# NingZhang1/pyscf_isdf

Measured on AMD Instinct MI355X. Metric: isdf_build_plus_get_jk_wall_time, lower is better.
Workload: dtype f64

## Files before the change

include/mi355_isdf.h:

```cpp
#ifndef MI355_ISDF_H
#define MI355_ISDF_H

#include <stdint.h>

#ifdef __cplusplus
extern "C" {
#endif

typedef struct isdf_ctx* isdf_handle;

#define ISDF_OK 0
#define ISDF_ERR_ARG 1
#define ISDF_ERR_HIP 2
#define ISDF_ERR_LIB 3
#define ISDF_ERR_NUM 4

int isdf_abi_version(void);

int isdf_create(int device_id, isdf_handle* out);
int isdf_destroy(isdf_handle h);
int isdf_set_stream(isdf_handle h, void* hip_stream);
const char* isdf_last_error(isdf_handle h);
int64_t isdf_workspace_bytes(isdf_handle h);
int isdf_release_workspace(isdf_handle h);
int isdf_set_option(isdf_handle h, const char* key, int value);
int isdf_set_coulomb_omega(isdf_handle h, double omega);
int isdf_set_coulomb_cutoff(isdf_handle h, double rc);
int isdf_set_coulomb_ws(isdf_handle h, double alpha, const double ak[9], const int32_t mesh[3], const double maxq[3],
                        const double* d_vq);

int isdf_prof_enable(isdf_handle h, int on);
int isdf_prof_reset(isdf_handle h);
int isdf_prof_count(isdf_handle h);
int isdf_prof_get(isdf_handle h, int index, char* name, int name_cap, int64_t* launches,
                  double* total_ms, double* total_work);

int isdf_eval_ao(isdf_handle h,
                 const int32_t* atm, int natm, const int32_t* bas, int nbas,
                 const double* env, int nenv,
                 const double* Ls, int nimgs, const double* rcut,
                 const double* d_coords, int64_t ngrids,
                 double* d_ao, int64_t ld);

int isdf_eval_ao_deriv1(isdf_handle h, const int32_t* atm, int natm, const int32_t* bas, int nbas, const double* env,
                        int nenv, const double* Ls, int nimgs, const double* rcut, const double* d_coords,
                        int64_t ngrids, double* d_ao, int64_t ld, int64_t plane_stride);
int isdf_eval_ao_k_deriv1(isdf_handle h, const int32_t* atm, int natm, const int32_t* bas, int nbas, const double* env,
                          int nenv, const double* Ls, int nimgs, const double* rcut, const double kpt[3], int periodic_part,
                          const double* d_coords, int64_t ngrids, double* d_re, double* d_im, int64_t ld,
                          int64_t plane_stride);

int isdf_eval_ao_k(isdf_handle h,
                   const int32_t* atm, int natm, const int32_t* bas, int nbas,
                   const double* env, int nenv,
                   const double* Ls, int nimgs, const double* rcut,
                   const double kpt[3], int periodic_part,
                   const double* d_coords, int64_t ngrids,
                   double* d_re, double* d_im, int64_t ld);

int isdf_block_row_absmax(isdf_handle h, const double* d_src, int nrow, int64_t ld, int nblk, const int64_t* d_blk_off,
                          double* d_out);
int isdf_gather_cols(isdf_handle h, const double* d_src, int nrow, int64_t ld_src,
                     const int64_t* d_idx, int64_t n, double* d_dst, int64_t ld_dst);

int isdf_partition_by_atom(isdf_handle h, const double* d_coords, int64_t ngrids, const double* atom_coords, int natm,
                           const double a[9], double tie_atol, int32_t* d_owner);

int isdf_select_ip(isdf_handle h, const double* d_ao, int nao, int64_t ld,
                   int nblk, const int64_t* blk_off, const int32_t* nip,
                   double tol, double tie_rtol,
                   double* d_L, int64_t ldL, int64_t* d_piv, int32_t* rank);

int isdf_select_ip_gram(isdf_handle h, double* d_A, int m, int64_t ldA, int nip, double tol, double tie_rtol,
                        int panel, int64_t* d_piv, int32_t* rank);

int isdf_select_ip_cplx(isdf_handle h, const double* d_ao, int nao, int nh, int64_t ld,
                        int nblk, const int64_t* blk_off, const int32_t* nip,
                        double tol, double tie_rtol,
                        double* d_L, int64_t ldL, int64_t* d_piv, int32_t* rank);

int isdf_fit_from_chol(isdf_handle h, double* d_L, int k, int64_t m, int64_t ldL,
                       const int64_t* d_piv);

int isdf_fit_prepare(isdf_handle h, const double* d_ao, int nao, int64_t ld,
                     const int64_t* d_ip, int P, double reg_rel, double* d_aoP, double* d_chol,
                     double* reg_used);
int isdf_fit_apply(isdf_handle h, const double* d_chol, const double* d_aoP, int P, int nao,
                   const double* d_ao, int64_t ng, int64_t ld, int forward_only,
                   double* d_theta, int64_t ldt);
int isdf_fit_prepare_cplx(isdf_handle h, const double* d_ao, int nao, int nh, int64_t ld,
                          const int64_t* d_ip, int P, double reg_rel, double* d_aoP, double* d_chol,
                          double* reg_used);
int isdf_fit_apply_cplx(isdf_handle h, const double* d_chol, const double* d_aoP, int P, int nao, int nh,
                        const double* d_ao, int64_t ng, int64_t ld, int forward_only,
                        double* d_theta, int64_t ldt);
int isdf_fit_global(isdf_handle h, const double* d_ao, int nao, int64_t ngrids, int64_t ld,
                    const int64_t* d_ip, int P, double reg_rel, double* d_theta, int64_t ldt,
                    double* d_aoP, double* reg_used);

int isdf_gather_aoP(isdf_handle h, const double* d_ao, int nao, int64_t ld, const int64_t* d_ip, int P,
                    double* d_aoP);
int isdf_gram_sq(isdf_handle h, const double* d_aoP, int P, int nao, int nh, double* d_A);
int isdf_pair_gram_rows(isdf_handle h, const double* d_aoP, int P, int nao, int nh, const double* d_ao,
                        int64_t ng, int64_t ld, double* d_B, int64_t ldb);
int isdf_block_chol(isdf_handle h, const double* d_A, int P, int nblk, const int32_t* blk_off,
                    double shift_rel, double* d_D, double* shift_used);
int isdf_block_solve(isdf_handle h, const double* d_D, int P, int nblk, const int32_t* blk_off, int side,
                     int trans, double* d_X, int64_t n, int64_t ldx);
int isdf_block_invert(isdf_handle h, const double* d_D, int P, int nblk, const int32_t* blk_off, double* d_Dinv);
int isdf_block_apply(isdf_handle h, const double* d_Dinv, int64_t ldd, int nblk, const int32_t* blk_off,
                     double* d_X, int64_t n, int64_t ldx);
int isdf_pair_rows_block_apply(isdf_handle h, const double* d_aoP, int P, int nao, const double* d_ao, int64_t ng,
                               int64_t ld, const double* d_Dinv, int64_t ldd, int nblk, const int32_t* blk_off,
                               double* d_B, int64_t ldb);

int isdf_gram_prod(isdf_handle h, const double* d_aoP, int P, int nao, const double* d_psiP, int nocc, double* d_A);
int isdf_pair_prod_rows(isdf_handle h, const double* d_aoP, int P, int nao, const double* d_psiP, int nocc,
                        const double* d_ao, int64_t ld, const double* d_psi, int64_t ldpsi, int64_t ng,
                        double* d_B, int64_t ldb);
int isdf_factor_solve_half(isdf_handle h, const double* d_fac, int P, int backward, double* d_X, int64_t n, int64_t ldx);
int isdf_gram_prod_cplx(isdf_handle h, const double* d_aoP, int P, int nao, int nh, const double* d_psiP, int npsi, int npsi_h,
                        double* d_A);
int isdf_pair_prod_rows_cplx(isdf_handle h, const double* d_aoP, int P, int nao, int nh, const double* d_psiP, int npsi,
                             int npsi_h, const double* d_ao, int64_t ld, const double* d_psi, int64_t ldpsi, int64_t ng,
                             double* d_B, int64_t ldb);

int isdf_shift_diag(isdf_handle h, double* d_A, int P, double shift_rel);
int isdf_chol_inplace(isdf_handle h, double* d_A, int P, double shift_rel, double* d_scratch, double* reg_used);

int isdf_factor_solve(isdf_handle h, const double* d_fac, int P, double* d_X, int64_t n, int64_t ldx);

int isdf_bj_probe_vectors(isdf_handle h, double* d_T, int n, const double* d_fac, const double* d_D, int P,
                          int nblk, const int32_t* blk_off);
int isdf_rows_combine(isdf_handle h, const double* d_E, int n, int64_t ldE, int rows, const double* d_Y,
                      int64_t ng, int64_t ldy, double* d_F, int64_t ldf, int accumulate);

int isdf_bj_probe_rows(isdf_handle h, double* d_T, int n, const double* d_fac, const double* d_D, int P, int nblk,
                       const int32_t* blk_off, const double* d_Yp, int64_t ng, int64_t ldy, double* d_F, int64_t ldf);

int isdf_gather_T(isdf_handle h, const double* d_L, int k, int64_t ldL, const int64_t* d_piv,
                  double* d_T);
int isdf_W_from_factor(isdf_handle h, const double* d_F, int P, int kind, double* d_M, int64_t ldm);

int isdf_coulomb_W(isdf_handle h, const double* d_theta, int P, int64_t ldt,
                   const int32_t mesh[3], const double a[9],
                   int row0, int nrows, int batch, int upper_only, double* d_W, int64_t ldw);
int isdf_coulG_half(isdf_handle h, const int32_t mesh[3], const double a[9], double* d_out);
int isdf_spectral_supported(isdf_handle h, const int32_t mesh[3], int batch, int* ok);
int isdf_spectral_rows(isdf_handle h, const double* d_in, int nrows, int64_t ld, const int32_t mesh[3], const int32_t* d_idx,
                       const double* d_scale, int npts, int batch, double* d_out, int64_t ldx);
int isdf_coulomb_rows(isdf_handle h, const double* d_in, int nrows, int64_t ld,
                      const int32_t mesh[3], const double a[9], int batch, double* d_out, int64_t ldo);
int isdf_symmetrize_upper(isdf_handle h, double* d_W, int P, int64_t ldw);
int isdf_symmetrize_mean(isdf_handle h, double* d_W, int P, int64_t ldw, int antisymmetric);

int isdf_get_j(isdf_handle h, const double* d_ao, int nao, int64_t ngrids, int64_t ld,
               const int32_t mesh[3], const double a[9],
               const double* d_dm, int nset, double* d_vj);
int isdf_rho(isdf_handle h, const double* d_ao, int nao, int64_t ng, int64_t ld,
             const double* d_dm, int nset, double* d_rho, int64_t ldrho);
int isdf_coulomb_potential(isdf_handle h, double* d_rho_inout, int nset, int64_t ldrho,
                           const int32_t mesh[3], const double a[9]);
int isdf_vj_from_vR(isdf_handle h, const double* d_ao, int nao, int64_t ng, int64_t ld,
                    const double* d_vR, int nset, int64_t ldv, double* d_vj);

int isdf_get_k_exact(isdf_handle h, const double* d_ao, int nao, int64_t ngrids, int64_t ld,
                     const double* d_C, int nocc, const int32_t mesh[3], const double a[9],
                     int i0, int ni, int max_rows, double* d_vk);

int isdf_get_k(isdf_handle h, const double* d_aoP, int P, int nao,
               const double* d_W, int64_t ldw, int row0, int nrows,
               const double* d_dm, int nset, double* d_vk);

int isdf_coulG_q(isdf_handle h, const int32_t mesh[3], const double a[9], const double q[3], int wrap_around,
                 double omega, double* d_out);

int isdf_coulomb_Wq(isdf_handle h, const double* d_theta, int P, int64_t ldt, const int32_t mesh[3],
                    const double* d_coulG, double weight, int row0, int nrows, int batch,
                    int upper_only, double* d_Wre, double* d_Wim, int64_t ldw);
int isdf_symmetrize_hermitian(isdf_handle h, double* d_Wre, double* d_Wim, int P, int64_t ldw);
int isdf_finish_Wq(isdf_handle h, const double* d_Wre, const double* d_Wim, int P, int64_t ldw,
                   const double* d_phase, double* d_Wc);
int isdf_get_k_pair(isdf_handle h, const double* d_A1, const double* d_A2, const double* d_D2,
                    const double* d_Wq, int P, int nao, double scale, double* d_vk);

int isdf_get_k_exact_kpt(isdf_handle h, const double* d_u1r, const double* d_u1i, int nao, int64_t ld1,
                         const double* d_m2r, const double* d_m2i, int nocc, int64_t ld2, const int32_t mesh[3],
                         const double* d_coulG, double weight, int i0, int ni, int max_rows, double* d_vk_re,
                         double* d_vk_im);

int isdf_coulomb_rows_q(isdf_handle h, const double* d_rows, int nrows, int64_t ld, const int32_t mesh[3],
                        const double* d_coulG, double* d_re, double* d_im);
int isdf_nyquist_spectra(isdf_handle h, const double* d_rows, int nrows, int64_t ld, const int32_t mesh[3], int axis,
                         double* d_re, double* d_im);
int isdf_zhadamard_planes(isdf_handle h, double* d_Ar, double* d_Ai, int64_t lda, const double* d_Br, const double* d_Bi,
                          int64_t ldb, int rows, int64_t cols);
int isdf_rho_k(isdf_handle h, const double* d_ur, const double* d_ui, int nao, int64_t ng, int64_t ld,
               const double* d_DTr, const double* d_DTi, double scale, double* d_rho);
int isdf_vj_k(isdf_handle h, const double* d_ur, const double* d_ui, int nao, int64_t ng, int64_t ld,
              const double* d_vR, double* d_vj_re, double* d_vj_im);

int isdf_pp_local_potential(isdf_handle h, int natm, const double* coords, const double* pp_par,
                            const int32_t mesh[3], const double a[9], double* d_vlocR);
int isdf_pp_projector_overlaps(isdf_handle h, const int32_t* atm, int natm, const int32_t* bas, int nbas,
                               const double* env, int nenv, const double* coords, const double kpt[3],
                               const int32_t* proj_tab, const double* proj_rl, int nproj,
                               const int32_t mesh[3], const double a[9], double* d_out);

int isdf_gemm_nn(isdf_handle h, int M, int64_t N, int K, double alpha, const double* d_A, int64_t lda, const double* d_B,
                 int64_t ldb, double beta, double* d_C, int64_t ldc);
int isdf_hadamard_rows(isdf_handle h, double* d_X, int64_t ldx, const double* d_Y, int64_t ldy, int rows, int64_t cols);

int isdf_uniform_grid(isdf_handle h, const int32_t mesh[3], const double a[9], double* d_coords_soa);
int isdf_rho_pair(isdf_handle h, const double* d_aoA, int nA, const double* d_aoB, int nB, int64_t ng, int64_t ld,
                  const double* d_dm, int nset, double* d_rho, int64_t ldrho);
int isdf_mg_embed_density(isdf_handle h, const double* d_field, int nset, const int32_t mesh_sub[3], double scale,
                          double* d_spec, const int32_t mesh[3], int accumulate);
int isdf_mg_restrict_potential(isdf_handle h, const double* d_spec, int nset, const int32_t mesh[3],
                               const int32_t mesh_sub[3], double scale, double* d_field);
int isdf_mg_coulomb_kernel(isdf_handle h, double* d_spec, int nset, const int32_t mesh[3], const double a[9]);
int isdf_lda_exchange(isdf_handle h, const double* d_rho, int64_t n, double* d_exc, double* d_vxc);
int isdf_lda_vwn_add(isdf_handle h, const double* d_rho, int64_t n, double* d_exc, double* d_vxc);
int isdf_gga_b88(isdf_handle h, const double* d_rho, const double* d_grad, int64_t gstride, int64_t n, double* d_exc,
                 double* d_vrho, double* d_w, int64_t wstride);
int isdf_xc_fused(isdf_handle h, const double* d_rho, const double* d_grad, int64_t gstride, int64_t n, double c_slater, double c_b88,
                  double c_vwn, int vwn_rpa, double c_lyp, double* d_exc, double* d_vrho, double* d_w, int64_t wstride);
int isdf_gga_lyp_polarised(isdf_handle h, const double* d_rho, const double* d_grad, int64_t gcstride, int64_t sstride, int64_t n,
                           double weight, int accumulate, double* d_ec, double* d_vrho, double* d_w, int64_t wcstride,
                           int64_t osstride);
int isdf_lda_exchange_fxc(isdf_handle h, const double* d_rho, int64_t n, double* d_fxc);
int isdf_lda_vwn_fxc_add(isdf_handle h, const double* d_rho, int64_t n, double* d_fxc);
int isdf_gga_b88_fxc(isdf_handle h, const double* d_rho0, int64_t r0stride, int64_t n, const double* d_rho1, int64_t r1xstride,
                     int64_t r1nstride, int nset, double* d_wv, int64_t wxstride, int64_t wnstride, double* d_fxc, int64_t fstride);
int isdf_xc_fxc_apply(isdf_handle h, int nx, const double* d_fxc, int64_t fxstride, int64_t fystride, int64_t n, const double* d_rho1,
                      int64_t r1xstride, int64_t r1nstride, int nset, double* d_wv, int64_t wxstride, int64_t wnstride, int accumulate);
int isdf_dot(isdf_handle h, const double* d_x, const double* d_y, int64_t n, double* result);

int isdf_gemm_nt(isdf_handle h, int M, int N, int64_t K, double alpha, const double* d_A, int64_t lda,
                 const double* d_B, int64_t ldb, const double* d_kscale, double beta, double* d_C,
                 int64_t ldc);

#ifdef __cplusplus
}
#endif
#endif
```

pyscf_isdf_amd/backend.py:

```python
import ctypes
import os
import numpy as np
import torch
from . import lib as _lib

_vp = ctypes.c_void_p


def _np_ptr(a):
    return a.ctypes.data_as(_vp)


class HipBackend:
    name = 'hip-gfx950'

    def __init__(self, device=0):
        if not torch.cuda.is_available():
            raise _lib.IsdfError('no GPU visible to torch; the ISDF path has no CPU fallback')
        self.device = torch.device('cuda', device)
        torch.cuda.set_device(self.device)
        self.handle = _lib.Handle(device)
        if os.environ.get('ISDF_TRSM') == 'subst':
            self.set_option('trsm_substitution', 1)
        if os.environ.get('ISDF_OWN_FFT') in ('0', '1', '2'):
            self.set_option('own_fft', int(os.environ['ISDF_OWN_FFT']))
        if os.environ.get('ISDF_GEMM_NN') == '1':
            self.set_option('gemm_nn_own', 1)

    def empty(self, shape, dtype=torch.float64):
        return torch.empty(shape, dtype=dtype, device=self.device)

    def zeros(self, shape, dtype=torch.float64):
        return torch.zeros(shape, dtype=dtype, device=self.device)

    def to_device(self, a, dtype=None):
        a = np.ascontiguousarray(a)
        if not a.flags.writeable:
            a = a.copy()
        t = torch.as_tensor(a)
        if dtype is not None:
            t = t.to(dtype)
        return t.to(self.device)

    def to_host(self, t):
        return t.detach().cpu().numpy()

    kernel_epoch = 0

    def set_coulomb_omega(self, omega):
        self.kernel_epoch += 1
        self.handle.call('isdf_set_coulomb_omega', float(omega or 0.0))

    def set_coulomb_cutoff(self, rc):
        self.kernel_epoch += 1
        self.handle.call('isdf_set_coulomb_cutoff', float(rc or 0.0))

    def set_coulomb_ws(self, ws):
        self.kernel_epoch += 1
        if ws is None:
            self.handle.call('isdf_set_coulomb_ws', 0.0, None, None, None, None)
            self._ws_table = None
            return
        ak = np.ascontiguousarray(ws['a'], dtype=np.float64)
        mesh = np.ascontiguousarray(ws['mesh'], dtype=np.int32)
        maxq = np.ascontiguousarray(ws['maxq'], dtype=np.float64)
        self._ws_table = self.to_device(np.ascontiguousarray(ws['vq'], dtype=np.float64))
        self.handle.call('isdf_set_coulomb_ws', float(ws['alpha']), _np_ptr(ak), _np_ptr(mesh), _np_ptr(maxq),
                         self._p(self._ws_table))

    def set_option(self, key, value):
        self.kernel_epoch += 1
        self.handle.call('isdf_set_option', key.encode(), int(value))

    def free_bytes(self):
        free, _ = torch.cuda.mem_get_info(self.device)
        return int(free + torch.cuda.memory_reserved(self.device) - torch.cuda.memory_allocated(self.device))

    def empty_cache(self):
        torch.cuda.empty_cache()

    def synchronize(self):
        torch.cuda.synchronize(self.device)

    def new_stream(self):
        return torch.cuda.Stream(device=self.device)

    def on_stream(self, stream):
        return torch.cuda.stream(stream)

    def record_event(self):
        ev = torch.cuda.Event()
        ev.record(torch.cuda.current_stream(self.device))
        return ev

    def wait_event(self, ev):
        if ev is not None:
            torch.cuda.current_stream(self.device).wait_event(ev)

    def release_workspace(self):
        self.handle.call('isdf_release_workspace')

    def prof_enable(self, on=True):
        self.handle.call('isdf_prof_enable', int(bool(on)))

    def prof_reset(self):
        self.handle.call('isdf_prof_reset')

    def prof_results(self):
        out = {}
        n = self.handle.lib.isdf_prof_count(self.handle.h)
        for i in range(n):
            name = ctypes.create_string_buffer(128)
            launches = ctypes.c_int64(0)
            ms = ctypes.c_double(0)
            work = ctypes.c_double(0)
            self.handle.call('isdf_prof_get', i, name, 128, ctypes.byref(launches), ctypes.byref(ms), ctypes.byref(work))
            out[name.value.decode()] = dict(launches=launches.value, ms=ms.value, work=work.value)
        return out

    def _stream(self):
        s = torch.cuda.current_stream(self.device).cuda_stream
        self.handle.call('isdf_set_stream', _vp(s))

    @staticmethod
    def _p(t):
        assert t.is_contiguous() or t.stride(-1) == 1
        return _vp(t.data_ptr())

    def eval_ao(self, atm, bas, env, Ls, rcut, coords_soa, ao):
        self._stream()
        atm = np.ascontiguousarray(atm, dtype=np.int32)
        bas = np.ascontiguousarray(bas, dtype=np.int32)
        env = np.ascontiguousarray(env, dtype=np.float64)
        Ls = np.ascontiguousarray(Ls, dtype=np.float64)
        rcut = np.ascontiguousarray(rcut, dtype=np.float64)
        G = coords_soa.shape[1]
        assert coords_soa.is_contiguous() and ao.stride(1) == 1 and ao.shape[1] >= G
        self.handle.call('isdf_eval_ao', _np_ptr(atm), len(atm), _np_ptr(bas), len(bas), _np_ptr(env), len(env),
                         _np_ptr(Ls), len(Ls), _np_ptr(rcut), self._p(coords_soa), G, self._p(ao), ao.stride(0))

    def eval_ao_deriv1(self, atm, bas, env, Ls, rcut, coords_soa, ao4):
        self._stream()
        atm = np.ascontiguousarray(atm, dtype=np.int32)
        bas = np.ascontiguousarray(bas, dtype=np.int32)
        env = np.ascontiguousarray(env, dtype=np.float64)
        Ls = np.ascontiguousarray(Ls, dtype=np.float64)
        rcut = np.ascontiguousarray(rcut, dtype=np.float64)
        G = coords_soa.shape[1]
        assert coords_soa.is_contiguous() and ao4.dim() == 3 and ao4.shape[0] == 4 and ao4.stride(2) == 1 and ao4.shape[2] >= G
        self.handle.call('isdf_eval_ao_deriv1', _np_ptr(atm), len(atm), _np_ptr(bas), len(bas), _np_ptr(env), len(env),
                         _np_ptr(Ls), len(Ls), _np_ptr(rcut), self._p(coords_soa), G, self._p(ao4), ao4.stride(1), ao4.stride(0))

    def eval_ao_k_deriv1(self, atm, bas, env, Ls, rcut, kpt, periodic_part, coords_soa, out_re, out_im):
        self._stream()
        atm = np.ascontiguousarray(atm, dtype=np.int32)
        bas = np.ascontiguousarray(bas, dtype=np.int32)
        env = np.ascontiguousarray(env, dtype=np.float64)
        Ls = np.ascontiguousarray(Ls, dtype=np.float64)
        rcut = np.ascontiguousarray(rcut, dtype=np.float64)
        kpt = np.ascontiguousarray(kpt, dtype=np.float64)
        G = coords_soa.shape[1]
        assert out_re.dim() == 3 and out_re.shape[0] == 4 and tuple(out_re.shape) == tuple(out_im.shape)
        assert out_re.stride() == out_im.stride() and out_re.stride(2) == 1 and out_re.shape[2] >= G
        self.handle.call('isdf_eval_ao_k_deriv1', _np_ptr(atm), len(atm), _np_ptr(bas), len(bas), _np_ptr(env), len(env),
                         _np_ptr(Ls), len(Ls), _np_ptr(rcut), _np_ptr(kpt), int(bool(periodic_part)), self._p(coords_soa), G,
                         self._p(out_re), self._p(out_im), out_re.stride(1), out_re.stride(0))

    def gather_cols(self, src, idx, dst):
        self._stream()
        assert idx.dtype == torch.int64 and src.stride(1) == 1 and dst.stride(1) == 1
        self.handle.call('isdf_gather_cols', self._p(src), src.shape[0], src.stride(0), self._p(idx), idx.numel(),
                         self._p(dst), dst.stride(0))

    def block_row_absmax(self, src, blk_off):
        self._stream()
        d_off = self.to_device(np.ascontiguousarray(blk_off, dtype=np.int64))
        out = self.empty((src.shape[0], len(blk_off) - 1))
        self.handle.call('isdf_block_row_absmax', self._p(src), src.shape[0], src.stride(0), len(blk_off) - 1, self._p(d_off), self._p(out))
        return self.to_host(out)

    def partition_by_atom(self, coords, atom_coords, a, tie_atol=1e-9):
        self._stream()
        coords_soa = self.to_device(np.ascontiguousarray(np.asarray(coords, dtype=np.float64).T))
        atoms = np.ascontiguousarray(atom_coords, dtype=np.float64)
        a = np.ascontiguousarray(a, dtype=np.float64)
        G = coords_soa.shape[1]
        owner = self.empty((G,), dtype=torch.int32)
        self.handle.call('isdf_partition_by_atom', self._p(coords_soa), G, _np_ptr(atoms), len(atoms), _np_ptr(a), float(tie_atol),
                         self._p(owner))
        return self.to_host(owner)

    def select_ip(self, ao, blk_off, nip, tol, tie_rtol, L, piv):
        self._stream()
        blk_off = np.ascontiguousarray(blk_off, dtype=np.int64)
        nip = np.ascontiguousarray(nip, dtype=np.int32)
        rank = np.zeros(len(nip), dtype=np.int32)
        assert piv.dtype == torch.int64 and piv.is_contiguous() and ao.stride(1) == 1 and L.stride(1) == 1
        self.handle.call('isdf_select_ip', self._p(ao), ao.shape[0], ao.stride(0), len(nip), _np_ptr(blk_off),
                         _np_ptr(nip), float(tol), float(tie_rtol), self._p(L), L.stride(0), self._p(piv), _np_ptr(rank))
        return rank

    def select_ip_gram(self, A, nip, tol, tie_rtol, piv, panel=0):
        self._stream()
        assert piv.dtype == torch.int64 and piv.is_contiguous() and A.stride(1) == 1 and A.shape[0] == A.shape[1]
        rank = ctypes.c_int32(0)
        self.handle.call('isdf_select_ip_gram', self._p(A), A.shape[0], A.stride(0), int(nip), float(tol), float(tie_rtol),
                         int(panel), self._p(piv), ctypes.byref(rank))
        return int(rank.value)

    def fit_from_chol(self, L, k, m, piv):
        self._stream()
        self.handle.call('isdf_fit_from_chol', self._p(L), int(k), int(m), L.stride(0), self._p(piv))

    def fit_prepare(self, ao, ip, reg_rel, aoP, chol):
        self._stream()
        assert ip.dtype == torch.int64 and aoP.is_contiguous() and chol.is_contiguous()
        reg = ctypes.c_double(0.0)
        self.handle.call('isdf_fit_prepare', self._p(ao), ao.shape[0], ao.stride(0), self._p(ip), ip.numel(),
                         float(reg_rel), self._p(aoP), self._p(chol), ctypes.byref(reg))
        return reg.value

    def fit_apply(self, chol, aoP, ao, ng, theta, forward_only=False):
        self._stream()
        self.handle.call('isdf_fit_apply', self._p(chol), self._p(aoP), aoP.shape[0], aoP.shape[1], self._p(ao),
                         int(ng), ao.stride(0), int(bool(forward_only)), self._p(theta), theta.stride(0))

    def gather_aoP(self, ao, ip, aoP):
        self._stream()
        self.handle.call('isdf_gather_aoP', self._p(ao), ao.shape[0], ao.stride(0), self._p(ip), ip.numel(), self._p(aoP))

    def gram_sq(self, aoP, A, nh=0):
        self._stream()
        self.handle.call('isdf_gram_sq', self._p(aoP), aoP.shape[0], aoP.shape[1], int(nh), self._p(A))

    def pair_gram_rows(self, aoP, ao, ng, B, nh=0):
        self._stream()
        self.handle.call('isdf_pair_gram_rows', self._p(aoP), aoP.shape[0], aoP.shape[1], int(nh), self._p(ao), int(ng),
                         ao.stride(0), self._p(B), B.stride(0))

    def gram_prod(self, aoP, psiP, A):
        self._stream()
        assert aoP.is_contiguous() and psiP.is_contiguous() and A.is_contiguous() and aoP.shape[0] == psiP.shape[0]
        self.handle.call('isdf_gram_prod', self._p(aoP), aoP.shape[0], aoP.shape[1], self._p(psiP), psiP.shape[1], self._p(A))

    def pair_prod_rows(self, aoP, psiP, ao, psi, ng, B):
        self._stream()
        assert aoP.is_contiguous() and psiP.is_contiguous() and aoP.shape[0] == psiP.shape[0]
        assert ao.stride(1) == 1 and psi.stride(1) == 1 and B.stride(1) == 1
        self.handle.call('isdf_pair_prod_rows', self._p(aoP), aoP.shape[0], aoP.shape[1], self._p(psiP), psiP.shape[1],
                         self._p(ao), ao.stride(0), self._p(psi), psi.stride(0), int(ng), self._p(B), B.stride(0))

    def gram_prod_cplx(self, aoP, nh, psiP, npsi_h, A):
        self._stream()
        assert aoP.is_contiguous() and psiP.is_contiguous() and A.is_contiguous() and aoP.shape[0] == psiP.shape[0]
        self.handle.call('isdf_gram_prod_cplx', self._p(aoP), aoP.shape[0], aoP.shape[1], int(nh), self._p(psiP), psiP.shape[1],
                         int(npsi_h), self._p(A))

    def pair_prod_rows_cplx(self, aoP, nh, psiP, npsi_h, ao, psi, ng, B):
        self._stream()
        assert aoP.is_contiguous() and psiP.is_contiguous() and aoP.shape[0] == psiP.shape[0]
        assert ao.stride(1) == 1 and psi.stride(1) == 1 and B.stride(1) == 1
        self.handle.call('isdf_pair_prod_rows_cplx', self._p(aoP), aoP.shape[0], aoP.shape[1], int(nh), self._p(psiP),
                         psiP.shape[1], int(npsi_h), self._p(ao), ao.stride(0), self._p(psi), psi.stride(0), int(ng), self._p(B),
                         B.stride(0))

    def factor_solve_half(self, fac, backward, X):
        self._stream()
        self.handle.call('isdf_factor_solve_half', self._p(fac), fac.shape[0], int(bool(backward)), self._p(X), X.shape[1],
                         X.stride(0))

    def block_chol(self, A, blk_off, shift_rel, D):
        self._stream()
        blk_off = np.ascontiguousarray(blk_off, dtype=np.int32)
        used = ctypes.c_double(0.0)
        self.handle.call('isdf_block_chol', self._p(A), A.shape[0], len(blk_off) - 1, _np_ptr(blk_off), float(shift_rel),
                         self._p(D), ctypes.byref(used))
        return used.value

    def block_solve(self, D, blk_off, side, trans, X):
        self._stream()
        blk_off = np.ascontiguousarray(blk_off, dtype=np.int32)
        n = X.shape[1] if side == 0 else X.shape[0]
        self.handle.call('isdf_block_solve', self._p(D), D.stride(0), len(blk_off) - 1, _np_ptr(blk_off), int(side), int(trans),
                         self._p(X), int(n), X.stride(0))

    def block_invert(self, D, blk_off, Dinv):
        self._stream()
        blk_off = np.ascontiguousarray(blk_off, dtype=np.int32)
        assert D.is_contiguous() and Dinv.is_contiguous() and Dinv.shape == D.shape
        self.handle.call('isdf_block_invert', self._p(D), D.shape[0], len(blk_off) - 1, _np_ptr(blk_off), self._p(Dinv))

    def block_apply(self, Dinv, blk_off, X):
        self._stream()
        blk_off = np.ascontiguousarray(blk_off, dtype=np.int32)
        self.handle.call('isdf_block_apply', self._p(Dinv), Dinv.stride(0), len(blk_off) - 1, _np_ptr(blk_off), self._p(X),
                         X.shape[1], X.stride(0))

    def pair_rows_block_apply(self, aoP, ao, ng, Dinv, blk_off, B):
        self._stream()
        blk_off = np.ascontiguousarray(blk_off, dtype=np.int32)
        assert aoP.stride(1) == 1 and aoP.stride(0) == aoP.shape[1]
        self.handle.call('isdf_pair_rows_block_apply', self._p(aoP), aoP.shape[0], aoP.shape[1], self._p(ao), int(ng), ao.stride(0),
                         self._p(Dinv), Dinv.stride(0), len(blk_off) - 1, _np_ptr(blk_off), self._p(B), B.stride(0))

    def shift_diag(self, A, shift_rel):
        self._stream()
        self.handle.call('isdf_shift_diag', self._p(A), A.shape[0], float(shift_rel))

    def chol_inplace(self, A, shift_rel, scratch=None):
        self._stream()
        reg = ctypes.c_double(0.0)
        assert scratch is None or scratch.numel() >= A.numel()
        self.handle.call('isdf_chol_inplace', self._p(A), A.shape[0], float(shift_rel),
                         self._p(scratch) if scratch is not None else None, ctypes.byref(reg))
        return reg.value

    def factor_solve(self, fac, X):
        self._stream()
        self.handle.call('isdf_factor_solve', self._p(fac), fac.shape[0], self._p(X), X.shape[1], X.stride(0))

    def bj_probe_rows(self, T, fac, D, blk_off, Yp, ng, F):
        self._stream()
        blk_off = np.ascontiguousarray(blk_off, dtype=np.int32)
        self.handle.call('isdf_bj_probe_rows', self._p(T), T.shape[0], self._p(fac), self._p(D), D.shape[0],
                         len(blk_off) - 1, _np_ptr(blk_off), self._p(Yp), int(ng), Yp.stride(0), self._p(F), F.stride(0))

    def bj_probe_vectors(self, T, fac, D, blk_off):
        self._stream()
        blk_off = np.ascontiguousarray(blk_off, dtype=np.int32)
        assert T.is_contiguous()
        self.handle.call('isdf_bj_probe_vectors', self._p(T), T.shape[0], self._p(fac), self._p(D), D.shape[0],
                         len(blk_off) - 1, _np_ptr(blk_off))

    def rows_combine(self, E, Y, F, accumulate=False):
        self._stream()
        assert E.stride(1) == 1 and Y.stride(1) == 1 and F.stride(1) == 1 and E.shape[1] == Y.shape[0]
        self.handle.call('isdf_rows_combine', self._p(E), E.shape[0], E.stride(0), E.shape[1], self._p(Y), Y.shape[1],
                         Y.stride(0), self._p(F), F.stride(0), int(bool(accumulate)))

    def gather_T(self, L, k, piv, T):
        self._stream()
        assert T.is_contiguous() and T.shape == (k, k)
        self.handle.call('isdf_gather_T', self._p(L), int(k), L.stride(0), self._p(piv), self._p(T))

    def W_from_factor(self, F, kind, M):
        self._stream()
        assert F.is_contiguous()
        self.handle.call('isdf_W_from_factor', self._p(F), M.shape[0], int(kind), self._p(M), M.stride(0))

    def fit_global(self, ao, ngrids, ip, reg_rel, theta, aoP):
        self._stream()
        assert ip.dtype == torch.int64 and aoP.is_contiguous()
        reg = ctypes.c_double(0.0)
        self.handle.call('isdf_fit_global', self._p(ao), ao.shape[0], int(ngrids), ao.stride(0), self._p(ip),
                         ip.numel(), float(reg_rel), self._p(theta), theta.stride(0), self._p(aoP), ctypes.byref(reg))
        return reg.value

    def coulomb_W(self, theta, mesh, a, row0, nrows, batch, W, upper_only=False):
        self._stream()
        mesh = np.ascontiguousarray(mesh, dtype=np.int32)
        a = np.ascontiguousarray(a, dtype=np.float64)
        self.handle.call('isdf_coulomb_W', self._p(theta), theta.shape[0], theta.stride(0), _np_ptr(mesh), _np_ptr(a),
                         int(row0), int(nrows), int(batch), int(bool(upper_only)), self._p(W), W.stride(0))

    def coulomb_rows(self, rows, mesh, a, batch, out=None):
        self._stream()
        out = rows if out is None else out
        mesh = np.ascontiguousarray(mesh, dtype=np.int32)
        a = np.ascontiguousarray(a, dtype=np.float64)
        self.handle.call('isdf_coulomb_rows', self._p(rows), rows.shape[0], rows.stride(0), _np_ptr(mesh), _np_ptr(a),
                         int(batch), self._p(out), out.stride(0))

    def spectral_supported(self, mesh, batch=512):
        ok = ctypes.c_int(0)
        mesh = np.ascontiguousarray(mesh, dtype=np.int32)
        self.handle.call('isdf_spectral_supported', _np_ptr(mesh), int(batch), ctypes.byref(ok))
        return bool(ok.value)

    def coulG_half(self, mesh, a):
        self._stream()
        mesh = np.ascontiguousarray(mesh, dtype=np.int32)
        a = np.ascontiguousarray(a, dtype=np.float64)
        out = self.empty((int(mesh[0]) * int(mesh[1]) * (int(mesh[2]) // 2 + 1),))
        self.handle.call('isdf_coulG_half', _np_ptr(mesh), _np_ptr(a), self._p(out))
        return self.to_host(out).reshape(int(mesh[0]), int(mesh[1]), int(mesh[2]) // 2 + 1)

    def spectral_rows(self, rows, mesh, idx, scale, out, batch=512):
        self._stream()
        mesh = np.ascontiguousarray(mesh, dtype=np.int32)
        assert rows.is_contiguous() and out.stride(1) == 1 and idx.dtype == torch.int32 and out.stride(0) % 2 == 0
        self.handle.call('isdf_spectral_rows', self._p(rows), rows.shape[0], rows.stride(0), _np_ptr(mesh), self._p(idx),
                         self._p(scale), int(idx.numel()), int(batch), self._p(out), out.stride(0))

    def symmetrize_upper(self, W):
        self._stream()
        self.handle.call('isdf_symmetrize_upper', self._p(W), W.shape[0], W.stride(0))

    def symmetrize_mean(self, W, antisymmetric=False):
        self._stream()
        self.handle.call('isdf_symmetrize_mean', self._p(W), W.shape[0], W.stride(0), int(bool(antisymmetric)))

    def get_j(self, ao, ngrids, mesh, a, dm, vj):
        self._stream()
        mesh = np.ascontiguousarray(mesh, dtype=np.int32)
        a = np.ascontiguousarray(a, dtype=np.float64)
        assert dm.is_contiguous() and vj.is_contiguous()
        self.handle.call('isdf_get_j', self._p(ao), ao.shape[0], int(ngrids), ao.stride(0), _np_ptr(mesh), _np_ptr(a),
                         self._p(dm), dm.shape[0], self._p(vj))

    def rho(self, ao, ng, dm, rho):
        self._stream()
        self.handle.call('isdf_rho', self._p(ao), ao.shape[0], int(ng), ao.stride(0), self._p(dm), dm.shape[0],
                         self._p(rho), rho.stride(0))

    def coulomb_potential(self, rho, mesh, a):
        self._stream()
        mesh = np.ascontiguousarray(mesh, dtype=np.int32)
        a = np.ascontiguousarray(a, dtype=np.float64)
        self.handle.call('isdf_coulomb_potential', self._p(rho), rho.shape[0], rho.stride(0), _np_ptr(mesh), _np_ptr(a))

    def vj_from_vR(self, ao, ng, vR, vj):
        self._stream()
        self.handle.call('isdf_vj_from_vR', self._p(ao), ao.shape[0], int(ng), ao.stride(0), self._p(vR), vR.shape[0],
                         vR.stride(0), self._p(vj))

    def get_k(self, aoP, W, row0, nrows, dm, vk):
        self._stream()
        assert aoP.is_contiguous() and dm.is_contiguous() and vk.is_contiguous()
        self.handle.call('isdf_get_k', self._p(aoP), aoP.shape[0], aoP.shape[1], self._p(W), W.stride(0), int(row0),
                         int(nrows), self._p(dm), dm.shape[0], self._p(vk))

    def get_k_exact(self, ao, ngrids, C, mesh, a, i0, ni, max_rows, vk):
        self._stream()
        mesh = np.ascontiguousarray(mesh, dtype=np.int32)
        a = np.ascontiguousarray(a, dtype=np.float64)
        assert C.is_contiguous() and vk.is_contiguous()
        self.handle.call('isdf_get_k_exact', self._p(ao), ao.shape[0], int(ngrids), ao.stride(0), self._p(C), C.shape[1],
                         _np_ptr(mesh), _np_ptr(a), int(i0), int(ni), int(max_rows), self._p(vk))

    def gemm_nn(self, A, B, C, alpha=1.0, beta=0.0):
        self._stream()
        self.handle.call('isdf_gemm_nn', A.shape[0], B.shape[1], A.shape[1], float(alpha), self._p(A), A.stride(0), self._p(B),
                         B.stride(0), float(beta), self._p(C), C.stride(0))

    def hadamard_rows(self, X, Y):
        self._stream()
        self.handle.call('isdf_hadamard_rows', self._p(X), X.stride(0), self._p(Y), Y.stride(0), X.shape[0], X.shape[1])

    def gemm_nt(self, A, B, C, alpha=1.0, beta=0.0, kscale=None):
        self._stream()
        M, K = A.shape
        N = B.shape[0]
        assert B.shape[1] == K and tuple(C.shape) == (M, N) and A.stride(1) == 1 and B.stride(1) == 1 and C.stride(1) == 1
        ks = self._p(kscale) if kscale is not None else _vp(0)
        self.handle.call('isdf_gemm_nt', M, N, K, float(alpha), self._p(A), A.stride(0), self._p(B), B.stride(0), ks,
                         float(beta), self._p(C), C.stride(0))

    def uniform_grid(self, mesh, a):
        self._stream()
        mesh = np.ascontiguousarray(mesh, dtype=np.int32)
        a = np.ascontiguousarray(a, dtype=np.float64)
        out = self.empty((3, int(np.prod(mesh))))
        self.handle.call('isdf_uniform_grid', _np_ptr(mesh), _np_ptr(a), self._p(out))
        return out

    def rho_pair(self, aoA, aoB, ng, dm, rho):
        self._stream()
        assert aoA.stride(0) == aoB.stride(0) and aoA.stride(1) == 1 and aoB.stride(1) == 1 and dm.is_contiguous()
        assert tuple(dm.shape[1:]) == (aoA.shape[0], aoB.shape[0])
        self.handle.call('isdf_rho_pair', self._p(aoA), aoA.shape[0], self._p(aoB), aoB.shape[0], int(ng), aoA.stride(0),
                         self._p(dm), dm.shape[0], self._p(rho), rho.stride(0))

    def mg_embed_density(self, field, mesh_sub, scale, spec, mesh, accumulate=True):
        self._stream()
        mesh_sub = np.ascontiguousarray(mesh_sub, dtype=np.int32)
        mesh = np.ascontiguousarray(mesh, dtype=np.int32)
        assert field.is_contiguous() and spec.is_contiguous() and spec.dtype == torch.complex128
        assert field.shape[1] == int(np.prod(mesh_sub)) and spec.shape[1] == int(mesh[0]) * int(mesh[1]) * (int(mesh[2]) // 2 + 1)
        self.handle.call('isdf_mg_embed_density', self._p(field), field.shape[0], _np_ptr(mesh_sub), float(scale), self._p(spec),
                         _np_ptr(mesh), int(bool(accumulate)))

    def mg_restrict_potential(self, spec, mesh, mesh_sub, scale, field):
        self._stream()
        mesh_sub = np.ascontiguousarray(mesh_sub, dtype=np.int32)
        mesh = np.ascontiguousarray(mesh, dtype=np.int32)
        assert field.is_contiguous() and spec.is_contiguous() and spec.dtype == torch.complex128
        assert field.shape[1] == int(np.prod(mesh_sub)) and spec.shape[1] == int(mesh[0]) * int(mesh[1]) * (int(mesh[2]) // 2 + 1)
        self.handle.call('isdf_mg_restrict_potential', self._p(spec), spec.shape[0], _np_ptr(mesh), _np_ptr(mesh_sub), float(scale),
                         self._p(field))

    def mg_coulomb_kernel(self, spec, mesh, a):
        self._stream()
        mesh = np.ascontiguousarray(mesh, dtype=np.int32)
        a = np.ascontiguousarray(a, dtype=np.float64)
        assert spec.is_contiguous() and spec.dtype == torch.complex128
        self.handle.call('isdf_mg_coulomb_kernel', self._p(spec), spec.shape[0], _np_ptr(mesh), _np_ptr(a))

    def lda_exchange(self, rho, exc, vxc):
        self._stream()
        assert rho.is_contiguous() and exc.is_contiguous() and vxc.is_contiguous()
        self.handle.call('isdf_lda_exchange', self._p(rho), rho.numel(), self._p(exc), self._p(vxc))

# ... 199 lines not shown
```

pyscf_isdf_amd/csrc/common.h:

```cpp
#pragma once
#include <hip/hip_runtime.h>
#include <rocblas/rocblas.h>
#include <rocsolver/rocsolver.h>
#include <hipfft/hipfft.h>
#include <cstdint>
#include <cstdio>
#include <cstring>
#include <string>
#include <vector>
#include <map>
#include "../../include/mi355_isdf.h"

struct FftPlan {
  hipfftHandle fwd = 0, bwd = 0;
  size_t work_bytes = 0;
};

struct ProfRec {
  hipEvent_t e0 = nullptr, e1 = nullptr;
};
struct ProfEntry {
  std::vector<ProfRec> recs;
  double work = 0.0;
  double ms = 0.0;
  int64_t launches = 0;
};

struct WsKernel {
  double alpha = 0.0;
  double ak[9] = {0};
  int mesh[3] = {0, 0, 0};
  double maxq[3] = {0, 0, 0};
  const double* vq = nullptr;
};

struct isdf_ctx {
  int profiling = 0;
  std::map<std::string, ProfEntry> prof;
  int device = 0;
  hipStream_t stream = nullptr;
  rocblas_handle blas = nullptr;
  std::string err;
  std::map<std::vector<int>, FftPlan> plans;
  std::map<std::string, std::pair<void*, size_t>> ws;
  int num_cu = 256;
  int trsm_substitution = 0;
  int own_fft = 2;
  int gemm_nn_own = 0;
  int attr_gemm_b = 0, attr_gemm_nn = 0;
  int conv_pipe = 1;
  int conv_sub_rows = 0;
  int gram_pivot_tpb = 256;
  int gram_compact = 1;
  int gram_compact_permille = 875;
  int block_apply_waves = 16;
  int block_apply_reg = 1;
  double coul_omega = 0.0;
  double coul_rc = 0.0;
  int coul_sphere = 0;
  WsKernel wsk;
};

int isdf_fail(isdf_handle h, int code, const char* fmt, ...);
void* isdf_ws(isdf_handle h, const char* name, size_t bytes);
int isdf_get_plan(isdf_handle h, const int32_t mesh[3], int batch, FftPlan** out);
int get_coulG_half(isdf_handle h, const int32_t mesh[3], const double a[9], double extra_scale, double** out);
bool conv_rows_own_supported(const int32_t mesh[3], int nb);
bool conv_rows_q_own_supported(isdf_handle h, const int32_t mesh[3], int nb);
bool spectral_rows_own_supported(isdf_handle h, const int32_t mesh[3], int nb);
int spectral_rows_own(isdf_handle h, const double* d_in, int nb, const int32_t mesh[3], const int32_t* d_idx, const double* d_scale,
                      int npts, double* d_out, int64_t ldx, HIP_vector_type<double, 2u>* zbuf);
int conv_rows_q_own(isdf_handle h, const double* d_in, double* d_re, double* d_im, int nb, const int32_t mesh[3], const double* tab,
                    double2* zhalf, double2* zfull);
int conv_rows_own(isdf_handle h, const double* d_in, double* d_out, int nb, const int32_t mesh[3], const double* cg,
                  double2* zbuf);

#define HIP_TRY(h, expr)                                                                    \
  do {                                                                                      \
    hipError_t e_ = (expr);                                                                 \
    if (e_ != hipSuccess)                                                                   \
      return isdf_fail(h, ISDF_ERR_HIP, "%s:%d %s -> %s", __FILE__, __LINE__, #expr,        \
                       hipGetErrorString(e_));                                              \
  } while (0)
#define BLAS_TRY(h, expr)                                                                   \
  do {                                                                                      \
    rocblas_status s_ = (expr);                                                             \
    if (s_ != rocblas_status_success)                                                       \
      return isdf_fail(h, ISDF_ERR_LIB, "%s:%d %s -> rocblas status %d", __FILE__, __LINE__, \
                       #expr, (int)s_);                                                     \
  } while (0)
#define FFT_TRY(h, expr)                                                                    \
  do {                                                                                      \
    hipfftResult r_ = (expr);                                                               \
    if (r_ != HIPFFT_SUCCESS)                                                               \
      return isdf_fail(h, ISDF_ERR_LIB, "%s:%d %s -> hipfft result %d", __FILE__, __LINE__,  \
                       #expr, (int)r_);                                                     \
  } while (0)
#define KERNEL_CHECK(h) HIP_TRY(h, hipGetLastError())
#define ARG_CHECK(h, cond)                                                                  \
  do {                                                                                      \
    if (!(cond)) return isdf_fail(h, ISDF_ERR_ARG, "%s:%d argument check failed: %s",       \
                                  __FILE__, __LINE__, #cond);                               \
  } while (0)

static inline int64_t cdiv(int64_t a, int64_t b) { return (a + b - 1) / b; }

struct ProfScope {
  isdf_handle h;
  ProfRec rec;
  ProfEntry* ent = nullptr;
  ProfScope(isdf_handle h_, const char* name, double work, int64_t launches = 1) : h(h_) {
    if (!h || !h->profiling) return;
    ent = &h->prof[name];
    ent->work += work;
    ent->launches += launches;
    if (hipEventCreate(&rec.e0) != hipSuccess || hipEventCreate(&rec.e1) != hipSuccess) { ent = nullptr; return; }
    (void)hipEventRecord(rec.e0, h->stream);
  }
  ~ProfScope() {
    if (!ent) return;
    (void)hipEventRecord(rec.e1, h->stream);
    ent->recs.push_back(rec);
  }
};

int gemm_nt_f64(isdf_handle h, int M, int N, int64_t K, double alpha, const double* A, int64_t lda,
                const double* B, int64_t ldb, double beta, double* C, int64_t ldc);
int gemm_nt_f64_scaled(isdf_handle h, int M, int N, int64_t K, double alpha, const double* A, int64_t lda,
                       const double* B, int64_t ldb, const double* kscale, double beta, double* C,
                       int64_t ldc);
int trsm_lower_left(isdf_handle h, bool trans, int m, int64_t n, const double* L, int64_t ldl, double* X, int64_t ldx);
int trsm_lower_right(isdf_handle h, bool trans, int m, int64_t n, const double* L, int64_t ldl, double* X, int64_t ldx);
int block_forward_solve(isdf_handle h, const double* D, int64_t ldd, int nblk, const int32_t* blk_off_host, double* X,
                        int64_t ldx, int64_t n);
int block_apply_inverse(isdf_handle h, const double* Dinv, int64_t ldd, int nblk, const int32_t* blk_off_host, double* X,
                        int64_t ldx, int64_t n, bool square_input = false);
int transpose_rm(isdf_handle h, const double* src, int64_t lds, int64_t rows, int64_t cols, double* dst, int64_t ldd);
int tri_left(isdf_handle h, bool trans, int m, int64_t n, const double* L, int64_t ldl, double* X, int64_t ldx);
int tri_right(isdf_handle h, bool trans, int m, int64_t n, const double* L, int64_t ldl, double* X, int64_t ldx);
bool gemm_nn_f64_supported(isdf_handle h, int64_t M, int64_t N, int64_t K, const double* A, int64_t lda, const double* B,
                           int64_t ldb);
int gemm_nn_f64(isdf_handle h, int64_t M, int64_t N, int64_t K, const double* A, int64_t lda, const double* B, int64_t ldb,
                double* C, int64_t ldc, bool square);
int gemm_rm(isdf_handle h, char opA, char opB, int64_t M, int64_t N, int64_t K, double alpha,
            const double* A, int64_t lda, const double* B, int64_t ldb, double beta, double* C,
            int64_t ldc);
```

pyscf_isdf_amd/csrc/gemm_f64.hip:

```cpp
#include "common.h"
#include <cstdlib>

int gemm_rm(isdf_handle h, char opA, char opB, int64_t M, int64_t N, int64_t K, double alpha,
            const double* A, int64_t lda, const double* B, int64_t ldb, double beta, double* C,
            int64_t ldc) {
  ARG_CHECK(h, M < 2147483647LL && N < 2147483647LL && K < 2147483647LL && lda < 2147483647LL &&
                   ldb < 2147483647LL && ldc < 2147483647LL);
  const rocblas_operation ta = (opA == 'N') ? rocblas_operation_none : rocblas_operation_transpose;
  const rocblas_operation tb = (opB == 'N') ? rocblas_operation_none : rocblas_operation_transpose;
  ProfScope ps(h, "rocblas_dgemm[flop]", 2.0 * M * N * (double)K);
  BLAS_TRY(h, rocblas_dgemm(h->blas, tb, ta, (rocblas_int)N, (rocblas_int)M, (rocblas_int)K, &alpha, B,
                            (rocblas_int)ldb, A, (rocblas_int)lda, &beta, C, (rocblas_int)ldc));
  return ISDF_OK;
}

namespace {

typedef double d4 __attribute__((ext_vector_type(4)));

constexpr int BM = 128, BN = 128, BK = 16;
constexpr int LDT = 17;
constexpr int TPB = 256;

struct GemmArgs {
  const double* A; int64_t lda;
  const double* B; int64_t ldb;
  const double* kscale;
  double* P;
  int64_t ldp, slab_stride;
  int M, N;
  int64_t K, kslab;
  int ntm, ntn, nslab;
  int64_t nunits, nunits_pad;
  double alpha, beta;
  int direct;
};

template <bool FAST>
__global__ __launch_bounds__(TPB, 2) void gemm_nt_mfma_kernel(GemmArgs g) {
  __shared__ double sA[2][BM * LDT];
  __shared__ double sB[2][BN * LDT];

  const int64_t bid = blockIdx.x;
  const int64_t per_xcd = g.nunits_pad / 8;
  const int64_t unit = (bid % 8) * per_xcd + bid / 8;
  if (unit >= g.nunits) return;
  const int tm = (int)(unit % g.ntm);
  const int tn = (int)((unit / g.ntm) % g.ntn);
  const int slab = (int)(unit / ((int64_t)g.ntm * g.ntn));
  const int64_t k0 = (int64_t)slab * g.kslab;
  const int64_t k1 = (k0 + g.kslab < g.K) ? k0 + g.kslab : g.K;
  const int nchunks = (int)((k1 - k0 + BK - 1) / BK);

  const int tid = threadIdx.x;
  const int lane = tid & 63, wave = tid >> 6;
  const int wm = wave >> 1, wn = wave & 1;

  const int srow = tid >> 3;
  const int sseg = tid & 7;
  const int arow0 = tm * BM + srow, brow0 = tn * BN + srow;
  const int mlast = g.M - 1, nlast = g.N - 1;
  const double* __restrict__ Ag = g.A;
  const double* __restrict__ Bg = g.B;
  const int64_t lda = g.lda, ldb = g.ldb;

  double2 ra0, ra1, ra2, ra3, rb0, rb1, rb2, rb3;
#define ISDF_LOAD_ONE(I, RA, RB)                                                              \
  {                                                                                           \
    const int ra = min(arow0 + 32 * I, mlast), rb = min(brow0 + 32 * I, nlast);               \
    const double* pa = Ag + (int64_t)ra * lda + k;                                            \
    const double* pb = Bg + (int64_t)rb * ldb + k;                                            \
    if (FAST) {                                                                               \
      RA = *reinterpret_cast<const double2*>(pa);                                             \
      RB = *reinterpret_cast<const double2*>(pb);                                             \
    } else {                                                                                  \
      RA.x = v0 ? pa[0] : 0.0; RA.y = v1 ? pa[1] : 0.0;                                       \
      RB.x = v0 ? pb[0] : 0.0; RB.y = v1 ? pb[1] : 0.0;                                       \
    }                                                                                         \
    RB.x *= s0; RB.y *= s1;                                                                   \
  }
#define ISDF_LOAD_CHUNK(C)                                                                    \
  {                                                                                           \
    const int64_t k = k0 + (int64_t)(C) * BK + sseg * 2;                                      \
    const bool v0 = FAST || (k < k1), v1 = FAST || (k + 1 < k1);                              \
    double s0 = 1.0, s1 = 1.0;                                                                \
    if (g.kscale) { if (v0) s0 = g.kscale[k]; if (v1) s1 = g.kscale[k + 1]; }                 \
    ISDF_LOAD_ONE(0, ra0, rb0) ISDF_LOAD_ONE(1, ra1, rb1)                                     \
    ISDF_LOAD_ONE(2, ra2, rb2) ISDF_LOAD_ONE(3, ra3, rb3)                                     \
  }
#define ISDF_STORE_ONE(BUF, I, RA, RB)                                                        \
  { double* qa = &sA[BUF][(srow + 32 * I) * LDT + sseg * 2];                                  \
    double* qb = &sB[BUF][(srow + 32 * I) * LDT + sseg * 2];                                  \
    qa[0] = RA.x; qa[1] = RA.y; qb[0] = RB.x; qb[1] = RB.y; }
#define ISDF_STORE_CHUNK(BUF)                                                                 \
  { ISDF_STORE_ONE(BUF, 0, ra0, rb0) ISDF_STORE_ONE(BUF, 1, ra1, rb1)                         \
    ISDF_STORE_ONE(BUF, 2, ra2, rb2) ISDF_STORE_ONE(BUF, 3, ra3, rb3) }

  d4 acc[4][4];
#pragma unroll
  for (int i = 0; i < 4; ++i)
#pragma unroll
    for (int j = 0; j < 4; ++j) acc[i][j] = (d4){0.0, 0.0, 0.0, 0.0};

  const int frow = lane & 15, fk = lane >> 4;
  ISDF_LOAD_CHUNK(0)
  ISDF_STORE_CHUNK(0)
  __syncthreads();
  for (int c = 0; c < nchunks; ++c) {
    const int buf = c & 1;
    if (c + 1 < nchunks) ISDF_LOAD_CHUNK(c + 1)
    const double* pa = &sA[buf][(wm * 64 + frow) * LDT + fk];
    const double* pb = &sB[buf][(wn * 64 + frow) * LDT + fk];
    double a0[4], b0[4], a1[4], b1[4];
#define ISDF_FRAGS(KK, AF, BF)                                                                \
    _Pragma("unroll") for (int i = 0; i < 4; ++i) {                                           \
      AF[i] = pa[i * 16 * LDT + (KK) * 4];                                                    \
      BF[i] = pb[i * 16 * LDT + (KK) * 4];                                                    \
    }
#define ISDF_MFMA16(AF, BF)                                                                   \
    _Pragma("unroll") for (int i = 0; i < 4; ++i)                                             \
      _Pragma("unroll") for (int j = 0; j < 4; ++j)                                           \
        acc[i][j] = __builtin_amdgcn_mfma_f64_16x16x4f64(AF[i], BF[j], acc[i][j], 0, 0, 0);
    ISDF_FRAGS(0, a0, b0)
    ISDF_FRAGS(1, a1, b1)
    ISDF_MFMA16(a0, b0)
    ISDF_FRAGS(2, a0, b0)
    ISDF_MFMA16(a1, b1)
    ISDF_FRAGS(3, a1, b1)
    ISDF_MFMA16(a0, b0)
    ISDF_MFMA16(a1, b1)
    if (c + 1 < nchunks) ISDF_STORE_CHUNK(buf ^ 1)
    __syncthreads();
  }

  double* out = g.P + (int64_t)slab * g.slab_stride;
#pragma unroll
  for (int i = 0; i < 4; ++i) {
#pragma unroll
    for (int r = 0; r < 4; ++r) {
      const int row = tm * BM + wm * 64 + i * 16 + (lane >> 4) + 4 * r;
      if (row >= g.M) continue;
#pragma unroll
      for (int j = 0; j < 4; ++j) {
        const int col = tn * BN + wn * 64 + j * 16 + (lane & 15);
        if (col >= g.N) continue;
        double* q = out + (int64_t)row * g.ldp + col;
        const double v = acc[i][j][r];
        if (g.direct) *q = (g.beta == 0.0) ? g.alpha * v : g.alpha * v + g.beta * (*q);
        else *q = v;
      }
    }
  }
}

constexpr int BM2 = 256;
constexpr int TPB2 = 512;

template <bool SCALED>
__global__ __launch_bounds__(TPB2, 2) void gemm_nt_mfma_kernel_b(GemmArgs g) {
  extern __shared__ double smem[];
  double* sA = smem;
  double* sB = smem + 2 * BM2 * LDT;
  const int64_t bid = blockIdx.x;
  const int64_t per_xcd = g.nunits_pad / 8;
  const int64_t unit = (bid % 8) * per_xcd + bid / 8;
  if (unit >= g.nunits) return;
  const int tm = (int)(unit % g.ntm);
  const int tn = (int)((unit / g.ntm) % g.ntn);
  const int slab = (int)(unit / ((int64_t)g.ntm * g.ntn));
  const int64_t k0 = (int64_t)slab * g.kslab;
  const int64_t k1 = (k0 + g.kslab < g.K) ? k0 + g.kslab : g.K;
  const int nchunks = (int)((k1 - k0) / BK);
  const int last = nchunks - 1;

  const int tid = threadIdx.x;
  const int lane = tid & 63, wave = tid >> 6;
  const int wm = wave >> 1, wn = wave & 1;
  const int srow = tid >> 3;
  const int sseg = tid & 7;
  const int mlast = g.M - 1, nlast = g.N - 1;
  const double* pA0 = g.A + (int64_t)min(tm * BM2 + srow, mlast) * g.lda + k0 + sseg * 2;
  const double* pA1 = g.A + (int64_t)min(tm * BM2 + srow + 64, mlast) * g.lda + k0 + sseg * 2;
  const double* pA2 = g.A + (int64_t)min(tm * BM2 + srow + 128, mlast) * g.lda + k0 + sseg * 2;
  const double* pA3 = g.A + (int64_t)min(tm * BM2 + srow + 192, mlast) * g.lda + k0 + sseg * 2;
  const double* pB0 = g.B + (int64_t)min(tn * BN + srow, nlast) * g.ldb + k0 + sseg * 2;
  const double* pB1 = g.B + (int64_t)min(tn * BN + srow + 64, nlast) * g.ldb + k0 + sseg * 2;
  const double* pS = SCALED ? g.kscale + k0 + sseg * 2 : nullptr;

  double2 xa0, xa1, xa2, xa3, xb0, xb1, ya0, ya1, ya2, ya3, yb0, yb1;
#define ISDF_LOADB(C, A0, A1, A2, A3, B0, B1)                                                 \
  {                                                                                           \
    const int off = (C) * BK;                                                                 \
    A0 = *reinterpret_cast<const double2*>(pA0 + off);                                        \
    A1 = *reinterpret_cast<const double2*>(pA1 + off);                                        \
    A2 = *reinterpret_cast<const double2*>(pA2 + off);                                        \
    A3 = *reinterpret_cast<const double2*>(pA3 + off);                                        \
    B0 = *reinterpret_cast<const double2*>(pB0 + off);                                        \
    B1 = *reinterpret_cast<const double2*>(pB1 + off);                                        \
    if (SCALED) {                                                                             \
      const double2 sc = *reinterpret_cast<const double2*>(pS + off);                         \
      B0.x *= sc.x; B0.y *= sc.y; B1.x *= sc.x; B1.y *= sc.y;                                 \
    }                                                                                         \
  }
#define ISDF_ST1(P, R) { double* q_ = (P); q_[0] = R.x; q_[1] = R.y; }
#define ISDF_STOREB(BUF, A0, A1, A2, A3, B0, B1)                                              \
  {                                                                                           \
    double* qa = sA + (BUF) * BM2 * LDT + srow * LDT + sseg * 2;                              \
    double* qb = sB + (BUF) * BN * LDT + srow * LDT + sseg * 2;                               \
    ISDF_ST1(qa, A0) ISDF_ST1(qa + 64 * LDT, A1) ISDF_ST1(qa + 128 * LDT, A2)                 \
    ISDF_ST1(qa + 192 * LDT, A3) ISDF_ST1(qb, B0) ISDF_ST1(qb + 64 * LDT, B1)                 \
  }

  d4 acc[4][4];
#pragma unroll
  for (int i = 0; i < 4; ++i)
#pragma unroll
    for (int j = 0; j < 4; ++j) acc[i][j] = (d4){0.0, 0.0, 0.0, 0.0};
  const int frow = lane & 15, fk = lane >> 4;

#define ISDF_FRAGB(KK, AF, BF)                                                                \
    _Pragma("unroll") for (int i = 0; i < 4; ++i) {                                           \
      AF[i] = pa[i * 16 * LDT + (KK) * 4];                                                    \
      BF[i] = pb[i * 16 * LDT + (KK) * 4];                                                    \
    }
#define ISDF_MFMAB(AF, BF)                                                                    \
    _Pragma("unroll") for (int i = 0; i < 4; ++i)                                             \
      _Pragma("unroll") for (int j = 0; j < 4; ++j)                                           \
        acc[i][j] = __builtin_amdgcn_mfma_f64_16x16x4f64(AF[i], BF[j], acc[i][j], 0, 0, 0);
#define ISDF_INTERLEAVE() _Pragma("unroll") for (int q_ = 0; q_ < 8; ++q_) {                  \
    __builtin_amdgcn_sched_group_barrier(0x008, 2, 0); __builtin_amdgcn_sched_group_barrier(0x100, 1, 0); }
#define ISDF_INTERLEAVE_W() _Pragma("unroll") for (int q_ = 0; q_ < 6; ++q_) {                \
    __builtin_amdgcn_sched_group_barrier(0x008, 2, 0); __builtin_amdgcn_sched_group_barrier(0x200, 1, 0); }
#define ISDF_INTERLEAVE_L() _Pragma("unroll") for (int q_ = 0; q_ < 8; ++q_) {                \
    __builtin_amdgcn_sched_group_barrier(0x008, 2, 0); __builtin_amdgcn_sched_group_barrier(0x100, 1, 0);                \
    if (q_ < 6) __builtin_amdgcn_sched_group_barrier(0x020, 1, 0); }
  const int aoff = (wm * 64 + frow) * LDT + fk, boff = (wn * 64 + frow) * LDT + fk;
  double a0[4], b0[4], a1[4], b1[4];
#define ISDF_FRAGQ(BUF, KK, AF, BF)                                                           \
  {                                                                                           \
    const double* pa = sA + (BUF) * BM2 * LDT + aoff;                                         \
    const double* pb = sB + (BUF) * BN * LDT + boff;                                          \
    _Pragma("unroll") for (int i = 0; i < 4; ++i) {                                           \
      AF[i] = pa[i * 16 * LDT + (KK) * 4];                                                    \
      BF[i] = pb[i * 16 * LDT + (KK) * 4];                                                    \
    }                                                                                         \
  }
#define ISDF_INTERLEAVE_RW() _Pragma("unroll") for (int q_ = 0; q_ < 8; ++q_) {               \
    __builtin_amdgcn_sched_group_barrier(0x008, 2, 0); __builtin_amdgcn_sched_group_barrier(0x100, 1, 0);                \
    if (q_ < 6) __builtin_amdgcn_sched_group_barrier(0x200, 1, 0); }
#define ISDF_CHUNKB(BUF, LOAD_AHEAD, STORE_NEXT)                                              \
  {                                                                                           \
    ISDF_FRAGQ(BUF, 1, a1, b1)                                                                \
    LOAD_AHEAD                                                                                \
    ISDF_MFMAB(a0, b0)                                                                        \
    ISDF_INTERLEAVE_L()                                                                       \
    __builtin_amdgcn_sched_barrier(0);                                                        \
    ISDF_FRAGQ(BUF, 2, a0, b0)                                                                \
    ISDF_MFMAB(a1, b1)                                                                        \
    ISDF_INTERLEAVE()                                                                         \
    __builtin_amdgcn_sched_barrier(0);                                                        \
    ISDF_FRAGQ(BUF, 3, a1, b1)                                                                \
    STORE_NEXT                                                                                \
    ISDF_MFMAB(a0, b0)                                                                        \
    ISDF_INTERLEAVE_RW()                                                                      \
    __builtin_amdgcn_sched_barrier(0);                                                        \
    __syncthreads();                                                                          \
    ISDF_FRAGQ(1 - (BUF), 0, a0, b0)                                                          \
    ISDF_MFMAB(a1, b1)                                                                        \
    ISDF_INTERLEAVE()                                                                         \
    __builtin_amdgcn_sched_barrier(0);                                                        \
  }

  ISDF_LOADB(0, xa0, xa1, xa2, xa3, xb0, xb1)
  ISDF_LOADB(1, ya0, ya1, ya2, ya3, yb0, yb1)
  ISDF_STOREB(0, xa0, xa1, xa2, xa3, xb0, xb1)
  __syncthreads();
  ISDF_FRAGQ(0, 0, a0, b0)
  __builtin_amdgcn_sched_barrier(0);
  for (int c = 0; c < nchunks; c += 2) {
    ISDF_CHUNKB(0, ISDF_LOADB(min(c + 2, last), xa0, xa1, xa2, xa3, xb0, xb1), ISDF_STOREB(1, ya0, ya1, ya2, ya3, yb0, yb1))
    ISDF_CHUNKB(1, ISDF_LOADB(min(c + 3, last), ya0, ya1, ya2, ya3, yb0, yb1), ISDF_STOREB(0, xa0, xa1, xa2, xa3, xb0, xb1))
  }

  double* out = g.P + (int64_t)slab * g.slab_stride;
#pragma unroll
  for (int i = 0; i < 4; ++i) {
#pragma unroll
    for (int r = 0; r < 4; ++r) {
      const int row = tm * BM2 + wm * 64 + i * 16 + (lane >> 4) + 4 * r;
      if (row >= g.M) continue;
#pragma unroll
      for (int j = 0; j < 4; ++j) {
        const int col = tn * BN + wn * 64 + j * 16 + (lane & 15);
        if (col >= g.N) continue;
        double* q = out + (int64_t)row * g.ldp + col;
        const double v = acc[i][j][r];
        if (g.direct) *q = (g.beta == 0.0) ? g.alpha * v : g.alpha * v + g.beta * (*q);
        else *q = v;
      }
    }
  }
}

constexpr int TPBD = 256;

template <bool SCALED>
__global__ __launch_bounds__(TPBD, 2) void gemm_nt_mfma_kernel_d(GemmArgs g) {
  __shared__ double sB[2][BN * LDT];
  const int64_t bid = blockIdx.x;
  const int64_t per_xcd = g.nunits_pad / 8;
  const int64_t unit = (bid % 8) * per_xcd + bid / 8;
  if (unit >= g.nunits) return;
  const int tm = (int)(unit % g.ntm);
  const int tn = (int)((unit / g.ntm) % g.ntn);
  const int slab = (int)(unit / ((int64_t)g.ntm * g.ntn));
  const int64_t k0 = (int64_t)slab * g.kslab;
  const int64_t k1 = (k0 + g.kslab < g.K) ? k0 + g.kslab : g.K;
  const int nchunks = (int)((k1 - k0) / BK);
  const int last = nchunks - 1;

  const int tid = threadIdx.x;
  const int lane = tid & 63, wave = tid >> 6;
  const int frow = lane & 15, fkq = lane >> 4;
  const int mlast = g.M - 1, nlast = g.N - 1;
  const double* pA0 = g.A + (int64_t)min(tm * BM + wave * 32 + frow, mlast) * g.lda + k0 + 4 * fkq;
  const double* pA1 = g.A + (int64_t)min(tm * BM + wave * 32 + 16 + frow, mlast) * g.lda + k0 + 4 * fkq;
  const int srow = tid >> 2, sseg = tid & 3;
  const double* pB0 = g.B + (int64_t)min(tn * BN + srow, nlast) * g.ldb + k0 + 4 * sseg;
  const double* pB1 = g.B + (int64_t)min(tn * BN + srow + 64, nlast) * g.ldb + k0 + 4 * sseg;
  const double* pS = SCALED ? g.kscale + k0 + 4 * sseg : nullptr;

  double2 xa00, xa01, xa10, xa11, xb00, xb01, xb10, xb11;
  double2 ya00, ya01, ya10, ya11, yb00, yb01, yb10, yb11;
#define ISDF_LOADD(C, A00, A01, A10, A11, B00, B01, B10, B11)                                 \
  {                                                                                           \
    const int off = (C) * BK;                                                                 \
    A00 = *reinterpret_cast<const double2*>(pA0 + off);                                       \
    A01 = *reinterpret_cast<const double2*>(pA0 + off + 2);                                   \
    A10 = *reinterpret_cast<const double2*>(pA1 + off);                                       \
    A11 = *reinterpret_cast<const double2*>(pA1 + off + 2);                                   \
    B00 = *reinterpret_cast<const double2*>(pB0 + off);                                       \
    B01 = *reinterpret_cast<const double2*>(pB0 + off + 2);                                   \
    B10 = *reinterpret_cast<const double2*>(pB1 + off);                                       \
    B11 = *reinterpret_cast<const double2*>(pB1 + off + 2);                                   \
    if (SCALED) {                                                                             \
      const double2 s0 = *reinterpret_cast<const double2*>(pS + off);                         \
      const double2 s1 = *reinterpret_cast<const double2*>(pS + off + 2);                     \
      B00.x *= s0.x; B00.y *= s0.y; B01.x *= s1.x; B01.y *= s1.y;                             \
      B10.x *= s0.x; B10.y *= s0.y; B11.x *= s1.x; B11.y *= s1.y;                             \
    }                                                                                         \
  }
#define ISDF_STORED(BUF, B00, B01, B10, B11)                                                  \
  {                                                                                           \
    double* q0 = &sB[BUF][srow * LDT + 4 * sseg];                                             \
    double* q1 = &sB[BUF][(srow + 64) * LDT + 4 * sseg];                                      \
    q0[0] = B00.x; q0[1] = B00.y; q0[2] = B01.x; q0[3] = B01.y;                               \
    q1[0] = B10.x; q1[1] = B10.y; q1[2] = B11.x; q1[3] = B11.y;                               \
  }

  d4 acc[2][8];
#pragma unroll
  for (int i = 0; i < 2; ++i)
#pragma unroll
    for (int j = 0; j < 8; ++j) acc[i][j] = (d4){0.0, 0.0, 0.0, 0.0};

  double bf0[8], bf1[8];
#define ISDF_FRAGD(BUF, J, BF)                                                                \
  {                                                                                           \
    const double* pb = &sB[BUF][frow * LDT + 4 * fkq + (J)];                                  \
    _Pragma("unroll") for (int jn = 0; jn < 8; ++jn) BF[jn] = pb[jn * 16 * LDT];              \
  }
#define ISDF_MFMAD(AV0, AV1, BF)                                                              \
    _Pragma("unroll") for (int jn = 0; jn < 8; ++jn) {                                        \
      acc[0][jn] = __builtin_amdgcn_mfma_f64_16x16x4f64(AV0, BF[jn], acc[0][jn], 0, 0, 0);    \
      acc[1][jn] = __builtin_amdgcn_mfma_f64_16x16x4f64(AV1, BF[jn], acc[1][jn], 0, 0, 0);    \
    }
#define ISDF_ILD_R() _Pragma("unroll") for (int q_ = 0; q_ < 8; ++q_) {                       \
    __builtin_amdgcn_sched_group_barrier(0x008, 2, 0); __builtin_amdgcn_sched_group_barrier(0x100, 1, 0); }
#define ISDF_ILD_RL() _Pragma("unroll") for (int q_ = 0; q_ < 8; ++q_) {                      \
    __builtin_amdgcn_sched_group_barrier(0x008, 2, 0); __builtin_amdgcn_sched_group_barrier(0x100, 1, 0);                \
    __builtin_amdgcn_sched_group_barrier(0x020, 1, 0); }
#define ISDF_ILD_RW() _Pragma("unroll") for (int q_ = 0; q_ < 8; ++q_) {                      \
    __builtin_amdgcn_sched_group_barrier(0x008, 2, 0); __builtin_amdgcn_sched_group_barrier(0x100, 1, 0);                \
    if (q_ < 4) __builtin_amdgcn_sched_group_barrier(0x200, 1, 0); }
#define ISDF_CHUNKD(BUF, A00, A01, A10, A11, LOAD_AHEAD, STORE_NEXT)                          \
  {                                                                                           \
    ISDF_FRAGD(BUF, 1, bf1)                                                                   \
    ISDF_MFMAD(A00.x, A10.x, bf0)                                                             \
    ISDF_ILD_R()                                                                              \
    __builtin_amdgcn_sched_barrier(0);                                                        \
    ISDF_FRAGD(BUF, 2, bf0)                                                                   \
    ISDF_MFMAD(A00.y, A10.y, bf1)                                                             \
    ISDF_ILD_R()                                                                              \
    __builtin_amdgcn_sched_barrier(0);                                                        \
    ISDF_FRAGD(BUF, 3, bf1)                                                                   \
    STORE_NEXT                                                                                \
    ISDF_MFMAD(A01.x, A11.x, bf0)                                                             \
    ISDF_ILD_RW()                                                                             \
    __builtin_amdgcn_sched_barrier(0);                                                        \
    __syncthreads();                                                                          \
    ISDF_FRAGD(1 - (BUF), 0, bf0)                                                             \
    ISDF_MFMAD(A01.y, A11.y, bf1)                                                             \
    LOAD_AHEAD                                                                                \
    ISDF_ILD_RL()                                                                             \
    __builtin_amdgcn_sched_barrier(0);                                                        \
  }

  ISDF_LOADD(0, xa00, xa01, xa10, xa11, xb00, xb01, xb10, xb11)
  ISDF_LOADD(min(1, last), ya00, ya01, ya10, ya11, yb00, yb01, yb10, yb11)
  ISDF_STORED(0, xb00, xb01, xb10, xb11)
  __syncthreads();
  ISDF_FRAGD(0, 0, bf0)
  __builtin_amdgcn_sched_barrier(0);
  for (int c = 0; c < nchunks; c += 2) {
    ISDF_CHUNKD(0, xa00, xa01, xa10, xa11, ISDF_LOADD(min(c + 2, last), xa00, xa01, xa10, xa11, xb00, xb01, xb10, xb11),
                ISDF_STORED(1, yb00, yb01, yb10, yb11))
    ISDF_CHUNKD(1, ya00, ya01, ya10, ya11, ISDF_LOADD(min(c + 3, last), ya00, ya01, ya10, ya11, yb00, yb01, yb10, yb11),
                ISDF_STORED(0, xb00, xb01, xb10, xb11))
  }

  double* out = g.P + (int64_t)slab * g.slab_stride;
#pragma unroll
  for (int i = 0; i < 2; ++i) {
#pragma unroll
    for (int r = 0; r < 4; ++r) {
      const int row = tm * BM + wave * 32 + i * 16 + (lane >> 4) + 4 * r;
      if (row >= g.M) continue;
#pragma unroll
      for (int j = 0; j < 8; ++j) {
        const int col = tn * BN + j * 16 + (lane & 15);
        if (col >= g.N) continue;
        double* q = out + (int64_t)row * g.ldp + col;
        const double v = acc[i][j][r];
        if (g.direct) *q = (g.beta == 0.0) ? g.alpha * v : g.alpha * v + g.beta * (*q);
        else *q = v;
      }
    }
  }
}

constexpr int LDN = 144;

struct GemmNNArgs {
  const double* A; int64_t lda;
  const double* B; int64_t ldb;
  double* C; int64_t ldc;
  int M, N, K;
  int ntm, ntn, stm, stn, ngm;
  int64_t nunits, nunits_pad;
};

template <bool SQ>
__global__ __launch_bounds__(TPB2, 2) void gemm_nn_mfma_kernel(GemmNNArgs g) {
  extern __shared__ double smem[];
  double* sA = smem;
  double* sB = smem + 2 * BM2 * LDT;
  const int64_t bid = blockIdx.x;
  const int64_t per_xcd = g.nunits_pad / 8;
  const int64_t unit = (bid % 8) * per_xcd + bid / 8;
  if (unit >= g.nunits) return;
  const int per = g.stm * g.stn;
  const int64_t grp = unit / per;
  const int within = (int)(unit - grp * per);
  const int tm = (int)(grp % g.ngm) * g.stm + within % g.stm;
  const int tn = (int)(grp / g.ngm) * g.stn + within / g.stm;
  if (tm >= g.ntm || tn >= g.ntn) return;
  const int nchunks = g.K / BK;
  const int last = nchunks - 1;

  const int tid = threadIdx.x;
  const int lane = tid & 63, wave = tid >> 6;
  const int wm = wave >> 1, wn = wave & 1;
  const int srow = tid >> 3, sseg = tid & 7;
  const int krow = tid >> 6, nseg = tid & 63;
  const int mlast = g.M - 1;
  const double* pA0 = g.A + (int64_t)min(tm * BM2 + srow, mlast) * g.lda + sseg * 2;
  const double* pA1 = g.A + (int64_t)min(tm * BM2 + srow + 64, mlast) * g.lda + sseg * 2;
  const double* pA2 = g.A + (int64_t)min(tm * BM2 + srow + 128, mlast) * g.lda + sseg * 2;
  const double* pA3 = g.A + (int64_t)min(tm * BM2 + srow + 192, mlast) * g.lda + sseg * 2;
  const double* pB0 = g.B + (int64_t)krow * g.ldb + min(tn * BN + 2 * nseg, g.N - 2);
  const double* pB1 = pB0 + 8 * g.ldb;
  const int64_t bstep = (int64_t)BK * g.ldb;

  double2 xa0, xa1, xa2, xa3, xb0, xb1, ya0, ya1, ya2, ya3, yb0, yb1;
#define ISDF_NN_LOAD(C, A0, A1, A2, A3, B0, B1)                                               \
  {                                                                                           \
    const int off = (C) * BK;                                                                 \
    const int64_t offb = (C) * bstep;                                                         \
    A0 = *reinterpret_cast<const double2*>(pA0 + off);                                        \
    A1 = *reinterpret_cast<const double2*>(pA1 + off);                                        \
    A2 = *reinterpret_cast<const double2*>(pA2 + off);                                        \
    A3 = *reinterpret_cast<const double2*>(pA3 + off);                                        \
    B0 = *reinterpret_cast<const double2*>(pB0 + offb);                                       \
    B1 = *reinterpret_cast<const double2*>(pB1 + offb);                                       \
  }
#define ISDF_NN_ST1(P, R) { double* q_ = (P); q_[0] = R.x; q_[1] = R.y; }
#define ISDF_NN_STORE(BUF, A0, A1, A2, A3, B0, B1)                                            \
  {                                                                                           \
    double* qa = sA + (BUF) * BM2 * LDT + srow * LDT + sseg * 2;                              \
    double* qb = sB + (BUF) * BK * LDN + krow * LDN + 2 * nseg;                               \
    ISDF_NN_ST1(qa, A0) ISDF_NN_ST1(qa + 64 * LDT, A1) ISDF_NN_ST1(qa + 128 * LDT, A2)        \
    ISDF_NN_ST1(qa + 192 * LDT, A3)                                                           \
    *reinterpret_cast<double2*>(qb) = B0;                                                     \
    *reinterpret_cast<double2*>(qb + 8 * LDN) = B1;                                           \
  }

  d4 acc[4][4];
#pragma unroll
  for (int i = 0; i < 4; ++i)
#pragma unroll
    for (int j = 0; j < 4; ++j) acc[i][j] = (d4){0.0, 0.0, 0.0, 0.0};
  const int frow = lane & 15, fk = lane >> 4;
  const int aoff = (wm * 64 + frow) * LDT + fk, boff = fk * LDN + wn * 64 + frow;
  double a0[4], b0[4], a1[4], b1[4];
#define ISDF_NN_FRAG(BUF, KK, AF, BF)                                                         \
  {                                                                                           \
    const double* pa = sA + (BUF) * BM2 * LDT + aoff;                                         \
    const double* pb = sB + (BUF) * BK * LDN + boff;                                          \
    _Pragma("unroll") for (int i = 0; i < 4; ++i) {                                           \
      AF[i] = pa[i * 16 * LDT + (KK) * 4];                                                    \
      BF[i] = pb[(KK) * 4 * LDN + i * 16];                                                    \
    }                                                                                         \
  }
#define ISDF_NN_MFMA(AF, BF)                                                                  \
    _Pragma("unroll") for (int i = 0; i < 4; ++i)                                             \
      _Pragma("unroll") for (int j = 0; j < 4; ++j)                                           \
        acc[i][j] = __builtin_amdgcn_mfma_f64_16x16x4f64(AF[i], BF[j], acc[i][j], 0, 0, 0);
#define ISDF_NN_IL() _Pragma("unroll") for (int q_ = 0; q_ < 8; ++q_) {                       \
    __builtin_amdgcn_sched_group_barrier(0x008, 2, 0); __builtin_amdgcn_sched_group_barrier(0x100, 1, 0); }
#define ISDF_NN_IL_L() _Pragma("unroll") for (int q_ = 0; q_ < 8; ++q_) {                     \
    __builtin_amdgcn_sched_group_barrier(0x008, 2, 0); __builtin_amdgcn_sched_group_barrier(0x100, 1, 0);                \
    if (q_ < 6) __builtin_amdgcn_sched_group_barrier(0x020, 1, 0); }
#define ISDF_NN_IL_RW() _Pragma("unroll") for (int q_ = 0; q_ < 8; ++q_) {                    \
    __builtin_amdgcn_sched_group_barrier(0x008, 2, 0); __builtin_amdgcn_sched_group_barrier(0x100, 1, 0);                \
    if (q_ < 6) __builtin_amdgcn_sched_group_barrier(0x200, 1, 0); }
#define ISDF_NN_CHUNK(BUF, LOAD_AHEAD, STORE_NEXT)                                            \
  {                                                                                           \
    ISDF_NN_FRAG(BUF, 1, a1, b1)                                                              \
    LOAD_AHEAD                                                                                \
    ISDF_NN_MFMA(a0, b0)                                                                      \
    ISDF_NN_IL_L()                                                                            \
    __builtin_amdgcn_sched_barrier(0);                                                        \
    ISDF_NN_FRAG(BUF, 2, a0, b0)                                                              \
    ISDF_NN_MFMA(a1, b1)                                                                      \
    ISDF_NN_IL()                                                                              \
    __builtin_amdgcn_sched_barrier(0);                                                        \
    ISDF_NN_FRAG(BUF, 3, a1, b1)                                                              \
    STORE_NEXT                                                                                \
    ISDF_NN_MFMA(a0, b0)                                                                      \
    ISDF_NN_IL_RW()                                                                           \
    __builtin_amdgcn_sched_barrier(0);                                                        \
    __syncthreads();                                                                          \
    ISDF_NN_FRAG(1 - (BUF), 0, a0, b0)                                                        \
    ISDF_NN_MFMA(a1, b1)                                                                      \
    ISDF_NN_IL()                                                                              \
    __builtin_amdgcn_sched_barrier(0);                                                        \
  }

  ISDF_NN_LOAD(0, xa0, xa1, xa2, xa3, xb0, xb1)
  ISDF_NN_LOAD(1, ya0, ya1, ya2, ya3, yb0, yb1)
  ISDF_NN_STORE(0, xa0, xa1, xa2, xa3, xb0, xb1)
  __syncthreads();
  ISDF_NN_FRAG(0, 0, a0, b0)
  __builtin_amdgcn_sched_barrier(0);
  for (int c = 0; c < nchunks; c += 2) {
    ISDF_NN_CHUNK(0, ISDF_NN_LOAD(min(c + 2, last), xa0, xa1, xa2, xa3, xb0, xb1), ISDF_NN_STORE(1, ya0, ya1, ya2, ya3, yb0, yb1))
    ISDF_NN_CHUNK(1, ISDF_NN_LOAD(min(c + 3, last), ya0, ya1, ya2, ya3, yb0, yb1), ISDF_NN_STORE(0, xa0, xa1, xa2, xa3, xb0, xb1))
  }

#pragma unroll
  for (int i = 0; i < 4; ++i) {
#pragma unroll
    for (int r = 0; r < 4; ++r) {
      const int row = tm * BM2 + wm * 64 + i * 16 + (lane >> 4) + 4 * r;
      if (row >= g.M) continue;
#pragma unroll
      for (int j = 0; j < 4; ++j) {
        const int col = tn * BN + wn * 64 + j * 16 + (lane & 15);
        if (col >= g.N) continue;
        const double v = acc[i][j][r];
        g.C[(int64_t)row * g.ldc + col] = SQ ? v * v : v;
      }
    }
  }
}

__global__ void reduce_slabs_kernel(const double* __restrict__ P, int nslab, int64_t slab_stride,
                                    int M, int N, double alpha, double beta, double* __restrict__ C,
                                    int64_t ldc) {
  const int64_t idx = (int64_t)blockIdx.x * blockDim.x + threadIdx.x;
  if (idx >= (int64_t)M * N) return;
  const int m = (int)(idx / N), n = (int)(idx % N);
  double s = 0.0;
  for (int t = 0; t < nslab; ++t) s += P[(int64_t)t * slab_stride + idx];
  double* q = C + (int64_t)m * ldc + n;
  *q = (beta == 0.0) ? alpha * s : alpha * s + beta * (*q);
}

}

int gemm_nt_f64_scaled(isdf_handle h, int M, int N, int64_t K, double alpha, const double* A, int64_t lda,
                       const double* B, int64_t ldb, const double* kscale, double beta, double* C,
                       int64_t ldc) {
  ARG_CHECK(h, M > 0 && N > 0 && K > 0 && A && B && C && lda >= K && ldb >= K && ldc >= N);
  GemmArgs g;
  g.A = A; g.lda = lda; g.B = B; g.ldb = ldb; g.kscale = kscale;
  g.M = M; g.N = N; g.K = K;
  static const int variant = getenv("ISDF_GEMM_VARIANT") ? atoi(getenv("ISDF_GEMM_VARIANT")) : -1;
  const bool alignedB = (lda % 2 == 0) && (ldb % 2 == 0) && (K % 32 == 0) && (((uintptr_t)A) % 16 == 0) &&
                        (((uintptr_t)B) % 16 == 0) && (!kscale || ((uintptr_t)kscale) % 16 == 0);
  const bool fitsB = (double)(cdiv(M, BM2) * BM2) <= 1.15 * (double)M;
  const bool useB = alignedB && M > BM && (variant == 1 || (variant == -1 && fitsB));
  const bool useD = alignedB && !useB && (variant == 3 || variant == -1);
  g.ntm = (int)cdiv(M, useB ? BM2 : BM); g.ntn = (int)cdiv(N, BN);
  const int64_t ntiles = (int64_t)g.ntm * g.ntn;
  const int64_t slots = (int64_t)h->num_cu * (useB ? 1 : 2);
  int64_t nslab = cdiv(8 * slots, ntiles);
  const int64_t cap = std::max<int64_t>(1, std::min<int64_t>(std::max<int64_t>(1, K / 2048),
                                                             std::max<int64_t>(1, ((int64_t)2 << 30) / ((int64_t)M * N * 8))));
  nslab = std::max<int64_t>(1, std::min<int64_t>(nslab, cap));
  {
    static const int tune = getenv("ISDF_GEMM_SLAB_TUNE") ? atoi(getenv("ISDF_GEMM_SLAB_TUNE")) : 1;
    if (tune && ntiles * nslab > slots) {
      double best = 1e30;
      int64_t pick = nslab;
      for (int64_t c = nslab; c <= std::min<int64_t>(2 * nslab, cap); ++c) {
        const double units = (double)ntiles * c;
        const double waste = (double)(cdiv((int64_t)units, slots) * slots) / units;
        if (waste < best - 1e-9) { best = waste; pick = c; }
      }
      nslab = pick;
    }
  }
  g.kslab = cdiv(cdiv(K, nslab), 2 * BK) * (2 * BK);
  g.nslab = (int)cdiv(K, g.kslab);
  g.nunits = ntiles * g.nslab;
  g.nunits_pad = cdiv(g.nunits, 8) * 8;
  g.alpha = alpha; g.beta = beta;
  if (g.nslab == 1) {
    g.direct = 1; g.P = C; g.ldp = ldc; g.slab_stride = 0;
  } else {
    g.direct = 0;
    g.P = (double*)isdf_ws(h, "gemm_partials", sizeof(double) * (size_t)g.nslab * M * N);
    if (!g.P) return ISDF_ERR_HIP;
    g.ldp = N; g.slab_stride = (int64_t)M * N;
  }
  const bool fast = (lda % 2 == 0) && (ldb % 2 == 0) && (K % BK == 0) &&
                    (((uintptr_t)A) % 16 == 0) && (((uintptr_t)B) % 16 == 0) &&
                    (!kscale || ((uintptr_t)kscale) % 16 == 0);
  ARG_CHECK(h, g.nunits_pad < 2147483647LL);
  const char* label = useD ? (kscale ? "gemm_nt_mfma_kernel_d<true>[flop]" : "gemm_nt_mfma_kernel_d<false>[flop]") : useB ? (kscale ? "gemm_nt_mfma_kernel_b<true>[flop]" : "gemm_nt_mfma_kernel_b<false>[flop]")
                           : (fast ? "gemm_nt_mfma_kernel<true>[flop]" : "gemm_nt_mfma_kernel<false>[flop]");
  {
    ProfScope ps(h, label, 2.0 * M * N * (double)K);
    if (useD) {
      if (kscale) hipLaunchKernelGGL(gemm_nt_mfma_kernel_d<true>, dim3((unsigned)g.nunits_pad), dim3(TPBD), 0, h->stream, g);
      else hipLaunchKernelGGL(gemm_nt_mfma_kernel_d<false>, dim3((unsigned)g.nunits_pad), dim3(TPBD), 0, h->stream, g);
    } else if (useB) {
      const size_t lds = sizeof(double) * 2 * (BM2 + BN) * LDT;
      if (!h->attr_gemm_b) {
        HIP_TRY(h, hipFuncSetAttribute((const void*)gemm_nt_mfma_kernel_b<true>, hipFuncAttributeMaxDynamicSharedMemorySize, (int)lds));
        HIP_TRY(h, hipFuncSetAttribute((const void*)gemm_nt_mfma_kernel_b<false>, hipFuncAttributeMaxDynamicSharedMemorySize, (int)lds));
        h->attr_gemm_b = 1;
      }
      if (kscale) hipLaunchKernelGGL(gemm_nt_mfma_kernel_b<true>, dim3((unsigned)g.nunits_pad), dim3(TPB2), lds, h->stream, g);
      else hipLaunchKernelGGL(gemm_nt_mfma_kernel_b<false>, dim3((unsigned)g.nunits_pad), dim3(TPB2), lds, h->stream, g);
    } else if (fast) hipLaunchKernelGGL(gemm_nt_mfma_kernel<true>, dim3((unsigned)g.nunits_pad), dim3(TPB), 0, h->stream, g);
    else hipLaunchKernelGGL(gemm_nt_mfma_kernel<false>, dim3((unsigned)g.nunits_pad), dim3(TPB), 0, h->stream, g);
    KERNEL_CHECK(h);
  }
  if (!g.direct) {
    ProfScope ps(h, "gemm_reduce_slabs_kernel[byte]", 8.0 * (double)M * N * (g.nslab + 1));
    hipLaunchKernelGGL(reduce_slabs_kernel, dim3((unsigned)cdiv((int64_t)M * N, 256)), dim3(256), 0, h->stream,
                       g.P, g.nslab, g.slab_stride, M, N, alpha, beta, C, ldc);
    KERNEL_CHECK(h);
  }
  return ISDF_OK;
}

int gemm_nt_f64(isdf_handle h, int M, int N, int64_t K, double alpha, const double* A, int64_t lda,
                const double* B, int64_t ldb, double beta, double* C, int64_t ldc) {
  return gemm_nt_f64_scaled(h, M, N, K, alpha, A, lda, B, ldb, nullptr, beta, C, ldc);
}

extern "C" int isdf_gemm_nt(isdf_handle h, int M, int N, int64_t K, double alpha, const double* d_A,
                            int64_t lda, const double* d_B, int64_t ldb, const double* d_kscale,
                            double beta, double* d_C, int64_t ldc) {
  if (!h) return ISDF_ERR_ARG;
  return gemm_nt_f64_scaled(h, M, N, K, alpha, d_A, lda, d_B, ldb, d_kscale, beta, d_C, ldc);
}

bool gemm_nn_f64_supported(isdf_handle h, int64_t M, int64_t N, int64_t K, const double* A, int64_t lda, const double* B,
                           int64_t ldb) {
  return h->gemm_nn_own && M > BM && (double)(cdiv(M, BM2) * BM2) <= 1.15 * (double)M && N >= 2 && N % 2 == 0 && K >= 32 && K % 32 == 0 &&
         lda % 2 == 0 && ldb % 2 == 0 && ((uintptr_t)A) % 16 == 0 && ((uintptr_t)B) % 16 == 0 && M < 2147483647LL &&
         N < 2147483647LL && K < 2147483647LL;
}

int gemm_nn_f64(isdf_handle h, int64_t M, int64_t N, int64_t K, const double* A, int64_t lda, const double* B, int64_t ldb,
                double* C, int64_t ldc, bool square) {
  ARG_CHECK(h, A && B && C && lda >= K && ldb >= N && ldc >= N && gemm_nn_f64_supported(h, M, N, K, A, lda, B, ldb));
  GemmNNArgs g;
  g.A = A; g.lda = lda; g.B = B; g.ldb = ldb; g.C = C; g.ldc = ldc;
  g.M = (int)M; g.N = (int)N; g.K = (int)K;
  g.ntm = (int)cdiv(M, BM2); g.ntn = (int)cdiv(N, BN);
  g.stm = g.ntm >= 4 ? 4 : (g.ntm >= 2 ? 2 : 1);
  g.stn = 32 / g.stm;
  g.ngm = (int)cdiv(g.ntm, g.stm);
  g.nunits = (int64_t)g.ngm * cdiv(g.ntn, g.stn) * 32;
  g.nunits_pad = cdiv(g.nunits, 8) * 8;
  ARG_CHECK(h, g.nunits_pad < 2147483647LL);
  const size_t lds = sizeof(double) * 2 * (BM2 * LDT + BK * LDN);
  if (!h->attr_gemm_nn) {
    HIP_TRY(h, hipFuncSetAttribute((const void*)gemm_nn_mfma_kernel<true>, hipFuncAttributeMaxDynamicSharedMemorySize, (int)lds));
    HIP_TRY(h, hipFuncSetAttribute((const void*)gemm_nn_mfma_kernel<false>, hipFuncAttributeMaxDynamicSharedMemorySize, (int)lds));
    h->attr_gemm_nn = 1;
  }
  ProfScope ps(h, square ? "gemm_nn_mfma_kernel<true>[flop]" : "gemm_nn_mfma_kernel<false>[flop]", 2.0 * M * N * (double)K);
  if (square) hipLaunchKernelGGL(gemm_nn_mfma_kernel<true>, dim3((unsigned)g.nunits_pad), dim3(TPB2), lds, h->stream, g);
  else hipLaunchKernelGGL(gemm_nn_mfma_kernel<false>, dim3((unsigned)g.nunits_pad), dim3(TPB2), lds, h->stream, g);
  KERNEL_CHECK(h);
  return ISDF_OK;
}
```

pyscf_isdf_amd/csrc/handle.hip:

```cpp
#include "common.h"
#include <cstdarg>

int isdf_fail(isdf_handle h, int code, const char* fmt, ...) {
  char buf[1024];
  va_list ap;
  va_start(ap, fmt);
  vsnprintf(buf, sizeof(buf), fmt, ap);
  va_end(ap);
  if (h) h->err = buf;
  else fprintf(stderr, "mi355_isdf: %s\n", buf);
  return code;
}

void* isdf_ws(isdf_handle h, const char* name, size_t bytes) {
  auto& slot = h->ws[name];
  if (slot.second >= bytes && slot.first) return slot.first;
  if (slot.first) {
    (void)hipStreamSynchronize(h->stream);
    (void)hipFree(slot.first);
    slot.first = nullptr;
    slot.second = 0;
  }
  void* p = nullptr;
  hipError_t e = hipMalloc(&p, bytes ? bytes : 8);
  if (e != hipSuccess) {
    isdf_fail(h, ISDF_ERR_HIP, "workspace '%s': hipMalloc(%zu) failed: %s", name, bytes,
              hipGetErrorString(e));
    return nullptr;
  }
  slot.first = p;
  slot.second = bytes;
  return p;
}

int isdf_get_plan(isdf_handle h, const int32_t mesh[3], int batch, FftPlan** out) {
  std::vector<int> key = {mesh[0], mesh[1], mesh[2], batch};
  auto it = h->plans.find(key);
  if (it != h->plans.end()) {
    *out = &it->second;
    return ISDF_OK;
  }
  FftPlan p;
  int dims[3] = {mesh[0], mesh[1], mesh[2]};
  int64_t G = (int64_t)mesh[0] * mesh[1] * mesh[2];
  int64_t Gc = (int64_t)mesh[0] * mesh[1] * (mesh[2] / 2 + 1);
  ARG_CHECK(h, G < (int64_t)2147483647);
  FFT_TRY(h, hipfftPlanMany(&p.fwd, 3, dims, nullptr, 1, (int)G, nullptr, 1, (int)Gc, HIPFFT_D2Z, batch));
  hipfftResult r2 = hipfftPlanMany(&p.bwd, 3, dims, nullptr, 1, (int)Gc, nullptr, 1, (int)G, HIPFFT_Z2D, batch);
  if (r2 == HIPFFT_SUCCESS) r2 = hipfftSetStream(p.fwd, h->stream);
  if (r2 == HIPFFT_SUCCESS) r2 = hipfftSetStream(p.bwd, h->stream);
  if (r2 != HIPFFT_SUCCESS) {
    (void)hipfftDestroy(p.fwd);
    if (p.bwd) (void)hipfftDestroy(p.bwd);
    return isdf_fail(h, ISDF_ERR_LIB, "hipFFT plan (%d x %d x %d, batch %d) failed: result %d", mesh[0], mesh[1], mesh[2], batch,
                     (int)r2);
  }
  auto res = h->plans.emplace(key, p);
  *out = &res.first->second;
  return ISDF_OK;
}

extern "C" {

int isdf_abi_version(void) { return 21; }

int isdf_set_coulomb_omega(isdf_handle h, double omega) {
  if (!h) return ISDF_ERR_ARG;
  h->coul_omega = omega;
  return ISDF_OK;
}

int isdf_set_coulomb_cutoff(isdf_handle h, double rc) {
  if (!h) return ISDF_ERR_ARG;
  ARG_CHECK(h, rc >= 0.0);
  h->coul_rc = rc;
  return ISDF_OK;
}

int isdf_set_coulomb_ws(isdf_handle h, double alpha, const double ak[9], const int32_t mesh[3], const double maxq[3],
                        const double* d_vq) {
  if (!h) return ISDF_ERR_ARG;
  if (alpha <= 0.0) { h->wsk = WsKernel(); return ISDF_OK; }
  ARG_CHECK(h, ak && mesh && maxq && d_vq && mesh[0] > 0 && mesh[1] > 0 && mesh[2] > 0);
  h->wsk.alpha = alpha;
  for (int i = 0; i < 9; ++i) h->wsk.ak[i] = ak[i];
  for (int i = 0; i < 3; ++i) { h->wsk.mesh[i] = mesh[i]; h->wsk.maxq[i] = maxq[i]; }
  h->wsk.vq = d_vq;
  return ISDF_OK;
}

int isdf_set_option(isdf_handle h, const char* key, int value) {
  if (!h) return ISDF_ERR_ARG;
  ARG_CHECK(h, key != nullptr);
  if (std::string(key) == "trsm_substitution") { h->trsm_substitution = value ? 1 : 0; return ISDF_OK; }
  if (std::string(key) == "own_fft") { h->own_fft = value < 0 ? 0 : (value > 2 ? 2 : value); return ISDF_OK; }
  if (std::string(key) == "gemm_nn_own") { h->gemm_nn_own = value ? 1 : 0; return ISDF_OK; }
  if (std::string(key) == "coul_sphere") { h->coul_sphere = value < 0 ? 0 : value; return ISDF_OK; }
  if (std::string(key) == "conv_pipe") { h->conv_pipe = value != 0; return ISDF_OK; }
  if (std::string(key) == "conv_sub_rows") { h->conv_sub_rows = value < 0 ? 0 : value; return ISDF_OK; }
  if (std::string(key) == "gram_pivot_tpb") {
    if (value != 64 && value != 128 && value != 256) return ISDF_ERR_ARG;
    h->gram_pivot_tpb = value;
    return ISDF_OK;
  }
  if (std::string(key) == "gram_compact") { h->gram_compact = value ? 1 : 0; return ISDF_OK; }
  if (std::string(key) == "gram_compact_permille") {
    if (value < 1 || value > 1000) return isdf_fail(h, ISDF_ERR_ARG, "isdf_set_option: gram_compact_permille %d not in [1, 1000]", value);
    h->gram_compact_permille = value;
    return ISDF_OK;
  }
  if (std::string(key) == "block_apply_waves") { h->block_apply_waves = value < 1 ? 1 : value; return ISDF_OK; }
  if (std::string(key) == "block_apply_reg") { h->block_apply_reg = value ? 1 : 0; return ISDF_OK; }
  return isdf_fail(h, ISDF_ERR_ARG, "isdf_set_option: unknown key '%s'", key);
}

int isdf_create(int device_id, isdf_handle* out) {
  if (!out) return ISDF_ERR_ARG;
  *out = nullptr;
  int ndev = 0;
  hipError_t e = hipGetDeviceCount(&ndev);
  if (e != hipSuccess || ndev == 0)
    return isdf_fail(nullptr, ISDF_ERR_HIP, "no HIP device visible (%s)", hipGetErrorString(e));
  if (device_id < 0 || device_id >= ndev)
    return isdf_fail(nullptr, ISDF_ERR_ARG, "device %d out of range (%d devices)", device_id, ndev);
  isdf_ctx* h = new isdf_ctx();
  h->device = device_id;
  if (hipSetDevice(device_id) != hipSuccess) { delete h; return ISDF_ERR_HIP; }
  hipDeviceProp_t prop;
  if (hipGetDeviceProperties(&prop, device_id) == hipSuccess) h->num_cu = prop.multiProcessorCount;
  if (rocblas_create_handle(&h->blas) != rocblas_status_success) {
    delete h;
    return isdf_fail(nullptr, ISDF_ERR_LIB, "rocblas_create_handle failed");
  }
  rocblas_set_pointer_mode(h->blas, rocblas_pointer_mode_host);
  *out = h;
  return ISDF_OK;
}

int isdf_release_workspace(isdf_handle h) {
  if (!h) return ISDF_ERR_ARG;
  (void)hipStreamSynchronize(h->stream);
  for (auto& kv : h->ws)
    if (kv.second.first) (void)hipFree(kv.second.first);
  h->ws.clear();
  for (auto& kv : h->plans) {
    if (kv.second.fwd) hipfftDestroy(kv.second.fwd);
    if (kv.second.bwd) hipfftDestroy(kv.second.bwd);
  }
  h->plans.clear();
  return ISDF_OK;
}

int isdf_destroy(isdf_handle h) {
  if (!h) return ISDF_OK;
  isdf_prof_reset(h);
  isdf_release_workspace(h);
  if (h->blas) rocblas_destroy_handle(h->blas);
  delete h;
  return ISDF_OK;
}

int isdf_set_stream(isdf_handle h, void* hip_stream) {
  if (!h) return ISDF_ERR_ARG;
  h->stream = (hipStream_t)hip_stream;
  BLAS_TRY(h, rocblas_set_stream(h->blas, h->stream));
  for (auto& kv : h->plans) {
    if (kv.second.fwd) FFT_TRY(h, hipfftSetStream(kv.second.fwd, h->stream));
    if (kv.second.bwd) FFT_TRY(h, hipfftSetStream(kv.second.bwd, h->stream));
  }
  return ISDF_OK;
}

const char* isdf_last_error(isdf_handle h) { return h ? h->err.c_str() : "null handle"; }

int isdf_prof_enable(isdf_handle h, int on) {
  if (!h) return ISDF_ERR_ARG;
  h->profiling = on ? 1 : 0;
  return ISDF_OK;
}

int isdf_prof_reset(isdf_handle h) {
  if (!h) return ISDF_ERR_ARG;
  (void)hipStreamSynchronize(h->stream);
  for (auto& kv : h->prof)
    for (auto& r : kv.second.recs) { (void)hipEventDestroy(r.e0); (void)hipEventDestroy(r.e1); }
  h->prof.clear();
  return ISDF_OK;
}

int isdf_prof_count(isdf_handle h) { return h ? (int)h->prof.size() : 0; }

int isdf_prof_get(isdf_handle h, int index, char* name, int name_cap, int64_t* launches, double* total_ms,
                  double* total_work) {
  if (!h || index < 0 || index >= (int)h->prof.size()) return ISDF_ERR_ARG;
  auto it = h->prof.begin();
  std::advance(it, index);
  (void)hipStreamSynchronize(h->stream);
  double ms = 0.0;
  for (auto& r : it->second.recs) {
    float t = 0.f;
    if (hipEventElapsedTime(&t, r.e0, r.e1) == hipSuccess) ms += t;
  }
  if (name && name_cap > 0) { strncpy(name, it->first.c_str(), name_cap - 1); name[name_cap - 1] = 0; }
  if (launches) *launches = it->second.launches;
  if (total_ms) *total_ms = ms;
  if (total_work) *total_work = it->second.work;
  return ISDF_OK;
}

int64_t isdf_workspace_bytes(isdf_handle h) {
  if (!h) return 0;
  int64_t s = 0;
  for (auto& kv : h->ws) s += (int64_t)kv.second.second;
  return s;
}

}
```

pyscf_isdf_amd/csrc/select_ip.hip:

```cpp
#include "common.h"
#include <cfloat>
#include <climits>

namespace {

constexpr int TPB = 256;

struct BlkState {
  unsigned long long dmax_bits;
  long long cand;
  double dp;
  double tol;
  long long pivot;
  int done;
  int rank;
};

__device__ inline double wave_max_d(double v) {
  for (int o = 32; o > 0; o >>= 1) v = fmax(v, __shfl_xor(v, o));
  return v;
}
__device__ inline long long wave_min_ll(long long v) {
  for (int o = 32; o > 0; o >>= 1) {
    long long u = __shfl_xor(v, o);
    v = u < v ? u : v;
  }
  return v;
}

__global__ __launch_bounds__(TPB) void init_diag_kernel(
    const double* __restrict__ ao, int nao, int64_t ld, const int* __restrict__ wg_blk,
    const int64_t* __restrict__ wg_lo, const int64_t* __restrict__ blk_off, double* __restrict__ d,
    BlkState* __restrict__ st) {
  __shared__ double red[TPB / 64];
  const int b = wg_blk[blockIdx.x];
  const int64_t i = wg_lo[blockIdx.x] + threadIdx.x;
  const bool valid = i < blk_off[b + 1];
  double s = 0.0;
  if (valid) {
    const double* __restrict__ p = ao + i;
#pragma unroll 8
    for (int mu = 0; mu < nao; ++mu) {
      const double v = p[(int64_t)mu * ld];
      s = fma(v, v, s);
    }
    s = s * s;
    d[i] = s;
  }
  double m = wave_max_d(valid ? s : 0.0);
  if ((threadIdx.x & 63) == 0) red[threadIdx.x >> 6] = m;
  __syncthreads();
  if (threadIdx.x == 0) {
    for (int w = 1; w < TPB / 64; ++w) m = fmax(m, red[w]);
    atomicMax(&st[b].dmax_bits, (unsigned long long)__double_as_longlong(m));
  }
}

__global__ __launch_bounds__(TPB) void find_first_kernel(
    const double* __restrict__ d, const int* __restrict__ wg_blk, const int64_t* __restrict__ wg_lo,
    const int64_t* __restrict__ blk_off, BlkState* __restrict__ st, double tie_rtol) {
  __shared__ long long red[TPB / 64];
  const int b = wg_blk[blockIdx.x];
  if (st[b].done) return;
  const int64_t i = wg_lo[blockIdx.x] + threadIdx.x;
  const double dmax = __longlong_as_double((long long)st[b].dmax_bits);
  const double thr = dmax * (1.0 - tie_rtol);
  long long c = LLONG_MAX;
  if (i < blk_off[b + 1] && d[i] >= thr && d[i] > 0.0) c = i - blk_off[b];
  c = wave_min_ll(c);
  if ((threadIdx.x & 63) == 0) red[threadIdx.x >> 6] = c;
  __syncthreads();
  if (threadIdx.x == 0) {
    for (int w = 1; w < TPB / 64; ++w) c = red[w] < c ? red[w] : c;
    if (c != LLONG_MAX) atomicMin(&st[b].cand, c);
  }
}

__global__ __launch_bounds__(TPB) void take_pivot_kernel(
    const double* __restrict__ ao, int nao, int64_t ld, const double* __restrict__ L, int64_t ldL,
    const double* __restrict__ d, const int64_t* __restrict__ blk_off, const int* __restrict__ nip,
    int j, double tol_in, int kmax, BlkState* __restrict__ st, int64_t* __restrict__ piv,
    double* __restrict__ pv, double* __restrict__ pl, int nh, double* __restrict__ pvr) {
  const int b = blockIdx.x;
  BlkState s = st[b];
  if (s.done) return;
  const double dmax = __longlong_as_double((long long)s.dmax_bits);
  const int64_t m = blk_off[b + 1] - blk_off[b];
  double tol = s.tol;
  if (j == 0) tol = tol_in < 0 ? (double)m * DBL_EPSILON * dmax : tol_in;
  const bool stop = (j >= nip[b]) || !(dmax > tol) || s.cand == LLONG_MAX;
  __syncthreads();
  if (stop) {
    if (threadIdx.x == 0) { st[b].done = 1; st[b].tol = tol; }
    return;
  }
  const int64_t p = blk_off[b] + s.cand;
  for (int mu = threadIdx.x; mu < nao; mu += TPB) pv[(int64_t)b * nao + mu] = ao[(int64_t)mu * ld + p];
  if (nh > 0)
    for (int mu = threadIdx.x; mu < nao; mu += TPB)
      pvr[(int64_t)b * nao + mu] = (mu < nh) ? ao[(int64_t)(nh + mu) * ld + p] : -ao[(int64_t)(mu - nh) * ld + p];
  for (int t = threadIdx.x; t < j; t += TPB) pl[(int64_t)b * kmax + t] = L[(int64_t)t * ldL + p];
  if (threadIdx.x == 0) {
    piv[(int64_t)b * kmax + j] = s.cand;
    st[b].pivot = s.cand;
    st[b].dp = sqrt(d[p]);
    st[b].tol = tol;
    st[b].rank = j + 1;
    st[b].dmax_bits = 0ull;
    st[b].cand = LLONG_MAX;
  }
}

template <bool LDS_PANEL>
__global__ __launch_bounds__(TPB) void update_kernel(
    const double* __restrict__ ao, int nao, int64_t ld, double* __restrict__ L, int64_t ldL,
    double* __restrict__ d, const int* __restrict__ wg_blk, const int64_t* __restrict__ wg_lo,
    const int64_t* __restrict__ blk_off, int j, int kmax, BlkState* __restrict__ st,
    const double* __restrict__ pv, const double* __restrict__ pl, int nh, const double* __restrict__ pvr) {
  extern __shared__ double panel[];
  __shared__ double red[TPB / 64];
  const int b = wg_blk[blockIdx.x];
  if (st[b].done) return;
  const double* s_pv;
  const double* s_pl;
  const double* s_pvr;
  if (LDS_PANEL) {
    double* w_pv = panel;
    double* w_pl = panel + nao;
    double* w_pvr = panel + nao + j;
    for (int mu = threadIdx.x; mu < nao; mu += TPB) w_pv[mu] = pv[(int64_t)b * nao + mu];
    for (int t = threadIdx.x; t < j; t += TPB) w_pl[t] = pl[(int64_t)b * kmax + t];
    if (nh > 0)
      for (int mu = threadIdx.x; mu < nao; mu += TPB) w_pvr[mu] = pvr[(int64_t)b * nao + mu];
    __syncthreads();
    s_pv = w_pv; s_pl = w_pl; s_pvr = w_pvr;
  } else {
    s_pv = pv + (int64_t)b * nao;
    s_pl = pl + (int64_t)b * kmax;
    s_pvr = pvr + (int64_t)b * nao;
  }
  const int64_t i = wg_lo[blockIdx.x] + threadIdx.x;
  const bool valid = i < blk_off[b + 1];
  double dnew = 0.0;
  if (valid) {
    const double dp = st[b].dp;
    const int64_t ploc = blk_off[b] + st[b].pivot;
    const double dold = d[i];
    double row;
    if (i == ploc) {
      row = dp;
      dnew = -1.0;
    } else if (dold < 0.0) {
      row = 0.0;
      dnew = -1.0;
    } else {
      const double* __restrict__ pa = ao + i;
      double s0 = 0.0, s1 = 0.0;
      if (nh > 0) {
#pragma unroll 8
        for (int mu = 0; mu < nao; ++mu) {
          const double x = pa[(int64_t)mu * ld];
          s0 = fma(x, s_pv[mu], s0);
          s1 = fma(x, s_pvr[mu], s1);
        }
      } else {
#pragma unroll 8
        for (int mu = 0; mu < nao; ++mu) s0 = fma(pa[(int64_t)mu * ld], s_pv[mu], s0);
      }
      double col = fma(s1, s1, s0 * s0);
      const double* __restrict__ pL = L + i;
#pragma unroll 8
      for (int t = 0; t < j; ++t) col = fma(-pL[(int64_t)t * ldL], s_pl[t], col);
      row = col / dp;
      dnew = fma(-row, row, dold);
      if (dnew < 0.0) dnew = 0.0;
    }
    L[(int64_t)j * ldL + i] = row;
    d[i] = dnew;
  }
  double m = wave_max_d(valid ? fmax(dnew, 0.0) : 0.0);
  if ((threadIdx.x & 63) == 0) red[threadIdx.x >> 6] = m;
  __syncthreads();
  if (threadIdx.x == 0) {
    for (int w = 1; w < TPB / 64; ++w) m = fmax(m, red[w]);
    atomicMax(&st[b].dmax_bits, (unsigned long long)__double_as_longlong(m));
  }
}

}

namespace {
__global__ __launch_bounds__(256) void partition_kernel(const double* __restrict__ coords, int64_t G, const double* __restrict__ atoms,
                                                        int natm, const double* __restrict__ shifts, double tie_atol,
                                                        int32_t* __restrict__ owner) {
  extern __shared__ double sm[];
  double* s_at = sm;
  double* s_sh = sm + 3 * natm;
  for (int t = threadIdx.x; t < 3 * natm; t += 256) s_at[t] = atoms[t];
  for (int t = threadIdx.x; t < 81; t += 256) s_sh[t] = shifts[t];
  __syncthreads();
  const int64_t g = (int64_t)blockIdx.x * 256 + threadIdx.x;
  if (g >= G) return;
  const double x = coords[g], y = coords[G + g], z = coords[2 * G + g];
  double dmin = 1e300;
  for (int a = 0; a < natm; ++a) {
    const double ax = x - s_at[3 * a], ay = y - s_at[3 * a + 1], az = z - s_at[3 * a + 2];
    double d2 = 1e300;
    for (int t = 0; t < 27; ++t) {
      const double dx = ax - s_sh[3 * t], dy = ay - s_sh[3 * t + 1], dz = az - s_sh[3 * t + 2];
      d2 = fmin(d2, dx * dx + dy * dy + dz * dz);
    }
    dmin = fmin(dmin, sqrt(d2));
  }
  int own = natm;
  for (int a = 0; a < natm && own == natm; ++a) {
    const double ax = x - s_at[3 * a], ay = y - s_at[3 * a + 1], az = z - s_at[3 * a + 2];
    double d2 = 1e300;
    for (int t = 0; t < 27; ++t) {
      const double dx = ax - s_sh[3 * t], dy = ay - s_sh[3 * t + 1], dz = az - s_sh[3 * t + 2];
      d2 = fmin(d2, dx * dx + dy * dy + dz * dz);
    }
    if (sqrt(d2) <= dmin + tie_atol) own = a;
  }
  owner[g] = own;
}
}

extern "C" int isdf_partition_by_atom(isdf_handle h, const double* d_coords, int64_t ngrids, const double* atom_coords, int natm,
                                      const double a[9], double tie_atol, int32_t* d_owner) {
  if (!h) return ISDF_ERR_ARG;
  ARG_CHECK(h, d_coords && atom_coords && a && d_owner && ngrids > 0 && natm > 0 && natm <= 2000 && tie_atol >= 0.0);
  std::vector<double> host(3 * (size_t)natm + 81);
  for (int i = 0; i < 3 * natm; ++i) host[i] = atom_coords[i];
  int t = 0;
  for (int i = -1; i <= 1; ++i)
    for (int j = -1; j <= 1; ++j)
      for (int k = -1; k <= 1; ++k, ++t)
        for (int c = 0; c < 3; ++c) host[3 * natm + 3 * t + c] = i * a[c] + j * a[3 + c] + k * a[6 + c];
  double* d_tab = (double*)isdf_ws(h, "partition_tab", sizeof(double) * host.size());
  if (!d_tab) return ISDF_ERR_HIP;
  HIP_TRY(h, hipMemcpyAsync(d_tab, host.data(), sizeof(double) * host.size(), hipMemcpyHostToDevice, h->stream));
  HIP_TRY(h, hipStreamSynchronize(h->stream));
  ProfScope ps(h, "partition_kernel[byte]", 28.0 * (double)ngrids);
  hipLaunchKernelGGL(partition_kernel, dim3((unsigned)cdiv(ngrids, 256)), dim3(256), sizeof(double) * host.size(), h->stream,
                     d_coords, ngrids, d_tab, natm, d_tab + 3 * natm, tie_atol, d_owner);
  KERNEL_CHECK(h);
  return ISDF_OK;
}

extern "C" int isdf_select_ip(isdf_handle h, const double* d_ao, int nao, int64_t ld, int nblk,
                              const int64_t* blk_off, const int32_t* nip, double tol,
                              double tie_rtol, double* d_L, int64_t ldL, int64_t* d_piv,
                              int32_t* rank) {
  return isdf_select_ip_cplx(h, d_ao, nao, 0, ld, nblk, blk_off, nip, tol, tie_rtol, d_L, ldL, d_piv, rank);
}

extern "C" int isdf_select_ip_cplx(isdf_handle h, const double* d_ao, int nao, int nh, int64_t ld, int nblk,
                                   const int64_t* blk_off, const int32_t* nip, double tol,
                                   double tie_rtol, double* d_L, int64_t ldL, int64_t* d_piv,
                                   int32_t* rank) {
  if (!h) return ISDF_ERR_ARG;
  ARG_CHECK(h, nh == 0 || 2 * nh == nao);
  ARG_CHECK(h, d_ao && blk_off && nip && d_L && d_piv && rank);
  ARG_CHECK(h, nao > 0 && nblk > 0 && tie_rtol >= 0.0 && tie_rtol < 1.0);
  const int64_t mtot = blk_off[nblk];
  ARG_CHECK(h, blk_off[0] == 0 && mtot > 0 && ld >= mtot && ldL >= mtot);
  int kmax = 0;
  std::vector<int> h_wg_blk;
  std::vector<int64_t> h_wg_lo;
  for (int b = 0; b < nblk; ++b) {
    ARG_CHECK(h, blk_off[b + 1] >= blk_off[b] && nip[b] >= 0);
    if (nip[b] > kmax) kmax = nip[b];
    for (int64_t lo = blk_off[b]; lo < blk_off[b + 1]; lo += TPB) {
      h_wg_blk.push_back(b);
      h_wg_lo.push_back(lo);
    }
  }
  ARG_CHECK(h, kmax > 0);
  const size_t panel_bytes = sizeof(double) * ((size_t)nao * (nh > 0 ? 2 : 1) + kmax);
  const bool lds_panel = panel_bytes <= 64 * 1024;
  const int nwg = (int)h_wg_blk.size();

  auto al = [](size_t x) { return (x + 255) / 256 * 256; };
  const size_t b_d = al(sizeof(double) * mtot), b_st = al(sizeof(BlkState) * nblk);
  const size_t b_wb = al(sizeof(int) * nwg), b_wl = al(sizeof(int64_t) * nwg);
  const size_t b_off = al(sizeof(int64_t) * (nblk + 1)), b_nip = al(sizeof(int) * nblk);
  const size_t b_pv = al(sizeof(double) * (size_t)nblk * nao) * 2, b_pl = al(sizeof(double) * (size_t)nblk * kmax);
  char* ws = (char*)isdf_ws(h, "select", b_d + b_st + b_wb + b_wl + b_off + b_nip + b_pv + b_pl);
  if (!ws) return ISDF_ERR_HIP;
  double* d_d = (double*)ws; ws += b_d;
  BlkState* d_st = (BlkState*)ws; ws += b_st;
  int* d_wg_blk = (int*)ws; ws += b_wb;
  int64_t* d_wg_lo = (int64_t*)ws; ws += b_wl;
  int64_t* d_off = (int64_t*)ws; ws += b_off;
  int* d_nip = (int*)ws; ws += b_nip;
  double* d_pv = (double*)ws; ws += b_pv;
  double* d_pvr = d_pv + (size_t)nblk * nao;
  double* d_pl = (double*)ws;

  std::vector<BlkState> h_st(nblk);
  for (auto& s : h_st) { s.dmax_bits = 0; s.cand = LLONG_MAX; s.dp = 0; s.tol = 0; s.pivot = -1; s.done = 0; s.rank = 0; }
  HIP_TRY(h, hipMemcpyAsync(d_st, h_st.data(), sizeof(BlkState) * nblk, hipMemcpyHostToDevice, h->stream));
  HIP_TRY(h, hipMemcpyAsync(d_wg_blk, h_wg_blk.data(), sizeof(int) * nwg, hipMemcpyHostToDevice, h->stream));
  HIP_TRY(h, hipMemcpyAsync(d_wg_lo, h_wg_lo.data(), sizeof(int64_t) * nwg, hipMemcpyHostToDevice, h->stream));
  HIP_TRY(h, hipMemcpyAsync(d_off, blk_off, sizeof(int64_t) * (nblk + 1), hipMemcpyHostToDevice, h->stream));
  HIP_TRY(h, hipMemcpyAsync(d_nip, nip, sizeof(int) * nblk, hipMemcpyHostToDevice, h->stream));
  HIP_TRY(h, hipMemsetAsync(d_piv, 0xff, sizeof(int64_t) * (size_t)nblk * kmax, h->stream));
  HIP_TRY(h, hipStreamSynchronize(h->stream));

  hipLaunchKernelGGL(init_diag_kernel, dim3(nwg), dim3(TPB), 0, h->stream, d_ao, nao, ld, d_wg_blk,
                     d_wg_lo, d_off, d_d, d_st);
  KERNEL_CHECK(h);
  for (int j = 0; j <= kmax; ++j) {
    hipLaunchKernelGGL(find_first_kernel, dim3(nwg), dim3(TPB), 0, h->stream, d_d, d_wg_blk, d_wg_lo,
                       d_off, d_st, tie_rtol);
    hipLaunchKernelGGL(take_pivot_kernel, dim3(nblk), dim3(TPB), 0, h->stream, d_ao, nao, ld, d_L, ldL,
                       d_d, d_off, d_nip, j, tol, kmax, d_st, d_piv, d_pv, d_pl, nh, d_pvr);
    if (j == kmax) break;
    ProfScope ps(h, "select_update_kernel[byte]", 8.0 * (double)mtot * (nao + j + 3));
    if (lds_panel)
      hipLaunchKernelGGL(update_kernel<true>, dim3(nwg), dim3(TPB), sizeof(double) * ((size_t)nao * (nh > 0 ? 2 : 1) + j),
                         h->stream, d_ao, nao, ld, d_L, ldL, d_d, d_wg_blk, d_wg_lo, d_off, j, kmax, d_st, d_pv, d_pl, nh, d_pvr);
    else
      hipLaunchKernelGGL(update_kernel<false>, dim3(nwg), dim3(TPB), 0, h->stream, d_ao, nao, ld, d_L, ldL, d_d,
                         d_wg_blk, d_wg_lo, d_off, j, kmax, d_st, d_pv, d_pl, nh, d_pvr);
  }
  KERNEL_CHECK(h);
  HIP_TRY(h, hipMemcpyAsync(h_st.data(), d_st, sizeof(BlkState) * nblk, hipMemcpyDeviceToHost, h->stream));
  HIP_TRY(h, hipStreamSynchronize(h->stream));
  for (int b = 0; b < nblk; ++b) rank[b] = h_st[b].rank;
  return ISDF_OK;
}
```

pyscf_isdf_amd/isdf.py:

```python
import os
import sys
import time
import warnings
import numpy as np
import torch
from . import gto
from ._common import (UniformGrids, partition_grid_by_atom, _monkhorst_pack_size, _aoslice_by_atom,
                      _default_fft_batch)
from .fit_route import FitRouteMixin
from .sharded import ShardedMixin
from .kpoints import KPointMixin
from .hcore import HcoreMixin
from .eri_surface import EriSurfaceMixin


class ISDF(FitRouteMixin, ShardedMixin, KPointMixin, HcoreMixin, EriSurfaceMixin):
    _keys = {'cell', 'kpts', 'grids', 'mesh', 'blockdim', 'exxdiv', 'c_isdf', 'select', 'tie_rtol'}

    def __init__(self, cell, kpts=np.zeros((1, 3)), c_isdf=12, select='refined', backend=None, comm=None):
        self.cell = cell
        self.stdout = getattr(cell, 'stdout', None) or sys.stdout
        self.verbose = getattr(cell, 'verbose', 0)
        self.max_memory = getattr(cell, 'max_memory', 4000)
        self.kpts_symm = None
        if hasattr(kpts, 'kpts_ibz') and hasattr(kpts, 'transform_dm'):
            self.kpts_symm = kpts
            kpts = kpts.kpts
        self.kpts = np.asarray(kpts).reshape(-1, 3)
        self.grids = UniformGrids(cell, cell.mesh)
        self.blockdim = 240
        self.exxdiv = None
        self.c_isdf = c_isdf
        self.select = select
        self.refine_over = 2.0
        self.pair_space = 'ao'
        self.occ_refit = 'always'
        self.w_spectral = True
        self.w_sphere = 'auto'
        self.w_sphere_tol = 1e-11
        self.w_sort_bins = 256
        self.w_spectral_check_tol = 5e-9
        self.w_spectral_max_c = 18
        self.cand_skip_zero_rows = True
        self.cand_ao_cutoff = None
        self.tie_rtol = 1e-10
        self.select_tol = -1.0
        self.reg_rel = 1e-12
        self.reg_used = 0.0
        self.k_ip_factor = None
        self.kpt_pair_q = 'auto'
        self.kpts_band = None
        self.force_sharded = False
        self.fit_route = 'auto'
        self.bj_check_tol = 3e-8
        self.bj_auto_kpts = False
        self.bj_max_c = 12
        self.bj_nprobe = 8
        self.bj_cluster_radius = 2.4
        self.bj_group = 1
        self.bj_check = None
        self.fit_route_used = None
        self.block_shift = 0.0
        self.block_shift_used = 0.0
        self.robust_k = False
        self.explicit_theta = False
        self.fft_batch = None
        self.block_apply_mfma = True
        self.max_resident_rows = None
        self.max_device_memory = None
        self.n_panels = 1
        self._backend = backend
        self._comm = comm
        self._rsh_df = {}
        self._built = False
        self._W_omega = {}
        self._fit_state = None
        self._fit_pending = False
        self._psi = self._psiP = None
        self._fit_dm = None
        self._V = None
        self._bufs = {}
        self._ovlp = None
        self.timings = {}
        self.ao = None
        self.aoP = None
        self.W = None
        self.ip = None

    @property
    def _want_theta(self):
        return bool(self.explicit_theta or self.robust_k)

    @property
    def _sharded(self):
        return self.comm.size > 1 or self.force_sharded or getattr(self.comm, 'always', False)

    @property
    def mesh(self):
        return self.grids.mesh

    @mesh.setter
    def mesh(self, mesh):
        self.grids.mesh = np.asarray(mesh)
        self.grids._coords = None

    @property
    def backend(self):
        if self._backend is None:
            from .backend import HipBackend
            dev = 0
            if self._comm is not None:
                dev = self._comm.local_rank
            if os.environ.get('ISDF_ONE_GPU'):
                dev = 0
            self._backend = HipBackend(dev)
        return self._backend

    def reset(self, cell=None):
        if cell is not None:
            self.cell = cell
        self.grids = UniformGrids(self.cell, self.cell.mesh)
        self._drop_build_state()
        self._bufs = {}
        self._rows_plan = (None,)
        if self._backend is not None:
            self._backend.empty_cache()
        self._rsh_df = {}
        return self

    def release_fit_buffers(self):
        ao = self.ao
        self._drop_build_state()
        self.ao = ao
        for name in ('theta', 'rows_scratch', 'W', 'factor', 'Dblk', 'Dinv', 'aoP', 'psi', 'psiP'):
            self._bufs.pop(name, None)
        self._Dinv = None
        self._Dinv_key = None
        if self._backend is not None:
            self._backend.release_workspace()
            self._backend.empty_cache()
        return self

    def _drop_build_state(self):
        self.ao = self.aoP = self.W = self.ip = None
        self._fit_state = None
        self._fit_pending = False
        self._psi = self._psiP = None
        self._fit_dm = None
        self._sel = None
        self._Dinv = None
        self._Dinv_key = None
        self._kfit_state = None
        self._ksel = None
        self._V = None
        self._Wq = None
        self._aoP_k = None
        self._W_omega = {}
        self._k_built = None
        self._band_built = None
        self._ovlp = None
        self._built = False
        self._build_serial = getattr(self, '_build_serial', 0) + 1

    def dump_flags(self, verbose=None):
        out = self.stdout
        out.write('\n******** %s ********\n' % self.__class__)
        out.write('mesh = %s (%d PWs)\n' % (self.mesh, np.prod(self.mesh)))
        out.write('c_isdf = %s  select = %s  pair_space = %s  tie_rtol = %g\n' % (self.c_isdf, self.select, self.pair_space, self.tie_rtol))
        out.write('len(kpts) = %d\n' % len(self.kpts))
        return self

    def check_sanity(self):
        if getattr(self.cell, 'dimension', 3) != 3:
            raise RuntimeError('ISDF is implemented for 3-D periodic cells only')
        return self

    @staticmethod
    def _is_gamma(kpts):
        return kpts is None or abs(np.asarray(kpts)).sum() < 1e-9

    def get_naoaux(self):
        return 0 if self.ip is None else len(self.ip)

    def update_mf(self, mf):
        mf = mf.copy() if hasattr(mf, 'copy') else mf
        mf.with_df = self
        return mf

    def _buffer(self, name, shape, dtype=torch.float64):
        n = int(np.prod(shape))
        buf = self._bufs.get(name)
        if buf is None or buf.numel() < n or buf.dtype != dtype:
            self._bufs.pop(name, None)
            buf = None
            self.backend.empty_cache()
            buf = self.backend.empty((n,), dtype=dtype)
            self._bufs[name] = buf
        return buf[:n].view(*shape)


    def _tick(self, name, t0):
        self.backend.synchronize()
        t1 = time.perf_counter()
        self.timings[name] = self.timings.get(name, 0.0) + (t1 - t0)
        return t1

    def nip_per_atom(self):
        aosl = _aoslice_by_atom(self.cell)
        return (np.asarray(aosl[:, 1] - aosl[:, 0]) * self.c_isdf).astype(np.int32)

    @property
    def comm(self):
        if self._comm is None:
            from .parallel import Comm
            self._comm = Comm()
        return self._comm

    def collocate(self):
        cell, be = self.cell, self.backend
        self._drop_build_state()
        G = int(np.prod(self.mesh))
        rcut = gto.estimate_rcut_per_shell(cell)
        Ls = gto.get_lattice_Ls(cell, rcut=rcut.max())
        self.ao = self._buffer('ao', (cell.nao_nr(), G))
        be.eval_ao(np.asarray(cell._atm), np.asarray(cell._bas), np.asarray(cell._env), Ls, rcut,
                   be.to_device(np.ascontiguousarray(self.grids.coords.T)), self.ao)
        return self

    def build(self):
        self.check_sanity()
        self._drop_build_state()
        if not self._is_gamma(self.kpts) or not self._is_gamma(self.kpts_band):
            return self._build_kpts()
        if self._sharded:
            return self._build_sharded()
        cell, be = self.cell, self.backend
        self.timings = {}
        t0 = time.perf_counter()
        mesh = np.asarray(self.mesh, dtype=np.int32)
        G = int(np.prod(mesh))
        nao = cell.nao_nr()
        a = np.asarray(cell.lattice_vectors(), dtype=float)
        coords = self.grids.coords
        rcut = gto.estimate_rcut_per_shell(cell)
        Ls = gto.get_lattice_Ls(cell, rcut=rcut.max())
        self._ao_args = (np.asarray(cell._atm), np.asarray(cell._bas), np.asarray(cell._env), Ls, rcut)
        t0 = self._tick('host_setup', t0)

        coords_soa = be.to_device(np.ascontiguousarray(coords.T))
        self.ao = self._buffer('ao', (nao, G))
        be.eval_ao(*self._ao_args, coords_soa, self.ao)
        del coords_soa
        t0 = self._tick('S1_eval_ao', t0)

        if self.pair_space not in ('ao', 'occ'):
            raise ValueError("pair_space must be 'ao' or 'occ'")
        if self.select == 'global':
            if self.pair_space == 'occ':
                raise NotImplementedError("pair_space='occ' is implemented for select='local' and 'refined'")
            P = int(min(self.c_isdf * nao, G))
            theta = self._buffer('theta', (P, G))
            piv = be.empty((1, P), dtype=torch.int64)
            rank = be.select_ip(self.ao, [0, G], [P], self.select_tol, self.tie_rtol, theta, piv)
            P = int(rank[0])
            t0 = self._tick('S2_select_ip', t0)
            theta = theta[:P]
            piv = piv[0, :P].contiguous()
            if self._want_theta:
                be.fit_from_chol(theta, P, G, piv)
                factor = None
            else:
                factor = (self._buffer('factor', (P, P)), 1)
                be.gather_T(theta, P, piv, factor[0])
            self.ip = be.to_host(piv).astype(np.int64)
            self.aoP = self._buffer('aoP', (P, nao))
            tmp = be.empty((nao, P))
            be.gather_cols(self.ao, piv, tmp)
            self.aoP.copy_(tmp.T)
            del tmp
            t0 = self._tick('S3_fit', t0)
        elif self.select in ('local', 'refined'):
            self._select_candidates(t0)
            if self.pair_space == 'occ':
                self._fit_pending = True
                self._built = True
                return self
            self._pick_and_fit()
            return self
        else:
            raise ValueError("select must be 'local', 'refined' or 'global'")

        self.W = self._buffer('W', (P, P))
        self._fit_state = dict(kind='explicit', theta=theta) if factor is None else \
            dict(kind='selection', theta=theta, T=factor[0])
        self._finish_W(self.W)
        self.fit_route_used = 'selection-cholesky'
        del theta
        t0 = self._tick('S4S5_coulomb_W', t0)
        self._keep_V_for_robust_k(t0)
        self._built = True
        return self

    def _select_candidates(self, t0):
        cell, be = self.cell, self.backend
        nao, G = self.ao.shape
        a = np.asarray(cell.lattice_vectors(), dtype=float)
        owner = be.partition_by_atom(self.grids.coords, cell.atom_coords(), a)
        perm = np.argsort(owner, kind='stable').astype(np.int64)
        counts = np.bincount(owner, minlength=cell.natm)
        blk_off = np.append(0, np.cumsum(counts)).astype(np.int64)
        nip_final = np.minimum(self.nip_per_atom(), counts).astype(np.int32)
        nip = nip_final
        if self.select == 'refined':
            nip = np.minimum(np.ceil(self.nip_per_atom() * float(self.refine_over)).astype(np.int64), counts).astype(np.int32)
        kmax = int(nip.max())
        t0 = self._tick('host_partition', t0)
        d_perm = be.to_device(perm)
        Pmax = int(nip_final.sum())
        key = (Pmax, G, nao, self.max_resident_rows, self.fft_batch, self.pair_space, self.max_device_memory)
        if getattr(self, '_rows_plan', (None,))[0] != key:
            self._rows_plan = (key,) + self._resident_rows(G, Pmax)
        rows_single, rows_panel = self._rows_plan[1:]
        paneled = Pmax > rows_single and not self._want_theta and self.fit_route != 'cholesky'
        rows_buf = max(min(Pmax, rows_panel) if paneled else Pmax, 2 * nao + kmax)
        spectral = None
        routes = self._fit_routes()
        if self.w_spectral and not self._want_theta and (routes[0] == 'blockjacobi' or (paneled and 'cholesky' != self.fit_route)) \
                and not self._sharded and not self.max_resident_rows and self.c_isdf <= self.w_spectral_max_c:
            plan = self._spectral_plan()
            if plan is not None and -(-Pmax * plan['ldx'] // G) <= rows_panel:
                spectral = dict(ldx=plan['ldx'], fraction=plan['fraction'])
                paneled = False
                rows_buf = max(-(-Pmax * plan['ldx'] // G), 2 * nao + kmax)
        scratch = self._buffer('theta', (rows_buf, G))
        ao_sel = scratch[:nao]
        L = scratch[nao:nao + kmax]
        be.gather_cols(self.ao, d_perm, ao_sel)
        if self.select == 'refined' and self.cand_ao_cutoff:
            ao_sel = self._local_ao_rows(ao_sel, scratch[nao + kmax:], blk_off, a)
        elif self.cand_skip_zero_rows:
            ao_sel = self._nonzero_ao_rows(ao_sel, scratch[nao + kmax:], blk_off)
        piv = be.empty((cell.natm, kmax), dtype=torch.int64)
        rank = be.select_ip(ao_sel, blk_off, nip, self.select_tol, self.tie_rtol, L, piv)
        del ao_sel, L, scratch
        piv_h = be.to_host(piv)
        self._tick('S2_select_candidates' if self.select == 'refined' else 'S2_select_ip', t0)
        self._sel = dict(owner=owner, perm=perm, blk_off=blk_off, nip_final=nip_final, piv_h=piv_h, rank=rank, paneled=paneled,
                         rows_buf=rows_buf, rows_panel=rows_panel, spectral=spectral, rows_single=rows_single)

    def _pick_and_fit(self, orbitals=None):
        cell, be, sel = self.cell, self.backend, self._sel
        nao, G = self.ao.shape
        t0 = time.perf_counter()
        perm, blk_off, piv_h, rank, owner = sel['perm'], sel['blk_off'], sel['piv_h'], sel['rank'], sel['owner']
        paneled, rows_buf, rows_panel = sel['paneled'], sel['rows_buf'], sel['rows_panel']
        self._fit_state = None
        self._W_omega = {}
        self._V = None
        self._psi = self._psiP = None
        if orbitals is not None:
            nocc = orbitals.shape[1]
            self._psi = self._buffer('psi', (nocc, G))
            be.gemm_nn(be.to_device(np.ascontiguousarray(orbitals.T)), self.ao, self._psi)
            t0 = self._tick('S2_occupied_on_grid', t0)
        clusters = self._bj_clusters()
        if self.select == 'refined':
            rank = self._refine_selection(perm, blk_off, piv_h, rank, int(sel['nip_final'].sum()), owner)
            ip = np.concatenate([self._refined_by_atom[b] for cl in clusters for b in cl])
        else:
            ip = np.concatenate([perm[blk_off[b] + piv_h[b, :rank[b]]] for cl in clusters for b in cl])
        self.ip = ip.astype(np.int64)
        P = len(ip)
        t0 = self._tick('S2_select_ip', t0)
        self.aoP = self._buffer('aoP', (P, nao))
        d_ip = be.to_device(self.ip)
        if self._psi is not None:
            self._psiP = self._buffer('psiP', (P, self._psi.shape[0]))
            be.gather_aoP(self._psi, d_ip, self._psiP)
        self.W = self._buffer('W', (P, P))
        self.w_spectral_fraction = None
        if sel.get('spectral') is not None:
            if self._build_spectral(rank, clusters, d_ip, t0):
                self._built = True
                return self
            t0 = time.perf_counter()
            rows_single, rows_panel = sel['rows_single'], sel['rows_panel']
            paneled = P > rows_single
            rows_buf = max(min(P, rows_panel) if paneled else P, 1)
        if paneled:
            self._build_paneled(rank, clusters, d_ip, rows_buf, rows_panel, t0)
            self._built = True
            return self
        theta = self._buffer('theta', (rows_buf, G))[:P]
        for route in self._fit_routes():
            if route == 'blockjacobi':
                ip_off = self._bj_blocks(rank, clusters)
                Afac, Dblk = self._bj_prepare(self.ao, 0, d_ip, ip_off, self.aoP, scratch=self.W)
                self._bj_rows(self.aoP, 0, self.ao, G, Dblk, ip_off, theta)
            else:
                chol = self._buffer('factor', (P, P))
                self._chol_fit(d_ip, chol, theta, forward_only=not self._want_theta)
            t0 = self._tick('S3_fit', t0)
            if route == 'blockjacobi':
                self._fit_state = dict(kind='blockjacobi', theta=theta, Afac=Afac, Dblk=Dblk, ip_off=ip_off)
            else:
                self._fit_state = dict(kind='explicit' if self._want_theta else 'cholesky', theta=theta, chol=chol)
            self._finish_W(self.W)
            t0 = self._tick('S4S5_coulomb_W', t0)
            self.fit_route_used = route
            if route == 'blockjacobi' and self.fit_route == 'auto':
                aoT = be.empty((nao, P))
                be.gather_cols(self.ao, d_ip, aoT)
                self.bj_check = self._bj_probe_mismatch(aoT, Afac, Dblk, ip_off, theta, G, None)
                del aoT
                t0 = self._tick('S5_route_check', t0)
                if self.bj_check <= self.bj_check_tol:
                    break
                warnings.warn('ISDF: block-Jacobi fit route failed its probe check (mismatch %.2e > %.2e); '
                              'rebuilding W with the Cholesky route' % (self.bj_check, self.bj_check_tol))
        self._keep_V_for_robust_k(t0)
        del theta
        self._built = True
        return self

    def _chol_fit(self, d_ip, chol, theta, forward_only):
        be = self.backend
        G = self.ao.shape[1]
        if self._psi is None:
            self.reg_used = be.fit_prepare(self.ao, d_ip, self.reg_rel, self.aoP, chol)
            be.fit_apply(chol, self.aoP, self.ao, G, theta, forward_only=forward_only)
            return
        be.gather_aoP(self.ao, d_ip, self.aoP)
        be.gram_prod(self.aoP, self._psiP, chol)
        be.shift_diag(chol, self.reg_rel)
        self.reg_used = self.reg_rel + be.chol_inplace(chol, 0.0, scratch=self.W)
        be.pair_prod_rows(self.aoP, self._psiP, self.ao, self._psi, G, theta)
        be.factor_solve_half(chol, False, theta)
        if not forward_only:
            be.factor_solve_half(chol, True, theta)

    def _occupied_orbitals(self, dm):
        nao = self.cell.nao_nr()
        mo_coeff, mo_occ = getattr(dm, 'mo_coeff', None), getattr(dm, 'mo_occ', None)
        cols = []
        if mo_coeff is not None and mo_occ is not None:
            mo_coeff, mo_occ = np.asarray(mo_coeff), np.asarray(mo_occ)
            if np.iscomplexobj(mo_coeff) and abs(mo_coeff.imag).max() > 1e-12:
                return None
            mo_coeff = mo_coeff.real.reshape(-1, nao, mo_coeff.shape[-1])
            mo_occ = np.asarray(mo_occ, dtype=float).reshape(len(mo_coeff), -1)
            for c, occ in zip(mo_coeff, mo_occ):
                cols.append(c[:, occ > 0] * np.sqrt(occ[occ > 0]))
        else:
            dms = np.asarray(dm)
            if np.iscomplexobj(dms):
                if abs(dms.imag).max() > 1e-12:
                    return None
                dms = dms.real
            for d in dms.reshape(-1, nao, nao):
                if abs(d - d.T).max() > 1e-10 * max(abs(d).max(), 1e-300):
                    return None
                ev, u = np.linalg.eigh(0.5 * (d + d.T))
                if ev.min() < -1e-10 * abs(ev).max():
                    return None
                keep = ev > 1e-12 * ev.max()
                cols.append(u[:, keep] * np.sqrt(ev[keep]))
        c = np.ascontiguousarray(np.hstack(cols), dtype=np.float64)
        if c.shape[1] == 0 or c.shape[1] > nao // 2:
            return None
        return c

    def _ensure_fit(self, dm=None):
        if self.pair_space != 'occ' or self._sel is None or self.ao is None:
            return
        orb = None if dm is None else self._occupied_orbitals(dm)
        want = None if orb is None else orb.dot(orb.T)
        if not self._fit_pending:
            have = self._fit_dm
            if want is None:
                if have is None:
                    return
            elif have is None:
                if self.occ_refit == 'once':
                    return
            elif self.occ_refit == 'once' or abs(want - have).max() <= 1e-12 * abs(want).max():
                return
        self._fit_dm = want
        if self._sel.get('sharded'):
            self._pick_and_fit_sharded(orb)
        else:
            self._pick_and_fit(orb)
        self._fit_pending = False

    def _build_spectral(self, rank, clusters, d_ip, t0):
        be = self.backend
        P = len(self.ip)
        nao, G = self.ao.shape
        ip_off = self._bj_blocks(rank, clusters)
        Afac, Dblk = self._bj_prepare(self.ao, 0, d_ip, ip_off, self.aoP, scratch=self.W)
        self._fit_state = dict(kind='blockjacobi-spectral', Afac=Afac, Dblk=Dblk, ip_off=ip_off)
        t0 = self._tick('S3_fit', t0)
        probe = None
        if self.fit_route == 'auto':
            aoT = be.empty((nao, P))
            be.gather_cols(self.ao, d_ip, aoT)
            T0, E = self._bj_probe_vectors(aoT, Afac, Dblk, ip_off)
            del aoT
            probe = (E, be.empty((E.shape[0], G)))
        self._finish_W_spectral(self.W, probe=probe)
        t0 = self._tick('S4S5_coulomb_W', t0)
        self.fit_route_used = 'blockjacobi'
        self.n_panels = 1
        if probe is None:
            return True
        self.bj_check = self._bj_probe_energies(T0, probe[1], self.W, None)
        self._tick('S5_route_check', t0)
        tol = min(self.bj_check_tol, self.w_spectral_check_tol)
        if self.bj_check <= tol:
            return True
        warnings.warn('ISDF: block-Jacobi fit route failed its probe check (mismatch %.2e > %.2e) in the spectral build; '
                      'rebuilding W the classic way' % (self.bj_check, tol))
        self.w_spectral_fraction = None
        return False

    def _build_paneled(self, rank, clusters, d_ip, rows_buf, rows_panel, t0):
        be = self.backend
        P = len(self.ip)
        nao, G = self.ao.shape
        group0 = int(self.bj_group)
        try:
            for attempt in range(2):
                ip_off = self._bj_blocks(rank, clusters)
                Afac, Dblk = self._bj_prepare(self.ao, 0, d_ip, ip_off, self.aoP, scratch=self.W)
                panels = self._panel_plan(ip_off, min(rows_panel, rows_buf))
                rows = self._buffer('theta', (rows_buf, G))
                self._fit_state = dict(kind='blockjacobi-paneled', rows=rows, panels=panels, Afac=Afac, Dblk=Dblk, ip_off=ip_off)
                t0 = self._tick('S3_fit', t0)
                probe = None
                if self.fit_route == 'auto':
                    aoT = be.empty((nao, P))
                    be.gather_cols(self.ao, d_ip, aoT)
                    T0, E = self._bj_probe_vectors(aoT, Afac, Dblk, ip_off)
                    del aoT
                    probe = (E, be.empty((E.shape[0], G)))
                self._finish_W_paneled(self.W, probe=probe)
                t0 = self._tick('S4S5_coulomb_W', t0)
                self.fit_route_used = 'blockjacobi'
                self.n_panels = len(panels)
                if probe is None:
                    return
                self.bj_check = self._bj_probe_energies(T0, probe[1], self.W, None)
                t0 = self._tick('S5_route_check', t0)
                if self.bj_check <= self.bj_check_tol:
                    return
                if attempt == 0:
                    warnings.warn('ISDF: block-Jacobi fit route failed its probe check (mismatch %.2e > %.2e) in a paneled build, where '
                                  'the Cholesky route is not available: rebuilding with pairs of clusters merged into one '
                                  'preconditioner block' % (self.bj_check, self.bj_check_tol))
                    self.bj_group = 2 * group0
            raise RuntimeError('ISDF: the paneled block-Jacobi build failed its probe check twice (mismatch %.2e > bj_check_tol = '
                               '%.2e): W would carry rounding noise of that relative size.  Use fewer points (c_isdf), more GPUs '
                               '(the rows then fit and the Cholesky route is available), or raise bj_check_tol knowingly.'
                               % (self.bj_check, self.bj_check_tol))
        finally:
            self.bj_group = group0

    def _local_ao_rows(self, ao_sel, out_rows, blk_off, a):
        cell = self.cell
        aosl = _aoslice_by_atom(cell)
        frac = np.asarray(cell.atom_coords(), dtype=float).dot(np.linalg.inv(a))
        d = frac[:, None, :] - frac[None, :, :]
        d -= np.round(d)
        near = np.linalg.norm(d.dot(a), axis=2) < float(self.cand_ao_cutoff)
        lists = [np.concatenate([np.arange(aosl[c, 0], aosl[c, 1]) for c in np.nonzero(near[b])[0]]) for b in range(cell.natm)]
        nloc = max(len(x) for x in lists)
        loc = out_rows[:nloc]
        loc.zero_()
        for b, rows in enumerate(lists):
            s0, s1 = int(blk_off[b]), int(blk_off[b + 1])
            if s1 > s0:
                loc[:len(rows), s0:s1] = ao_sel[self.backend.to_device(rows.astype(np.int64)), s0:s1]
        return loc

    def _nonzero_ao_rows(self, ao_sel, out_rows, blk_off):
        be = self.backend
        natm = len(blk_off) - 1
        mx = be.block_row_absmax(ao_sel, blk_off)
        lists = [np.nonzero(mx[:, b] > 0.0)[0] for b in range(natm)]
        nloc = max([len(x) for x in lists] + [1])
        self._cand_rows_kept = (nloc, ao_sel.shape[0])
        if nloc > 0.95 * ao_sel.shape[0]:
            return ao_sel
        loc = out_rows[:nloc]
        loc.zero_()
        for b, rows in enumerate(lists):
            s0, s1 = int(blk_off[b]), int(blk_off[b + 1])
            if s1 > s0 and len(rows):
                loc[:len(rows), s0:s1] = ao_sel[be.to_device(rows.astype(np.int64)), s0:s1]
        return loc

    def _refine_selection(self, perm, blk_off, piv_h, rank, P_target, owner):
        be = self.backend
        natm = self.cell.natm
        cand = np.concatenate([perm[blk_off[b] + piv_h[b, :rank[b]]] for b in range(natm)]).astype(np.int64)
        aoC = be.empty((len(cand), self.ao.shape[0]))
        d_cand = be.to_device(cand)
        be.gather_aoP(self.ao, d_cand, aoC)
        psiC = None
        if self._psi is not None:
            psiC = be.empty((len(cand), self._psi.shape[0]))
            be.gather_aoP(self._psi, d_cand, psiC)
        rows_buf = self._bufs.get('theta')
        gram = None if rows_buf is None or rows_buf.numel() < len(cand) ** 2 else rows_buf[:len(cand) ** 2].view(len(cand), len(cand))
        chosen = self._refine_pick(aoC, cand, P_target, gram=gram, psiC=psiC)
        del aoC, gram, psiC
        own = owner[chosen]
        self._refined_by_atom = [chosen[own == b] for b in range(natm)]
        return np.array([len(x) for x in self._refined_by_atom], dtype=np.int32)

    def _refine_pick(self, aoC, cand, P_target, gram=None, nh=0, psiC=None):
        be = self.backend
        m = len(cand)
        P_target = min(int(P_target), m)
        A = be.empty((m, m)) if gram is None else gram
        if psiC is not None and nh:
            be.gram_prod_cplx(aoC, nh, psiC, psiC.shape[1] // 2, A)
        elif psiC is not None:
            be.gram_prod(aoC, psiC, A)
        else:
            be.gram_sq(aoC, A, nh)
        piv2 = be.empty((P_target,), dtype=torch.int64)
        r2 = be.select_ip_gram(A, P_target, self.select_tol, self.tie_rtol, piv2)
        chosen = np.asarray(cand)[be.to_host(piv2)[:r2]]
        del A, piv2
        return chosen

    def _keep_V_for_robust_k(self, t0):
        if not self.robust_k:
            return
        be = self.backend
        theta = self._fit_state['theta']
        mesh = np.asarray(self.mesh, dtype=np.int32)
        a = np.asarray(self.cell.lattice_vectors(), dtype=float)
        be.coulomb_rows(theta, mesh, a, self._last_fft_batch)
        self._V = theta
        self._fit_state = None
# ... 339 lines not shown
```

pyscf_isdf_amd/lib.py:

```python
import ctypes
import os

_HERE = os.path.dirname(os.path.abspath(__file__))
LIB_PATH = os.path.join(_HERE, 'lib', 'libmi355_isdf.so')
ABI_VERSION = 21

_lib = None

c_int, c_i64, c_dbl, c_vp = ctypes.c_int, ctypes.c_int64, ctypes.c_double, ctypes.c_void_p

SIGNATURES = {
    'isdf_abi_version': (c_int, []),
    'isdf_create': (c_int, [c_int, ctypes.POINTER(c_vp)]),
    'isdf_destroy': (c_int, [c_vp]),
    'isdf_set_stream': (c_int, [c_vp, c_vp]),
    'isdf_last_error': (ctypes.c_char_p, [c_vp]),
    'isdf_workspace_bytes': (c_i64, [c_vp]),
    'isdf_set_coulomb_omega': (c_int, [c_vp, c_dbl]),
    'isdf_set_coulomb_cutoff': (c_int, [c_vp, c_dbl]),
    'isdf_set_coulomb_ws': (c_int, [c_vp, c_dbl, c_vp, c_vp, c_vp, c_vp]),
    'isdf_set_option': (c_int, [c_vp, ctypes.c_char_p, c_int]),
    'isdf_release_workspace': (c_int, [c_vp]),
    'isdf_prof_enable': (c_int, [c_vp, c_int]),
    'isdf_prof_reset': (c_int, [c_vp]),
    'isdf_prof_count': (c_int, [c_vp]),
    'isdf_prof_get': (c_int, [c_vp, c_int, ctypes.c_char_p, c_int, ctypes.POINTER(c_i64), ctypes.POINTER(c_dbl), ctypes.POINTER(c_dbl)]),
    'isdf_eval_ao': (c_int, [c_vp, c_vp, c_int, c_vp, c_int, c_vp, c_int, c_vp, c_int, c_vp, c_vp, c_i64, c_vp, c_i64]),
    'isdf_block_row_absmax': (c_int, [c_vp, c_vp, c_int, c_i64, c_int, c_vp, c_vp]),
    'isdf_gather_cols': (c_int, [c_vp, c_vp, c_int, c_i64, c_vp, c_i64, c_vp, c_i64]),
    'isdf_partition_by_atom': (c_int, [c_vp, c_vp, c_i64, c_vp, c_int, c_vp, c_dbl, c_vp]),
    'isdf_select_ip': (c_int, [c_vp, c_vp, c_int, c_i64, c_int, c_vp, c_vp, c_dbl, c_dbl, c_vp, c_i64, c_vp, c_vp]),
    'isdf_select_ip_gram': (c_int, [c_vp, c_vp, c_int, c_i64, c_int, c_dbl, c_dbl, c_int, c_vp, ctypes.POINTER(ctypes.c_int32)]),
    'isdf_fit_from_chol': (c_int, [c_vp, c_vp, c_int, c_i64, c_i64, c_vp]),
    'isdf_fit_prepare': (c_int, [c_vp, c_vp, c_int, c_i64, c_vp, c_int, c_dbl, c_vp, c_vp, ctypes.POINTER(c_dbl)]),
    'isdf_fit_apply': (c_int, [c_vp, c_vp, c_vp, c_int, c_int, c_vp, c_i64, c_i64, c_int, c_vp, c_i64]),
    'isdf_gather_aoP': (c_int, [c_vp, c_vp, c_int, c_i64, c_vp, c_int, c_vp]),
    'isdf_gram_sq': (c_int, [c_vp, c_vp, c_int, c_int, c_int, c_vp]),
    'isdf_pair_gram_rows': (c_int, [c_vp, c_vp, c_int, c_int, c_int, c_vp, c_i64, c_i64, c_vp, c_i64]),
    'isdf_gram_prod': (c_int, [c_vp, c_vp, c_int, c_int, c_vp, c_int, c_vp]),
    'isdf_pair_prod_rows': (c_int, [c_vp, c_vp, c_int, c_int, c_vp, c_int, c_vp, c_i64, c_vp, c_i64, c_i64, c_vp, c_i64]),
    'isdf_factor_solve_half': (c_int, [c_vp, c_vp, c_int, c_int, c_vp, c_i64, c_i64]),
    'isdf_gram_prod_cplx': (c_int, [c_vp, c_vp, c_int, c_int, c_int, c_vp, c_int, c_int, c_vp]),
    'isdf_pair_prod_rows_cplx': (c_int, [c_vp, c_vp, c_int, c_int, c_int, c_vp, c_int, c_int, c_vp, c_i64, c_vp, c_i64, c_i64,
                                         c_vp, c_i64]),
    'isdf_block_chol': (c_int, [c_vp, c_vp, c_int, c_int, c_vp, c_dbl, c_vp, ctypes.POINTER(c_dbl)]),
    'isdf_block_solve': (c_int, [c_vp, c_vp, c_int, c_int, c_vp, c_int, c_int, c_vp, c_i64, c_i64]),
    'isdf_block_invert': (c_int, [c_vp, c_vp, c_int, c_int, c_vp, c_vp]),
    'isdf_block_apply': (c_int, [c_vp, c_vp, c_i64, c_int, c_vp, c_vp, c_i64, c_i64]),
    'isdf_pair_rows_block_apply': (c_int, [c_vp, c_vp, c_int, c_int, c_vp, c_i64, c_i64, c_vp, c_i64, c_int, c_vp, c_vp, c_i64]),
    'isdf_shift_diag': (c_int, [c_vp, c_vp, c_int, c_dbl]),
    'isdf_chol_inplace': (c_int, [c_vp, c_vp, c_int, c_dbl, c_vp, ctypes.POINTER(c_dbl)]),
    'isdf_factor_solve': (c_int, [c_vp, c_vp, c_int, c_vp, c_i64, c_i64]),
    'isdf_bj_probe_vectors': (c_int, [c_vp, c_vp, c_int, c_vp, c_vp, c_int, c_int, c_vp]),
    'isdf_rows_combine': (c_int, [c_vp, c_vp, c_int, c_i64, c_int, c_vp, c_i64, c_i64, c_vp, c_i64, c_int]),
    'isdf_bj_probe_rows': (c_int, [c_vp, c_vp, c_int, c_vp, c_vp, c_int, c_int, c_vp, c_vp, c_i64, c_i64, c_vp, c_i64]),
    'isdf_gather_T': (c_int, [c_vp, c_vp, c_int, c_i64, c_vp, c_vp]),
    'isdf_W_from_factor': (c_int, [c_vp, c_vp, c_int, c_int, c_vp, c_i64]),
    'isdf_fit_global': (c_int, [c_vp, c_vp, c_int, c_i64, c_i64, c_vp, c_int, c_dbl, c_vp, c_i64, c_vp, ctypes.POINTER(c_dbl)]),
    'isdf_coulomb_W': (c_int, [c_vp, c_vp, c_int, c_i64, c_vp, c_vp, c_int, c_int, c_int, c_int, c_vp, c_i64]),
    'isdf_coulomb_rows': (c_int, [c_vp, c_vp, c_int, c_i64, c_vp, c_vp, c_int, c_vp, c_i64]),
    'isdf_symmetrize_upper': (c_int, [c_vp, c_vp, c_int, c_i64]),
    'isdf_symmetrize_mean': (c_int, [c_vp, c_vp, c_int, c_i64, c_int]),
    'isdf_get_j': (c_int, [c_vp, c_vp, c_int, c_i64, c_i64, c_vp, c_vp, c_vp, c_int, c_vp]),
    'isdf_rho': (c_int, [c_vp, c_vp, c_int, c_i64, c_i64, c_vp, c_int, c_vp, c_i64]),
    'isdf_coulomb_potential': (c_int, [c_vp, c_vp, c_int, c_i64, c_vp, c_vp]),
    'isdf_vj_from_vR': (c_int, [c_vp, c_vp, c_int, c_i64, c_i64, c_vp, c_int, c_i64, c_vp]),
    'isdf_eval_ao_k': (c_int, [c_vp, c_vp, c_int, c_vp, c_int, c_vp, c_int, c_vp, c_int, c_vp, c_vp, c_int, c_vp, c_i64, c_vp, c_vp, c_i64]),
    'isdf_select_ip_cplx': (c_int, [c_vp, c_vp, c_int, c_int, c_i64, c_int, c_vp, c_vp, c_dbl, c_dbl, c_vp, c_i64, c_vp, c_vp]),
    'isdf_fit_prepare_cplx': (c_int, [c_vp, c_vp, c_int, c_int, c_i64, c_vp, c_int, c_dbl, c_vp, c_vp, ctypes.POINTER(c_dbl)]),
    'isdf_fit_apply_cplx': (c_int, [c_vp, c_vp, c_vp, c_int, c_int, c_int, c_vp, c_i64, c_i64, c_int, c_vp, c_i64]),
    'isdf_coulG_q': (c_int, [c_vp, c_vp, c_vp, c_vp, c_int, c_dbl, c_vp]),
    'isdf_coulomb_Wq': (c_int, [c_vp, c_vp, c_int, c_i64, c_vp, c_vp, c_dbl, c_int, c_int, c_int, c_int, c_vp, c_vp, c_i64]),
    'isdf_symmetrize_hermitian': (c_int, [c_vp, c_vp, c_vp, c_int, c_i64]),
    'isdf_finish_Wq': (c_int, [c_vp, c_vp, c_vp, c_int, c_i64, c_vp, c_vp]),
    'isdf_get_k_pair': (c_int, [c_vp, c_vp, c_vp, c_vp, c_vp, c_int, c_int, c_dbl, c_vp]),
    'isdf_get_k_exact_kpt': (c_int, [c_vp, c_vp, c_vp, c_int, c_i64, c_vp, c_vp, c_int, c_i64, c_vp, c_vp, c_dbl, c_int, c_int, c_int, c_vp, c_vp]),
    'isdf_coulG_half': (c_int, [c_vp, c_vp, c_vp, c_vp]),
    'isdf_spectral_supported': (c_int, [c_vp, c_vp, c_int, ctypes.POINTER(c_int)]),
    'isdf_spectral_rows': (c_int, [c_vp, c_vp, c_int, c_i64, c_vp, c_vp, c_vp, c_int, c_int, c_vp, c_i64]),
    'isdf_coulomb_rows_q': (c_int, [c_vp, c_vp, c_int, c_i64, c_vp, c_vp, c_vp, c_vp]),
    'isdf_nyquist_spectra': (c_int, [c_vp, c_vp, c_int, c_i64, c_vp, c_int, c_vp, c_vp]),
    'isdf_zhadamard_planes': (c_int, [c_vp, c_vp, c_vp, c_i64, c_vp, c_vp, c_i64, c_int, c_i64]),
    'isdf_rho_k': (c_int, [c_vp, c_vp, c_vp, c_int, c_i64, c_i64, c_vp, c_vp, c_dbl, c_vp]),
    'isdf_vj_k': (c_int, [c_vp, c_vp, c_vp, c_int, c_i64, c_i64, c_vp, c_vp, c_vp]),
    'isdf_pp_local_potential': (c_int, [c_vp, c_int, c_vp, c_vp, c_vp, c_vp, c_vp]),
    'isdf_pp_projector_overlaps': (c_int, [c_vp, c_vp, c_int, c_vp, c_int, c_vp, c_int, c_vp, c_vp, c_vp, c_vp, c_int, c_vp, c_vp, c_vp]),
    'isdf_gemm_nn': (c_int, [c_vp, c_int, c_i64, c_int, c_dbl, c_vp, c_i64, c_vp, c_i64, c_dbl, c_vp, c_i64]),
    'isdf_hadamard_rows': (c_int, [c_vp, c_vp, c_i64, c_vp, c_i64, c_int, c_i64]),
    'isdf_eval_ao_deriv1': (c_int, [c_vp, c_vp, c_int, c_vp, c_int, c_vp, c_int, c_vp, c_int, c_vp, c_vp, c_i64, c_vp, c_i64, c_i64]),
    'isdf_eval_ao_k_deriv1': (c_int, [c_vp, c_vp, c_int, c_vp, c_int, c_vp, c_int, c_vp, c_int, c_vp, c_vp, c_int, c_vp, c_i64, c_vp, c_vp, c_i64, c_i64]),
    'isdf_uniform_grid': (c_int, [c_vp, c_vp, c_vp, c_vp]),
    'isdf_rho_pair': (c_int, [c_vp, c_vp, c_int, c_vp, c_int, c_i64, c_i64, c_vp, c_int, c_vp, c_i64]),
    'isdf_mg_embed_density': (c_int, [c_vp, c_vp, c_int, c_vp, c_dbl, c_vp, c_vp, c_int]),
    'isdf_mg_restrict_potential': (c_int, [c_vp, c_vp, c_int, c_vp, c_vp, c_dbl, c_vp]),
    'isdf_mg_coulomb_kernel': (c_int, [c_vp, c_vp, c_int, c_vp, c_vp]),
    'isdf_lda_exchange': (c_int, [c_vp, c_vp, c_i64, c_vp, c_vp]),
    'isdf_lda_vwn_add': (c_int, [c_vp, c_vp, c_i64, c_vp, c_vp]),
    'isdf_gga_b88': (c_int, [c_vp, c_vp, c_vp, c_i64, c_i64, c_vp, c_vp, c_vp, c_i64]),
    'isdf_xc_fused': (c_int, [c_vp, c_vp, c_vp, c_i64, c_i64, c_dbl, c_dbl, c_dbl, c_int, c_dbl, c_vp, c_vp, c_vp, c_i64]),
    'isdf_gga_lyp_polarised': (c_int, [c_vp, c_vp, c_vp, c_i64, c_i64, c_i64, c_dbl, c_int, c_vp, c_vp, c_vp, c_i64, c_i64]),
    'isdf_lda_exchange_fxc': (c_int, [c_vp, c_vp, c_i64, c_vp]),
    'isdf_lda_vwn_fxc_add': (c_int, [c_vp, c_vp, c_i64, c_vp]),
    'isdf_gga_b88_fxc': (c_int, [c_vp, c_vp, c_i64, c_i64, c_vp, c_i64, c_i64, c_int, c_vp, c_i64, c_i64, c_vp, c_i64]),
    'isdf_xc_fxc_apply': (c_int, [c_vp, c_int, c_vp, c_i64, c_i64, c_i64, c_vp, c_i64, c_i64, c_int, c_vp, c_i64, c_i64, c_int]),
    'isdf_dot': (c_int, [c_vp, c_vp, c_vp, c_i64, c_vp]),
    'isdf_gemm_nt': (c_int, [c_vp, c_int, c_int, c_i64, c_dbl, c_vp, c_i64, c_vp, c_i64, c_vp, c_dbl, c_vp, c_i64]),
    'isdf_get_k_exact': (c_int, [c_vp, c_vp, c_int, c_i64, c_i64, c_vp, c_int, c_vp, c_vp, c_int, c_int, c_int, c_vp]),
    'isdf_get_k': (c_int, [c_vp, c_vp, c_int, c_int, c_vp, c_i64, c_int, c_int, c_vp, c_int, c_vp]),
}


def load():
    global _lib
    if _lib is not None:
        return _lib
    if not os.path.exists(LIB_PATH):
        raise RuntimeError(
            'libmi355_isdf.so not found at %s — build it with `python -c "import __graft_entry__ as g; '
            'g.build()"` or `make -C pyscf_isdf_amd/csrc`.  There is no CPU fallback.' % LIB_PATH)
    try:
        import torch
    except ImportError:
        pass
    lib = ctypes.CDLL(LIB_PATH, mode=ctypes.RTLD_GLOBAL)
    for name, (res, args) in SIGNATURES.items():
        fn = getattr(lib, name)
        fn.restype = res
        fn.argtypes = args
    v = lib.isdf_abi_version()
    if v != ABI_VERSION:
        raise RuntimeError('libmi355_isdf.so ABI version %d != binding version %d' % (v, ABI_VERSION))
    _lib = lib
    return lib


class IsdfError(RuntimeError):
    pass


class Handle:

    def __init__(self, device=0):
        self.lib = load()
        h = c_vp()
        rc = self.lib.isdf_create(int(device), ctypes.byref(h))
        if rc != 0 or not h.value:
            raise IsdfError('isdf_create(device=%d) failed with status %d (no MI355X visible?)' % (device, rc))
        self.h = h
        self.device = device

    def call(self, name, *args):
        rc = getattr(self.lib, name)(self.h, *args)
        if rc != 0:
            msg = self.lib.isdf_last_error(self.h)
            raise IsdfError('%s failed (status %d): %s' % (name, rc, msg.decode() if msg else ''))

    def close(self):
        if getattr(self, 'h', None) is not None and self.h.value:
            self.lib.isdf_destroy(self.h)
            self.h = c_vp()

    def __del__(self):
        try:
            self.close()
        except Exception:
            pass
```

Baseline: 18.11.

## Precompute per-atom candidate Gram matrices with MFMA for pivoted Cholesky selection

```diff
diff --git a/include/mi355_isdf.h b/include/mi355_isdf.h
--- a/include/mi355_isdf.h
+++ b/include/mi355_isdf.h
@@ -70,6 +70,13 @@
                    int nblk, const int64_t* blk_off, const int32_t* nip,
                    double tol, double tie_rtol,
                    double* d_L, int64_t ldL, int64_t* d_piv, int32_t* rank);
+
+int isdf_select_ip_ws(isdf_handle h, const double* d_ao, int nao, int64_t ld,
+                      int nblk, const int64_t* blk_off, const int32_t* nip,
+                      double tol, double tie_rtol,
+                      double* d_L, int64_t ldL, int64_t* d_piv, int32_t* rank,
+                      void* d_work, int64_t work_bytes);
+int64_t isdf_select_ip_work_bytes(int nao, int64_t m);
 
 int isdf_select_ip_gram(isdf_handle h, double* d_A, int m, int64_t ldA, int nip, double tol, double tie_rtol,
                         int panel, int64_t* d_piv, int32_t* rank);
diff --git a/pyscf_isdf_amd/backend.py b/pyscf_isdf_amd/backend.py
--- a/pyscf_isdf_amd/backend.py
+++ b/pyscf_isdf_amd/backend.py
@@ -190,14 +190,19 @@
                          self._p(owner))
         return self.to_host(owner)
 
-    def select_ip(self, ao, blk_off, nip, tol, tie_rtol, L, piv):
+    def select_ip_work_bytes(self, nao, m):
+        return int(self.handle.lib.isdf_select_ip_work_bytes(int(nao), int(m)))
+
+    def select_ip(self, ao, blk_off, nip, tol, tie_rtol, L, piv, work=None):
         self._stream()
         blk_off = np.ascontiguousarray(blk_off, dtype=np.int64)
         nip = np.ascontiguousarray(nip, dtype=np.int32)
         rank = np.zeros(len(nip), dtype=np.int32)
         assert piv.dtype == torch.int64 and piv.is_contiguous() and ao.stride(1) == 1 and L.stride(1) == 1
-        self.handle.call('isdf_select_ip', self._p(ao), ao.shape[0], ao.stride(0), len(nip), _np_ptr(blk_off),
-                         _np_ptr(nip), float(tol), float(tie_rtol), self._p(L), L.stride(0), self._p(piv), _np_ptr(rank))
+        assert work is None or work.is_contiguous()
+        self.handle.call('isdf_select_ip_ws', self._p(ao), ao.shape[0], ao.stride(0), len(nip), _np_ptr(blk_off),
+                         _np_ptr(nip), float(tol), float(tie_rtol), self._p(L), L.stride(0), self._p(piv), _np_ptr(rank),
+                         None if work is None else self._p(work), 0 if work is None else work.numel() * work.element_size())
         return rank
 
     def select_ip_gram(self, A, nip, tol, tie_rtol, piv, panel=0):
diff --git a/pyscf_isdf_amd/csrc/common.h b/pyscf_isdf_amd/csrc/common.h
--- a/pyscf_isdf_amd/csrc/common.h
+++ b/pyscf_isdf_amd/csrc/common.h
@@ -47,7 +47,8 @@
   int trsm_substitution = 0;
   int own_fft = 2;
   int gemm_nn_own = 0;
-  int attr_gemm_b = 0, attr_gemm_nn = 0;
+  int attr_gemm_b = 0, attr_gemm_nn = 0, attr_gram_tri = 0;
+  int cand_gram = 1;
   int conv_pipe = 1;
   int conv_sub_rows = 0;
   int gram_pivot_tpb = 256;
@@ -145,3 +146,12 @@
 int gemm_rm(isdf_handle h, char opA, char opB, int64_t M, int64_t N, int64_t K, double alpha,
             const double* A, int64_t lda, const double* B, int64_t ldb, double beta, double* C,
             int64_t ldc);
+
+__host__ __device__ inline int64_t gram_tri_row(int64_t r) {
+  const int64_t tm = r >> 8;
+  return 32768 * tm * (tm + 1) + (r & 255) * ((tm + 1) << 8);
+}
+static inline int64_t gram_tri_size(int64_t m) { return m > 0 ? gram_tri_row(m - 1) + (((m - 1) >> 8) + 1) * 256 : 0; }
+struct GramTriUnit { int blk, tm, tn, pad; };
+int gram_tri_blocks(isdf_handle h, const double* X, int64_t ldx, int K, const GramTriUnit* d_units, int64_t nunits,
+                    const int64_t* d_blk_off, int64_t row0, const int64_t* d_tri_off, double* S, double flop);
diff --git a/pyscf_isdf_amd/csrc/gemm_f64.hip b/pyscf_isdf_amd/csrc/gemm_f64.hip
--- a/pyscf_isdf_amd/csrc/gemm_f64.hip
+++ b/pyscf_isdf_amd/csrc/gemm_f64.hip
@@ -168,138 +168,42 @@
   const int tm = (int)(unit % g.ntm);
   const int tn = (int)((unit / g.ntm) % g.ntn);
   const int slab = (int)(unit / ((int64_t)g.ntm * g.ntn));
-  const int64_t k0 = (int64_t)slab * g.kslab;
-  const int64_t k1 = (k0 + g.kslab < g.K) ? k0 + g.kslab : g.K;
-  const int nchunks = (int)((k1 - k0) / BK);
-  const int last = nchunks - 1;
-
-  const int tid = threadIdx.x;
-  const int lane = tid & 63, wave = tid >> 6;
-  const int wm = wave >> 1, wn = wave & 1;
-  const int srow = tid >> 3;
-  const int sseg = tid & 7;
-  const int mlast = g.M - 1, nlast = g.N - 1;
-  const double* pA0 = g.A + (int64_t)min(tm * BM2 + srow, mlast) * g.lda + k0 + sseg * 2;
-  const double* pA1 = g.A + (int64_t)min(tm * BM2 + srow + 64, mlast) * g.lda + k0 + sseg * 2;
-  const double* pA2 = g.A + (int64_t)min(tm * BM2 + srow + 128, mlast) * g.lda + k0 + sseg * 2;
-  const double* pA3 = g.A + (int64_t)min(tm * BM2 + srow + 192, mlast) * g.lda + k0 + sseg * 2;
-  const double* pB0 = g.B + (int64_t)min(tn * BN + srow, nlast) * g.ldb + k0 + sseg * 2;
-  const double* pB1 = g.B + (int64_t)min(tn * BN + srow + 64, nlast) * g.ldb + k0 + sseg * 2;
-  const double* pS = SCALED ? g.kscale + k0 + sseg * 2 : nullptr;
-
-  double2 xa0, xa1, xa2, xa3, xb0, xb1, ya0, ya1, ya2, ya3, yb0, yb1;
-#define ISDF_LOADB(C, A0, A1, A2, A3, B0, B1)                                                 \
-  {                                                                                           \
-    const int off = (C) * BK;                                                                 \
-    A0 = *reinterpret_cast<const double2*>(pA0 + off);                                        \
-    A1 = *reinterpret_cast<const double2*>(pA1 + off);                                        \
-    A2 = *reinterpret_cast<const double2*>(pA2 + off);                                        \
-    A3 = *reinterpret_cast<const double2*>(pA3 + off);                                        \
-    B0 = *reinterpret_cast<const double2*>(pB0 + off);                                        \
-    B1 = *reinterpret_cast<const double2*>(pB1 + off);                                        \
-    if (SCALED) {                                                                             \
-      const double2 sc = *reinterpret_cast<const double2*>(pS + off);                         \
-      B0.x *= sc.x; B0.y *= sc.y; B1.x *= sc.x; B1.y *= sc.y;                                 \
-    }                                                                                         \
-  }
-#define ISDF_ST1(P, R) { double* q_ = (P); q_[0] = R.x; q_[1] = R.y; }
-#define ISDF_STOREB(BUF, A0, A1, A2, A3, B0, B1)                                              \
-  {                                                                                           \
-    double* qa = sA + (BUF) * BM2 * LDT + srow * LDT + sseg * 2;                              \
-    double* qb = sB + (BUF) * BN * LDT + srow * LDT + sseg * 2;                               \
-    ISDF_ST1(qa, A0) ISDF_ST1(qa + 64 * LDT, A1) ISDF_ST1(qa + 128 * LDT, A2)                 \
-    ISDF_ST1(qa + 192 * LDT, A3) ISDF_ST1(qb, B0) ISDF_ST1(qb + 64 * LDT, B1)                 \
-  }
-
-  d4 acc[4][4];
-#pragma unroll
-  for (int i = 0; i < 4; ++i)
-#pragma unroll
-    for (int j = 0; j < 4; ++j) acc[i][j] = (d4){0.0, 0.0, 0.0, 0.0};
-  const int frow = lane & 15, fk = lane >> 4;
-
-#define ISDF_FRAGB(KK, AF, BF)                                                                \
-    _Pragma("unroll") for (int i = 0; i < 4; ++i) {                                           \
-      AF[i] = pa[i * 16 * LDT + (KK) * 4];                                                    \
-      BF[i] = pb[i * 16 * LDT + (KK) * 4];                                                    \
-    }
-#define ISDF_MFMAB(AF, BF)                                                                    \
-    _Pragma("unroll") for (int i = 0; i < 4; ++i)                                             \
-      _Pragma("unroll") for (int j = 0; j < 4; ++j)                                           \
-        acc[i][j] = __builtin_amdgcn_mfma_f64_16x16x4f64(AF[i], BF[j], acc[i][j], 0, 0, 0);
-#define ISDF_INTERLEAVE() _Pragma("unroll") for (int q_ = 0; q_ < 8; ++q_) {                  \
-    __builtin_amdgcn_sched_group_barrier(0x008, 2, 0); __builtin_amdgcn_sched_group_barrier(0x100, 1, 0); }
-#define ISDF_INTERLEAVE_W() _Pragma("unroll") for (int q_ = 0; q_ < 6; ++q_) {                \
-    __builtin_amdgcn_sched_group_barrier(0x008, 2, 0); __builtin_amdgcn_sched_group_barrier(0x200, 1, 0); }
-#define ISDF_INTERLEAVE_L() _Pragma("unroll") for (int q_ = 0; q_ < 8; ++q_) {                \
-    __builtin_amdgcn_sched_group_barrier(0x008, 2, 0); __builtin_amdgcn_sched_group_barrier(0x100, 1, 0);                \
-    if (q_ < 6) __builtin_amdgcn_sched_group_barrier(0x020, 1, 0); }
-  const int aoff = (wm * 64 + frow) * LDT + fk, boff = (wn * 64 + frow) * LDT + fk;
-  double a0[4], b0[4], a1[4], b1[4];
-#define ISDF_FRAGQ(BUF, KK, AF, BF)                                                           \
-  {                                                                                           \
-    const double* pa = sA + (BUF) * BM2 * LDT + aoff;                                         \
-    const double* pb = sB + (BUF) * BN * LDT + boff;                                          \
-    _Pragma("unroll") for (int i = 0; i < 4; ++i) {                                           \
-      AF[i] = pa[i * 16 * LDT + (KK) * 4];                                                    \
-      BF[i] = pb[i * 16 * LDT + (KK) * 4];                                                    \
-    }                                                                                         \
-  }
-#define ISDF_INTERLEAVE_RW() _Pragma("unroll") for (int q_ = 0; q_ < 8; ++q_) {               \
-    __builtin_amdgcn_sched_group_barrier(0x008, 2, 0); __builtin_amdgcn_sched_group_barrier(0x100, 1, 0);                \
-    if (q_ < 6) __builtin_amdgcn_sched_group_barrier(0x200, 1, 0); }
-#define ISDF_CHUNKB(BUF, LOAD_AHEAD, STORE_NEXT)                                              \
-  {                                                                                           \
-    ISDF_FRAGQ(BUF, 1, a1, b1)                                                                \
-    LOAD_AHEAD                                                                                \
-    ISDF_MFMAB(a0, b0)                                                                        \
-    ISDF_INTERLEAVE_L()                                                                       \
-    __builtin_amdgcn_sched_barrier(0);                                                        \
-    ISDF_FRAGQ(BUF, 2, a0, b0)                                                                \
-    ISDF_MFMAB(a1, b1)                                                                        \
-    ISDF_INTERLEAVE()                                                                         \
-    __builtin_amdgcn_sched_barrier(0);                                                        \
-    ISDF_FRAGQ(BUF, 3, a1, b1)                                                                \
-    STORE_NEXT                                                                                \
-    ISDF_MFMAB(a0, b0)                                                                        \
-    ISDF_INTERLEAVE_RW()                                                                      \
-    __builtin_amdgcn_sched_barrier(0);                                                        \
-    __syncthreads();                                                                          \
-    ISDF_FRAGQ(1 - (BUF), 0, a0, b0)                                                          \
-    ISDF_MFMAB(a1, b1)                                                                        \
-    ISDF_INTERLEAVE()                                                                         \
-    __builtin_amdgcn_sched_barrier(0);                                                        \
-  }
-
-  ISDF_LOADB(0, xa0, xa1, xa2, xa3, xb0, xb1)
-  ISDF_LOADB(1, ya0, ya1, ya2, ya3, yb0, yb1)
-  ISDF_STOREB(0, xa0, xa1, xa2, xa3, xb0, xb1)
-  __syncthreads();
-  ISDF_FRAGQ(0, 0, a0, b0)
-  __builtin_amdgcn_sched_barrier(0);
-  for (int c = 0; c < nchunks; c += 2) {
-    ISDF_CHUNKB(0, ISDF_LOADB(min(c + 2, last), xa0, xa1, xa2, xa3, xb0, xb1), ISDF_STOREB(1, ya0, ya1, ya2, ya3, yb0, yb1))
-    ISDF_CHUNKB(1, ISDF_LOADB(min(c + 3, last), ya0, ya1, ya2, ya3, yb0, yb1), ISDF_STOREB(0, xa0, xa1, xa2, xa3, xb0, xb1))
-  }
-
-  double* out = g.P + (int64_t)slab * g.slab_stride;
-#pragma unroll
-  for (int i = 0; i < 4; ++i) {
-#pragma unroll
-    for (int r = 0; r < 4; ++r) {
-      const int row = tm * BM2 + wm * 64 + i * 16 + (lane >> 4) + 4 * r;
-      if (row >= g.M) continue;
-#pragma unroll
-      for (int j = 0; j < 4; ++j) {
-        const int col = tn * BN + wn * 64 + j * 16 + (lane & 15);
-        if (col >= g.N) continue;
-        double* q = out + (int64_t)row * g.ldp + col;
-        const double v = acc[i][j][r];
-        if (g.direct) *q = (g.beta == 0.0) ? g.alpha * v : g.alpha * v + g.beta * (*q);
-        else *q = v;
-      }
-    }
-  }
+#include "gemm_nt_b_unit.inc"
+}
+
+struct GramTriArgs {
+  const double* X; int64_t ldx; int K;
+  const GramTriUnit* units;
+  const int64_t* blk_off;
+  int64_t row0;
+  const int64_t* tri_off;
+  double* S;
+  int64_t nunits, nunits_pad;
+};
+
+__global__ __launch_bounds__(TPB2, 2) void gram_tri_mfma_kernel(GramTriArgs t) {
+  extern __shared__ double smem[];
+  const int64_t bid = blockIdx.x;
+  const int64_t per_xcd = t.nunits_pad / 8;
+  const int64_t unit = (bid % 8) * per_xcd + bid / 8;
+  if (unit >= t.nunits) return;
+  const GramTriUnit u = t.units[unit];
+  const int64_t r0 = t.blk_off[u.blk];
+  GemmArgs g;
+  g.A = g.B = t.X + (r0 - t.row0) * t.ldx;
+  g.lda = g.ldb = t.ldx;
+  g.kscale = nullptr;
+  g.M = g.N = (int)(t.blk_off[u.blk + 1] - r0);
+  g.K = g.kslab = t.K;
+  g.ldp = (int64_t)(u.tm + 1) * BM2;
+  g.P = t.S + t.tri_off[u.blk] + (gram_tri_row((int64_t)u.tm * BM2) - (int64_t)u.tm * BM2 * g.ldp);
+  g.slab_stride = 0;
+  g.direct = 1; g.alpha = 1.0; g.beta = 0.0;
+  constexpr bool SCALED = false;
+  double* sA = smem;
+  double* sB = smem + 2 * BM2 * LDT;
+  const int tm = u.tm, tn = u.tn, slab = 0;
+#include "gemm_nt_b_unit.inc"
 }
 
 constexpr int TPBD = 256;
@@ -690,6 +594,25 @@
   return gemm_nt_f64_scaled(h, M, N, K, alpha, d_A, lda, d_B, ldb, d_kscale, beta, d_C, ldc);
 }
 
+int gram_tri_blocks(isdf_handle h, const double* X, int64_t ldx, int K, const GramTriUnit* d_units, int64_t nunits,
+                    const int64_t* d_blk_off, int64_t row0, const int64_t* d_tri_off, double* S, double flop) {
+  ARG_CHECK(h, X && d_units && d_blk_off && d_tri_off && S && nunits > 0 && K > 0 && K % 32 == 0 && ldx >= K && ldx % 2 == 0 &&
+                   ((uintptr_t)X) % 16 == 0);
+  GramTriArgs t;
+  t.X = X; t.ldx = ldx; t.K = K; t.units = d_units; t.blk_off = d_blk_off; t.row0 = row0; t.tri_off = d_tri_off; t.S = S;
+  t.nunits = nunits; t.nunits_pad = cdiv(nunits, 8) * 8;
+  ARG_CHECK(h, t.nunits_pad < 2147483647LL);
+  const size_t lds = sizeof(double) * 2 * (BM2 + BN) * LDT;
+  if (!h->attr_gram_tri) {
+    HIP_TRY(h, hipFuncSetAttribute((const void*)gram_tri_mfma_kernel, hipFuncAttributeMaxDynamicSharedMemorySize, (int)lds));
+    h->attr_gram_tri = 1;
+  }
+  ProfScope ps(h, "cand_gram_blocks[flop]", flop);
+  hipLaunchKernelGGL(gram_tri_mfma_kernel, dim3((unsigned)t.nunits_pad), dim3(TPB2), lds, h->stream, t);
+  KERNEL_CHECK(h);
+  return ISDF_OK;
+}
+
 bool gemm_nn_f64_supported(isdf_handle h, int64_t M, int64_t N, int64_t K, const double* A, int64_t lda, const double* B,
                            int64_t ldb) {
   return h->gemm_nn_own && M > BM && (double)(cdiv(M, BM2) * BM2) <= 1.15 * (double)M && N >= 2 && N % 2 == 0 && K >= 32 && K % 32 == 0 &&
diff --git a/pyscf_isdf_amd/csrc/gemm_nt_b_unit.inc b/pyscf_isdf_amd/csrc/gemm_nt_b_unit.inc
--- /dev/null
+++ b/pyscf_isdf_amd/csrc/gemm_nt_b_unit.inc
@@ -0,0 +1,132 @@
+  const int64_t k0 = (int64_t)slab * g.kslab;
+  const int64_t k1 = (k0 + g.kslab < g.K) ? k0 + g.kslab : g.K;
+  const int nchunks = (int)((k1 - k0) / BK);
+  const int last = nchunks - 1;
+
+  const int tid = threadIdx.x;
+  const int lane = tid & 63, wave = tid >> 6;
+  const int wm = wave >> 1, wn = wave & 1;
+  const int srow = tid >> 3;
+  const int sseg = tid & 7;
+  const int mlast = g.M - 1, nlast = g.N - 1;
+  const double* pA0 = g.A + (int64_t)min(tm * BM2 + srow, mlast) * g.lda + k0 + sseg * 2;
+  const double* pA1 = g.A + (int64_t)min(tm * BM2 + srow + 64, mlast) * g.lda + k0 + sseg * 2;
+  const double* pA2 = g.A + (int64_t)min(tm * BM2 + srow + 128, mlast) * g.lda + k0 + sseg * 2;
+  const double* pA3 = g.A + (int64_t)min(tm * BM2 + srow + 192, mlast) * g.lda + k0 + sseg * 2;
+  const double* pB0 = g.B + (int64_t)min(tn * BN + srow, nlast) * g.ldb + k0 + sseg * 2;
+  const double* pB1 = g.B + (int64_t)min(tn * BN + srow + 64, nlast) * g.ldb + k0 + sseg * 2;
+  const double* pS = SCALED ? g.kscale + k0 + sseg * 2 : nullptr;
+
+  double2 xa0, xa1, xa2, xa3, xb0, xb1, ya0, ya1, ya2, ya3, yb0, yb1;
+#define ISDF_LOADB(C, A0, A1, A2, A3, B0, B1)                                                 \
+  {                                                                                           \
+    const int off = (C) * BK;                                                                 \
+    A0 = *reinterpret_cast<const double2*>(pA0 + off);                                        \
+    A1 = *reinterpret_cast<const double2*>(pA1 + off);                                        \
+    A2 = *reinterpret_cast<const double2*>(pA2 + off);                                        \
+    A3 = *reinterpret_cast<const double2*>(pA3 + off);                                        \
+    B0 = *reinterpret_cast<const double2*>(pB0 + off);                                        \
+    B1 = *reinterpret_cast<const double2*>(pB1 + off);                                        \
+    if (SCALED) {                                                                             \
+      const double2 sc = *reinterpret_cast<const double2*>(pS + off);                         \
+      B0.x *= sc.x; B0.y *= sc.y; B1.x *= sc.x; B1.y *= sc.y;                                 \
+    }                                                                                         \
+  }
+#define ISDF_ST1(P, R) { double* q_ = (P); q_[0] = R.x; q_[1] = R.y; }
+#define ISDF_STOREB(BUF, A0, A1, A2, A3, B0, B1)                                              \
+  {                                                                                           \
+    double* qa = sA + (BUF) * BM2 * LDT + srow * LDT + sseg * 2;                              \
+    double* qb = sB + (BUF) * BN * LDT + srow * LDT + sseg * 2;                               \
+    ISDF_ST1(qa, A0) ISDF_ST1(qa + 64 * LDT, A1) ISDF_ST1(qa + 128 * LDT, A2)                 \
+    ISDF_ST1(qa + 192 * LDT, A3) ISDF_ST1(qb, B0) ISDF_ST1(qb + 64 * LDT, B1)                 \
+  }
+
+  d4 acc[4][4];
+#pragma unroll
+  for (int i = 0; i < 4; ++i)
+#pragma unroll
+    for (int j = 0; j < 4; ++j) acc[i][j] = (d4){0.0, 0.0, 0.0, 0.0};
+  const int frow = lane & 15, fk = lane >> 4;
+
+#define ISDF_FRAGB(KK, AF, BF)                                                                \
+    _Pragma("unroll") for (int i = 0; i < 4; ++i) {                                           \
+      AF[i] = pa[i * 16 * LDT + (KK) * 4];                                                    \
+      BF[i] = pb[i * 16 * LDT + (KK) * 4];                                                    \
+    }
+#define ISDF_MFMAB(AF, BF)                                                                    \
+    _Pragma("unroll") for (int i = 0; i < 4; ++i)                                             \
+      _Pragma("unroll") for (int j = 0; j < 4; ++j)                                           \
+        acc[i][j] = __builtin_amdgcn_mfma_f64_16x16x4f64(AF[i], BF[j], acc[i][j], 0, 0, 0);
+#define ISDF_INTERLEAVE() _Pragma("unroll") for (int q_ = 0; q_ < 8; ++q_) {                  \
+    __builtin_amdgcn_sched_group_barrier(0x008, 2, 0); __builtin_amdgcn_sched_group_barrier(0x100, 1, 0); }
+#define ISDF_INTERLEAVE_W() _Pragma("unroll") for (int q_ = 0; q_ < 6; ++q_) {                \
+    __builtin_amdgcn_sched_group_barrier(0x008, 2, 0); __builtin_amdgcn_sched_group_barrier(0x200, 1, 0); }
+#define ISDF_INTERLEAVE_L() _Pragma("unroll") for (int q_ = 0; q_ < 8; ++q_) {                \
+    __builtin_amdgcn_sched_group_barrier(0x008, 2, 0); __builtin_amdgcn_sched_group_barrier(0x100, 1, 0);                \
+    if (q_ < 6) __builtin_amdgcn_sched_group_barrier(0x020, 1, 0); }
+  const int aoff = (wm * 64 + frow) * LDT + fk, boff = (wn * 64 + frow) * LDT + fk;
+  double a0[4], b0[4], a1[4], b1[4];
+#define ISDF_FRAGQ(BUF, KK, AF, BF)                                                           \
+  {                                                                                           \
+    const double* pa = sA + (BUF) * BM2 * LDT + aoff;                                         \
+    const double* pb = sB + (BUF) * BN * LDT + boff;                                          \
+    _Pragma("unroll") for (int i = 0; i < 4; ++i) {                                           \
+      AF[i] = pa[i * 16 * LDT + (KK) * 4];                                                    \
+      BF[i] = pb[i * 16 * LDT + (KK) * 4];                                                    \
+    }                                                                                         \
+  }
+#define ISDF_INTERLEAVE_RW() _Pragma("unroll") for (int q_ = 0; q_ < 8; ++q_) {               \
+    __builtin_amdgcn_sched_group_barrier(0x008, 2, 0); __builtin_amdgcn_sched_group_barrier(0x100, 1, 0);                \
+    if (q_ < 6) __builtin_amdgcn_sched_group_barrier(0x200, 1, 0); }
+#define ISDF_CHUNKB(BUF, LOAD_AHEAD, STORE_NEXT)                                              \
+  {                                                                                           \
+    ISDF_FRAGQ(BUF, 1, a1, b1)                                                                \
+    LOAD_AHEAD                                                                                \
+    ISDF_MFMAB(a0, b0)                                                                        \
+    ISDF_INTERLEAVE_L()                                                                       \
+    __builtin_amdgcn_sched_barrier(0);                                                        \
+    ISDF_FRAGQ(BUF, 2, a0, b0)                                                                \
+    ISDF_MFMAB(a1, b1)                                                                        \
+    ISDF_INTERLEAVE()                                                                         \
+    __builtin_amdgcn_sched_barrier(0);                                                        \
+    ISDF_FRAGQ(BUF, 3, a1, b1)                                                                \
+    STORE_NEXT                                                                                \
+    ISDF_MFMAB(a0, b0)                                                                        \
+    ISDF_INTERLEAVE_RW()                                                                      \
+    __builtin_amdgcn_sched_barrier(0);                                                        \
+    __syncthreads();                                                                          \
+    ISDF_FRAGQ(1 - (BUF), 0, a0, b0)                                                          \
+    ISDF_MFMAB(a1, b1)                                                                        \
+    ISDF_INTERLEAVE()                                                                         \
+    __builtin_amdgcn_sched_barrier(0);                                                        \
+  }
+
+  ISDF_LOADB(0, xa0, xa1, xa2, xa3, xb0, xb1)
+  ISDF_LOADB(1, ya0, ya1, ya2, ya3, yb0, yb1)
+  ISDF_STOREB(0, xa0, xa1, xa2, xa3, xb0, xb1)
+  __syncthreads();
+  ISDF_FRAGQ(0, 0, a0, b0)
+  __builtin_amdgcn_sched_barrier(0);
+  for (int c = 0; c < nchunks; c += 2) {
+    ISDF_CHUNKB(0, ISDF_LOADB(min(c + 2, last), xa0, xa1, xa2, xa3, xb0, xb1), ISDF_STOREB(1, ya0, ya1, ya2, ya3, yb0, yb1))
+    ISDF_CHUNKB(1, ISDF_LOADB(min(c + 3, last), ya0, ya1, ya2, ya3, yb0, yb1), ISDF_STOREB(0, xa0, xa1, xa2, xa3, xb0, xb1))
+  }
+
+  double* out = g.P + (int64_t)slab * g.slab_stride;
+#pragma unroll
+  for (int i = 0; i < 4; ++i) {
+#pragma unroll
+    for (int r = 0; r < 4; ++r) {
+      const int row = tm * BM2 + wm * 64 + i * 16 + (lane >> 4) + 4 * r;
+      if (row >= g.M) continue;
+#pragma unroll
+      for (int j = 0; j < 4; ++j) {
+        const int col = tn * BN + wn * 64 + j * 16 + (lane & 15);
+        if (col >= g.N) continue;
+        double* q = out + (int64_t)row * g.ldp + col;
+        const double v = acc[i][j][r];
+        if (g.direct) *q = (g.beta == 0.0) ? g.alpha * v : g.alpha * v + g.beta * (*q);
+        else *q = v;
+      }
+    }
+  }
diff --git a/pyscf_isdf_amd/csrc/handle.hip b/pyscf_isdf_amd/csrc/handle.hip
--- a/pyscf_isdf_amd/csrc/handle.hip
+++ b/pyscf_isdf_amd/csrc/handle.hip
@@ -103,6 +103,7 @@
     h->gram_pivot_tpb = value;
     return ISDF_OK;
   }
+  if (std::string(key) == "cand_gram") { h->cand_gram = value ? 1 : 0; return ISDF_OK; }
   if (std::string(key) == "gram_compact") { h->gram_compact = value ? 1 : 0; return ISDF_OK; }
   if (std::string(key) == "gram_compact_permille") {
     if (value < 1 || value > 1000) return isdf_fail(h, ISDF_ERR_ARG, "isdf_set_option: gram_compact_permille %d not in [1, 1000]", value);
diff --git a/pyscf_isdf_amd/csrc/select_ip.hip b/pyscf_isdf_amd/csrc/select_ip.hip
--- a/pyscf_isdf_amd/csrc/select_ip.hip
+++ b/pyscf_isdf_amd/csrc/select_ip.hip
@@ -80,8 +80,8 @@
     const double* __restrict__ ao, int nao, int64_t ld, const double* __restrict__ L, int64_t ldL,
     const double* __restrict__ d, const int64_t* __restrict__ blk_off, const int* __restrict__ nip,
     int j, double tol_in, int kmax, BlkState* __restrict__ st, int64_t* __restrict__ piv,
-    double* __restrict__ pv, double* __restrict__ pl, int nh, double* __restrict__ pvr) {
-  const int b = blockIdx.x;
+    double* __restrict__ pv, double* __restrict__ pl, int nh, double* __restrict__ pvr, int b0) {
+  const int b = b0 + blockIdx.x;
   BlkState s = st[b];
   if (s.done) return;
   const double dmax = __longlong_as_double((long long)s.dmax_bits);
@@ -95,7 +95,8 @@
     return;
   }
   const int64_t p = blk_off[b] + s.cand;
-  for (int mu = threadIdx.x; mu < nao; mu += TPB) pv[(int64_t)b * nao + mu] = ao[(int64_t)mu * ld + p];
+  if (ao)
+    for (int mu = threadIdx.x; mu < nao; mu += TPB) pv[(int64_t)b * nao + mu] = ao[(int64_t)mu * ld + p];
   if (nh > 0)
     for (int mu = threadIdx.x; mu < nao; mu += TPB)
       pvr[(int64_t)b * nao + mu] = (mu < nh) ? ao[(int64_t)(nh + mu) * ld + p] : -ao[(int64_t)(mu - nh) * ld + p];
@@ -111,12 +112,13 @@
   }
 }
 
-template <bool LDS_PANEL>
+template <bool LDS_PANEL, bool GRAM>
 __global__ __launch_bounds__(TPB) void update_kernel(
     const double* __restrict__ ao, int nao, int64_t ld, double* __restrict__ L, int64_t ldL,
     double* __restrict__ d, const int* __restrict__ wg_blk, const int64_t* __restrict__ wg_lo,
     const int64_t* __restrict__ blk_off, int j, int kmax, BlkState* __restrict__ st,
-    const double* __restrict__ pv, const double* __restrict__ pl, int nh, const double* __restrict__ pvr) {
+    const double* __restrict__ pv, const double* __restrict__ pl, int nh, const double* __restrict__ pvr,
+    const int64_t* __restrict__ tri_off) {
   extern __shared__ double panel[];
   __shared__ double red[TPB / 64];
   const int b = wg_blk[blockIdx.x];
@@ -126,9 +128,10 @@
   const double* s_pvr;
   if (LDS_PANEL) {
     double* w_pv = panel;
-    double* w_pl = panel + nao;
-    double* w_pvr = panel + nao + j;
-    for (int mu = threadIdx.x; mu < nao; mu += TPB) w_pv[mu] = pv[(int64_t)b * nao + mu];
+    double* w_pl = panel + (GRAM ? 0 : nao);
+    double* w_pvr = w_pl + j;
+    if (!GRAM)
+      for (int mu = threadIdx.x; mu < nao; mu += TPB) w_pv[mu] = pv[(int64_t)b * nao + mu];
     for (int t = threadIdx.x; t < j; t += TPB) w_pl[t] = pl[(int64_t)b * kmax + t];
     if (nh > 0)
       for (int mu = threadIdx.x; mu < nao; mu += TPB) w_pvr[mu] = pvr[(int64_t)b * nao + mu];
@@ -156,7 +159,11 @@
     } else {
       const double* __restrict__ pa = ao + i;
       double s0 = 0.0, s1 = 0.0;
-      if (nh > 0) {
+      if (GRAM) {
+        const int64_t il = i - blk_off[b], pl_ = st[b].pivot;
+        const double* __restrict__ S = ao + tri_off[b];
+        s0 = il < (((pl_ >> 8) + 1) << 8) ? S[gram_tri_row(pl_) + il] : S[gram_tri_row(il) + pl_];
+      } else if (nh > 0) {
 #pragma unroll 8
         for (int mu = 0; mu < nao; ++mu) {
           const double x = pa[(int64_t)mu * ld];
@@ -248,17 +255,15 @@
   return ISDF_OK;
 }
 
-extern "C" int isdf_select_ip(isdf_handle h, const double* d_ao, int nao, int64_t ld, int nblk,
-                              const int64_t* blk_off, const int32_t* nip, double tol,
-                              double tie_rtol, double* d_L, int64_t ldL, int64_t* d_piv,
-                              int32_t* rank) {
-  return isdf_select_ip_cplx(h, d_ao, nao, 0, ld, nblk, blk_off, nip, tol, tie_rtol, d_L, ldL, d_piv, rank);
-}
-
-extern "C" int isdf_select_ip_cplx(isdf_handle h, const double* d_ao, int nao, int nh, int64_t ld, int nblk,
-                                   const int64_t* blk_off, const int32_t* nip, double tol,
-                                   double tie_rtol, double* d_L, int64_t ldL, int64_t* d_piv,
-                                   int32_t* rank) {
+namespace {
+
+int64_t gram_kpad(int nao) { return cdiv(nao, 32) * 32; }
+
+struct BlkGroup { int b0, b1, w0, w1, kmax; int64_t u0, u1; };
+
+int select_blocks(isdf_handle h, const double* d_ao, int nao, int nh, int64_t ld, int nblk,
+                  const int64_t* blk_off, const int32_t* nip, double tol, double tie_rtol, double* d_L,
+                  int64_t ldL, int64_t* d_piv, int32_t* rank, void* d_work, int64_t work_bytes) {
   if (!h) return ISDF_ERR_ARG;
   ARG_CHECK(h, nh == 0 || 2 * nh == nao);
   ARG_CHECK(h, d_ao && blk_off && nip && d_L && d_piv && rank);
@@ -266,27 +271,68 @@
   const int64_t mtot = blk_off[nblk];
   ARG_CHECK(h, blk_off[0] == 0 && mtot > 0 && ld >= mtot && ldL >= mtot);
   int kmax = 0;
-  std::vector<int> h_wg_blk;
+  std::vector<int> h_wg_blk, h_wg_first(nblk + 1);
   std::vector<int64_t> h_wg_lo;
   for (int b = 0; b < nblk; ++b) {
     ARG_CHECK(h, blk_off[b + 1] >= blk_off[b] && nip[b] >= 0);
     if (nip[b] > kmax) kmax = nip[b];
+    h_wg_first[b] = (int)h_wg_blk.size();
     for (int64_t lo = blk_off[b]; lo < blk_off[b + 1]; lo += TPB) {
       h_wg_blk.push_back(b);
       h_wg_lo.push_back(lo);
     }
   }
   ARG_CHECK(h, kmax > 0);
-  const size_t panel_bytes = sizeof(double) * ((size_t)nao * (nh > 0 ? 2 : 1) + kmax);
+  const int nwg = (int)h_wg_blk.size();
+  h_wg_first[nblk] = nwg;
+
+  std::vector<BlkGroup> groups;
+  std::vector<GramTriUnit> h_units;
+  std::vector<int64_t> h_tri_off(nblk, 0);
+  const int kpad = (int)gram_kpad(nao);
+  char* work = (char*)(((uintptr_t)d_work + 255) / 256 * 256);
+  const int64_t avail = d_work ? (work_bytes - (int64_t)(work - (char*)d_work)) / 8 : 0;
+  bool gram = nh == 0 && h->cand_gram && avail > 0;
+  if (gram) {
+    BlkGroup g{0, 0, 0, 0, 0, 0, 0};
+    int64_t used = 0, tri = 0;
+    for (int b = 0; b < nblk && gram; ++b) {
+      const int64_t m = blk_off[b + 1] - blk_off[b];
+      const int64_t need = gram_tri_size(m) + m * kpad;
+      if (need > avail) { gram = false; break; }
+      if (used + need > avail) {
+        g.b1 = b; g.u1 = (int64_t)h_units.size();
+        groups.push_back(g);
+        g = BlkGroup{b, b, 0, 0, 0, g.u1, g.u1};
+        used = tri = 0;
+      }
+      h_tri_off[b] = tri;
+      tri += gram_tri_size(m);
+      used += need;
+      if (nip[b] > g.kmax) g.kmax = nip[b];
+      if (nip[b] > 0)
+        for (int tm = 0; tm < (int)cdiv(m, 256); ++tm)
+          for (int tn = 0; tn <= 2 * tm + 1 && (int64_t)tn * 128 < m; ++tn) h_units.push_back(GramTriUnit{b, tm, tn, 0});
+    }
+    g.b1 = nblk; g.u1 = (int64_t)h_units.size();
+    groups.push_back(g);
+  }
+  if (!gram) {
+    groups.assign(1, BlkGroup{0, nblk, 0, 0, kmax, 0, 0});
+    h_units.clear();
+  }
+  for (auto& g : groups) { g.w0 = h_wg_first[g.b0]; g.w1 = h_wg_first[g.b1]; }
+
+  const size_t panel_bytes = sizeof(double) * (gram ? (size_t)kmax : (size_t)nao * (nh > 0 ? 2 : 1) + kmax);
   const bool lds_panel = panel_bytes <= 64 * 1024;
-  const int nwg = (int)h_wg_blk.size();
 
   auto al = [](size_t x) { return (x + 255) / 256 * 256; };
   const size_t b_d = al(sizeof(double) * mtot), b_st = al(sizeof(BlkState) * nblk);
   const size_t b_wb = al(sizeof(int) * nwg), b_wl = al(sizeof(int64_t) * nwg);
   const size_t b_off = al(sizeof(int64_t) * (nblk + 1)), b_nip = al(sizeof(int) * nblk);
   const size_t b_pv = al(sizeof(double) * (size_t)nblk * nao) * 2, b_pl = al(sizeof(double) * (size_t)nblk * kmax);
-  char* ws = (char*)isdf_ws(h, "select", b_d + b_st + b_wb + b_wl + b_off + b_nip + b_pv + b_pl);
+  const size_t b_tri = al(sizeof(int64_t) * nblk), b_un = al(sizeof(GramTriUnit) * h_units.size());
+  char* ws = (char*)isdf_ws(h, "select", b_d + b_st + b_wb + b_wl + b_off + b_nip + b_pv + b_pl + b_tri + b_un);
   if (!ws) return ISDF_ERR_HIP;
   double* d_d = (double*)ws; ws += b_d;
   BlkState* d_st = (BlkState*)ws; ws += b_st;
@@ -296,7 +342,9 @@
   int* d_nip = (int*)ws; ws += b_nip;
   double* d_pv = (double*)ws; ws += b_pv;
   double* d_pvr = d_pv + (size_t)nblk * nao;
-  double* d_pl = (double*)ws;
+  double* d_pl = (double*)ws; ws += b_pl;
+  int64_t* d_tri_off = (int64_t*)ws; ws += b_tri;
+  GramTriUnit* d_units = (GramTriUnit*)ws;
 
   std::vector<BlkState> h_st(nblk);
   for (auto& s : h_st) { s.dmax_bits = 0; s.cand = LLONG_MAX; s.dp = 0; s.tol = 0; s.pivot = -1; s.done = 0; s.rank = 0; }
@@ -305,29 +353,98 @@
   HIP_TRY(h, hipMemcpyAsync(d_wg_lo, h_wg_lo.data(), sizeof(int64_t) * nwg, hipMemcpyHostToDevice, h->stream));
   HIP_TRY(h, hipMemcpyAsync(d_off, blk_off, sizeof(int64_t) * (nblk + 1), hipMemcpyHostToDevice, h->stream));
   HIP_TRY(h, hipMemcpyAsync(d_nip, nip, sizeof(int) * nblk, hipMemcpyHostToDevice, h->stream));
+  if (gram) {
+    HIP_TRY(h, hipMemcpyAsync(d_tri_off, h_tri_off.data(), sizeof(int64_t) * nblk, hipMemcpyHostToDevice, h->stream));
+    if (!h_units.empty())
+      HIP_TRY(h, hipMemcpyAsync(d_units, h_units.data(), sizeof(GramTriUnit) * h_units.size(), hipMemcpyHostToDevice, h->stream));
+  }
   HIP_TRY(h, hipMemsetAsync(d_piv, 0xff, sizeof(int64_t) * (size_t)nblk * kmax, h->stream));
   HIP_TRY(h, hipStreamSynchronize(h->stream));
 
   hipLaunchKernelGGL(init_diag_kernel, dim3(nwg), dim3(TPB), 0, h->stream, d_ao, nao, ld, d_wg_blk,
                      d_wg_lo, d_off, d_d, d_st);
   KERNEL_CHECK(h);
-  for (int j = 0; j <= kmax; ++j) {
-    hipLaunchKernelGGL(find_first_kernel, dim3(nwg), dim3(TPB), 0, h->stream, d_d, d_wg_blk, d_wg_lo,
-                       d_off, d_st, tie_rtol);
-    hipLaunchKernelGGL(take_pivot_kernel, dim3(nblk), dim3(TPB), 0, h->stream, d_ao, nao, ld, d_L, ldL,
-                       d_d, d_off, d_nip, j, tol, kmax, d_st, d_piv, d_pv, d_pl, nh, d_pvr);
-    if (j == kmax) break;
-    ProfScope ps(h, "select_update_kernel[byte]", 8.0 * (double)mtot * (nao + j + 3));
-    if (lds_panel)
-      hipLaunchKernelGGL(update_kernel<true>, dim3(nwg), dim3(TPB), sizeof(double) * ((size_t)nao * (nh > 0 ? 2 : 1) + j),
-                         h->stream, d_ao, nao, ld, d_L, ldL, d_d, d_wg_blk, d_wg_lo, d_off, j, kmax, d_st, d_pv, d_pl, nh, d_pvr);
-    else
-      hipLaunchKernelGGL(update_kernel<false>, dim3(nwg), dim3(TPB), 0, h->stream, d_ao, nao, ld, d_L, ldL, d_d,
-                         d_wg_blk, d_wg_lo, d_off, j, kmax, d_st, d_pv, d_pl, nh, d_pvr);
-  }
-  KERNEL_CHECK(h);
+  for (const BlkGroup& g : groups) {
+    const int gwg = g.w1 - g.w0, gblk = g.b1 - g.b0;
+    const int64_t p0 = blk_off[g.b0], mg = blk_off[g.b1] - p0;
+    if (gwg == 0) continue;
+    const double* d_S = nullptr;
+    if (gram && g.u1 > g.u0) {
+      int64_t tri = 0;
+      double flop = 0.0;
+      for (int b = g.b0; b < g.b1; ++b) {
+        const int64_t m = blk_off[b + 1] - blk_off[b];
+        tri += gram_tri_size(m);
+        if (nip[b] > 0) flop += (double)m * (m + 1) * nao;
+      }
+      double* d_X = (double*)work + tri;
+      {
+        ProfScope ps(h, "cand_gram_transpose[byte]", 16.0 * (double)mg * nao);
+        if (kpad != nao) HIP_TRY(h, hipMemsetAsync(d_X, 0, sizeof(double) * (size_t)mg * kpad, h->stream));
+        const int rc = transpose_rm(h, d_ao + p0, ld, nao, mg, d_X, kpad);
+        if (rc != ISDF_OK) return rc;
+      }
+      const int rc = gram_tri_blocks(h, d_X, kpad, kpad, d_units + g.u0, g.u1 - g.u0, d_off, p0, d_tri_off, (double*)work, flop);
+      if (rc != ISDF_OK) return rc;
+      d_S = (const double*)work;
+    }
+    for (int j = 0; j <= g.kmax; ++j) {
+      hipLaunchKernelGGL(find_first_kernel, dim3(gwg), dim3(TPB), 0, h->stream, d_d, d_wg_blk + g.w0, d_wg_lo + g.w0,
+                         d_off, d_st, tie_rtol);
+      hipLaunchKernelGGL(take_pivot_kernel, dim3(gblk), dim3(TPB), 0, h->stream, gram ? nullptr : d_ao, nao, ld, d_L, ldL,
+                         d_d, d_off, d_nip, j, tol, kmax, d_st, d_piv, d_pv, d_pl, nh, d_pvr, g.b0);
+      if (j == g.kmax) break;
+      if (gram) {
+        ProfScope ps(h, "select_update_gram_kernel[byte]", 8.0 * (double)mg * (j + 4));
+        if (lds_panel)
+          hipLaunchKernelGGL((update_kernel<true, true>), dim3(gwg), dim3(TPB), sizeof(double) * (size_t)j, h->stream, d_S, nao, ld,
+                             d_L, ldL, d_d, d_wg_blk + g.w0, d_wg_lo + g.w0, d_off, j, kmax, d_st, d_pv, d_pl, 0, d_pvr, d_tri_off);
+        else
+          hipLaunchKernelGGL((update_kernel<false, true>), dim3(gwg), dim3(TPB), 0, h->stream, d_S, nao, ld, d_L, ldL, d_d,
+                             d_wg_blk + g.w0, d_wg_lo + g.w0, d_off, j, kmax, d_st, d_pv, d_pl, 0, d_pvr, d_tri_off);
+        continue;
+      }
+      ProfScope ps(h, "select_update_kernel[byte]", 8.0 * (double)mtot * (nao + j + 3));
+      if (lds_panel)
+        hipLaunchKernelGGL((update_kernel<true, false>), dim3(gwg), dim3(TPB), sizeof(double) * ((size_t)nao * (nh > 0 ? 2 : 1) + j),
+                           h->stream, d_ao, nao, ld, d_L, ldL, d_d, d_wg_blk + g.w0, d_wg_lo + g.w0, d_off, j, kmax, d_st, d_pv, d_pl,
+                           nh, d_pvr, d_tri_off);
+      else
+        hipLaunchKernelGGL((update_kernel<false, false>), dim3(gwg), dim3(TPB), 0, h->stream, d_ao, nao, ld, d_L, ldL, d_d,
+                           d_wg_blk + g.w0, d_wg_lo + g.w0, d_off, j, kmax, d_st, d_pv, d_pl, nh, d_pvr, d_tri_off);
+    }
+    KERNEL_CHECK(h);
+  }
   HIP_TRY(h, hipMemcpyAsync(h_st.data(), d_st, sizeof(BlkState) * nblk, hipMemcpyDeviceToHost, h->stream));
   HIP_TRY(h, hipStreamSynchronize(h->stream));
   for (int b = 0; b < nblk; ++b) rank[b] = h_st[b].rank;
   return ISDF_OK;
 }
+
+}
+
+extern "C" int isdf_select_ip(isdf_handle h, const double* d_ao, int nao, int64_t ld, int nblk,
+                              const int64_t* blk_off, const int32_t* nip, double tol,
+                              double tie_rtol, double* d_L, int64_t ldL, int64_t* d_piv,
+                              int32_t* rank) {
+  return isdf_select_ip_ws(h, d_ao, nao, ld, nblk, blk_off, nip, tol, tie_rtol, d_L, ldL, d_piv, rank, nullptr, 0);
+}
+
+extern "C" int isdf_select_ip_cplx(isdf_handle h, const double* d_ao, int nao, int nh, int64_t ld, int nblk,
+                                   const int64_t* blk_off, const int32_t* nip, double tol,
+                                   double tie_rtol, double* d_L, int64_t ldL, int64_t* d_piv,
+                                   int32_t* rank) {
+  return select_blocks(h, d_ao, nao, nh, ld, nblk, blk_off, nip, tol, tie_rtol, d_L, ldL, d_piv, rank, nullptr, 0);
+}
+
+extern "C" int isdf_select_ip_ws(isdf_handle h, const double* d_ao, int nao, int64_t ld, int nblk,
+                                 const int64_t* blk_off, const int32_t* nip, double tol,
+                                 double tie_rtol, double* d_L, int64_t ldL, int64_t* d_piv,
+                                 int32_t* rank, void* d_work, int64_t work_bytes) {
+  return select_blocks(h, d_ao, nao, 0, ld, nblk, blk_off, nip, tol, tie_rtol, d_L, ldL, d_piv, rank, d_work, work_bytes);
+}
+
+extern "C" int64_t isdf_select_ip_work_bytes(int nao, int64_t m) {
+  if (nao <= 0 || m <= 0) return 0;
+  return (int64_t)sizeof(double) * (gram_tri_size(m) + m * gram_kpad(nao));
+}
diff --git a/pyscf_isdf_amd/isdf.py b/pyscf_isdf_amd/isdf.py
--- a/pyscf_isdf_amd/isdf.py
+++ b/pyscf_isdf_amd/isdf.py
@@ -42,6 +42,7 @@
         self.w_spectral_check_tol = 5e-9
         self.w_spectral_max_c = 18
         self.cand_skip_zero_rows = True
+        self.cand_gram = True
         self.cand_ao_cutoff = None
         self.tie_rtol = 1e-10
         self.select_tol = -1.0
@@ -341,7 +342,17 @@
         elif self.cand_skip_zero_rows:
             ao_sel = self._nonzero_ao_rows(ao_sel, scratch[nao + kmax:], blk_off)
         piv = be.empty((cell.natm, kmax), dtype=torch.int64)
-        rank = be.select_ip(ao_sel, blk_off, nip, self.select_tol, self.tie_rtol, L, piv)
+        kw = {}
+        if self.cand_gram and hasattr(be, 'select_ip_work_bytes'):
+            used = nao + kmax + (0 if ao_sel.data_ptr() == scratch.data_ptr() else ao_sel.shape[0])
+            work = scratch[used:].reshape(-1)
+            need = [be.select_ip_work_bytes(ao_sel.shape[0], m) for m in counts]
+            if work.numel() * 8 < max(need) <= 1 << 30:
+                work = be.empty(((min(sum(need), 1 << 30) + 256) // 8,))
+            kw['work'] = work
+            del work
+        rank = be.select_ip(ao_sel, blk_off, nip, self.select_tol, self.tie_rtol, L, piv, **kw)
+        kw.clear()
         del ao_sel, L, scratch
         piv_h = be.to_host(piv)
         self._tick('S2_select_candidates' if self.select == 'refined' else 'S2_select_ip', t0)
diff --git a/pyscf_isdf_amd/lib.py b/pyscf_isdf_amd/lib.py
--- a/pyscf_isdf_amd/lib.py
+++ b/pyscf_isdf_amd/lib.py
@@ -30,6 +30,9 @@
     'isdf_gather_cols': (c_int, [c_vp, c_vp, c_int, c_i64, c_vp, c_i64, c_vp, c_i64]),
     'isdf_partition_by_atom': (c_int, [c_vp, c_vp, c_i64, c_vp, c_int, c_vp, c_dbl, c_vp]),
     'isdf_select_ip': (c_int, [c_vp, c_vp, c_int, c_i64, c_int, c_vp, c_vp, c_dbl, c_dbl, c_vp, c_i64, c_vp, c_vp]),
+    'isdf_select_ip_ws': (c_int, [c_vp, c_vp, c_int, c_i64, c_int, c_vp, c_vp, c_dbl, c_dbl, c_vp, c_i64, c_vp, c_vp, c_vp,
+                                  c_i64]),
+    'isdf_select_ip_work_bytes': (c_i64, [c_int, c_i64]),
     'isdf_select_ip_gram': (c_int, [c_vp, c_vp, c_int, c_i64, c_int, c_dbl, c_dbl, c_int, c_vp, ctypes.POINTER(ctypes.c_int32)]),
     'isdf_fit_from_chol': (c_int, [c_vp, c_vp, c_int, c_i64, c_i64, c_vp]),
     'isdf_fit_prepare': (c_int, [c_vp, c_vp, c_int, c_i64, c_vp, c_int, c_dbl, c_vp, c_vp, ctypes.POINTER(c_dbl)]),
```

Result: faster. 17.05 (median of 6 runs) (-5.9%).
